# AdeeshKolluru/AdsorbDiff

Measured on AMD Instinct MI355X. Metric: sampled adsorbate sites/sec (50 denoise steps, ~200-atom slabs), higher is better.
Workload: dtype f32 (f16x3-split MFMA, fp32 accumulate; ADF_GEMM=f32 selects exact f32)

## Files before the change

### adsorbdiff_amd/csrc/api.hip

```cpp
#include <stdarg.h>
#include <stdlib.h>
#include <string.h>

#include <new>

#include "common.h"

static thread_local char g_err[512] = "";

void adf_set_error(const char* fmt, ...) {
    va_list ap;
    va_start(ap, fmt);
    vsnprintf(g_err, sizeof(g_err), fmt, ap);
    va_end(ap);
}

extern "C" const char* adf_last_error(void) { return g_err; }
extern "C" const char* adf_version(void) { return "adsorbdiff_hip 0.5.0 (gfx950)"; }

void adf_prof_begin(adf_painn* h, int cat, hipStream_t s) {
    if (!h->prof_on) return;
    if (h->prof_used + 2 > h->prof_ev->size()) {
        for (int i = 0; i < 512; ++i) {
            hipEvent_t e;
            if (hipEventCreate(&e) != hipSuccess) return;
            h->prof_ev->push_back(e);
        }
    }
    h->prof_cat->push_back(cat);
    (void)hipEventRecord((*h->prof_ev)[h->prof_used], s);
    h->prof_used += 1;
}
void adf_prof_end(adf_painn* h, hipStream_t s) {
    if (!h->prof_on || (h->prof_used & 1) == 0) return;
    (void)hipEventRecord((*h->prof_ev)[h->prof_used], s);
    h->prof_used += 1;
}

extern "C" int32_t adf_profile_enable(adf_painn_t h, int32_t on) {
    if (!h) { adf_set_error("null handle"); return ADF_EINVAL; }
    h->prof_on = on != 0;
    h->prof_used = 0;
    h->prof_cat->clear();
    ADF_HIP_CHECK(hipMemset(h->kcount, 0, 8 * sizeof(unsigned long long)));
    return ADF_OK;
}

extern "C" int32_t adf_profile_read(adf_painn_t h, float* ms, int64_t* count, int64_t* message_ksteps, void* stream) {
    if (!h || !ms || !count) { adf_set_error("null argument"); return ADF_EINVAL; }
    ADF_HIP_CHECK(hipStreamSynchronize((hipStream_t)stream));
    if (message_ksteps) {
        unsigned long long k[8];
        ADF_HIP_CHECK(hipMemcpy(k, h->kcount, sizeof(k), hipMemcpyDeviceToHost));
        ADF_HIP_CHECK(hipMemset(h->kcount, 0, sizeof(k)));
        *message_ksteps = (int64_t)k[0];
    }
    for (int c = 0; c < ADF_PROF_NCAT; ++c) { ms[c] = 0.f; count[c] = 0; }
    const size_t pairs = h->prof_used / 2;
    for (size_t i = 0; i < pairs; ++i) {
        float t = 0.f;
        ADF_HIP_CHECK(hipEventElapsedTime(&t, (*h->prof_ev)[2 * i], (*h->prof_ev)[2 * i + 1]));
        const int c = (*h->prof_cat)[i];
        ms[c] += t;
        count[c] += 1;
    }
    h->prof_used = 0;
    h->prof_cat->clear();
    return ADF_OK;
}

template <typename T>
static int32_t dev_alloc(T** p, size_t count) {
    if (*p) { (void)hipFree(*p); *p = nullptr; }
    if (count == 0) return ADF_OK;
    hipError_t e = hipMalloc(reinterpret_cast<void**>(p), count * sizeof(T));
    if (e != hipSuccess) {
        *p = nullptr;
        (void)hipGetLastError();
        adf_set_error("hipMalloc of %zu bytes failed: %s", count * sizeof(T), hipGetErrorString(e));
        return ADF_EOOM;
    }
    return ADF_OK;
}

extern "C" int32_t adf_painn_create(const adf_painn_hparams* hp, adf_painn_t* out) {
    if (!hp || !out) { adf_set_error("null argument"); return ADF_EINVAL; }
    if (hp->hidden_channels % ADF_SLICE_CH != 0 || hp->hidden_channels < 128 || hp->hidden_channels > 1024) {
        adf_set_error("hidden_channels=%d must be a multiple of %d in [128,1024]", hp->hidden_channels, ADF_SLICE_CH);
        return ADF_EINVAL;
    }
    if (hp->num_rbf % 2 != 0 || hp->num_rbf > 128 || hp->num_rbf < 2) {
        adf_set_error("num_rbf=%d must be even and <= 128", hp->num_rbf);
        return ADF_EINVAL;
    }
    if (hp->max_neighbors < 1 || hp->max_neighbors > ADF_MAX_K) {
        adf_set_error("max_neighbors=%d must be in [1,%d]", hp->max_neighbors, ADF_MAX_K);
        return ADF_EINVAL;
    }
    if (hp->num_layers < 1 || hp->num_layers > 16 || hp->num_heads < 0 || hp->num_heads > 2) {
        adf_set_error("num_layers must be in [1,16], num_heads in [0,2]");
        return ADF_EINVAL;
    }
    adf_painn* h = new (std::nothrow) adf_painn();
    if (!h) { adf_set_error("host allocation failed"); return ADF_EOOM; }
    memset(h, 0, sizeof(*h));
    h->hp = *hp;
    h->prof_ev = new std::vector<hipEvent_t>();
    h->prof_cat = new std::vector<int>();
    hipDeviceProp_t prop;
    if (hipGetDevice(&h->device) != hipSuccess || hipGetDeviceProperties(&prop, h->device) != hipSuccess) {
        adf_set_error("no usable HIP device: %s", hipGetErrorString(hipGetLastError()));
        adf_painn_destroy(h);
        return ADF_EHIP;
    }
    h->num_cus = prop.multiProcessorCount;
    h->dist_floor = 1.0e-3f;
    {
        const char* e = getenv("ADF_INCREMENTAL");
        h->inc_on = !(e && e[0] == '0');
        const char* e2 = getenv("ADF_INC_SYNC");
        h->inc_sync = e2 && e2[0] == '1';
    }
    const int H = hp->hidden_channels, R = hp->num_rbf, L = hp->num_layers;
    int32_t st = dev_alloc(&h->rbf_pack, (size_t)L * (H / ADF_SLICE_CH) * R * 192);
    if (st == ADF_OK) st = dev_alloc(&h->rbf_bias_pack, (size_t)L * (H / ADF_SLICE_CH) * 192);
    {
        uint16_t* p16 = nullptr;
        if (st == ADF_OK) st = dev_alloc(&p16, (size_t)L * (H / ADF_SLICE_CH) * R * 192 * 2);
        h->rbf_pack16 = p16;
    }
    if (st == ADF_OK) st = dev_alloc(&h->rbf_bias_pack16, (size_t)L * (H / ADF_SLICE_CH) * 192);
    if (st == ADF_OK) st = dev_alloc(&h->rbf_scales, 16);
    if (st == ADF_OK) st = dev_alloc(&h->flags, ADF_NFLAGS);
    if (st == ADF_OK && hipMemset(h->flags, 0, sizeof(int32_t) * ADF_NFLAGS) != hipSuccess) st = ADF_EHIP;
    {
        const size_t HH = (size_t)H * H;
        const size_t per_layer = HH + 3 * HH + 2 * HH + 2 * HH + 3 * HH;
        const size_t per_head = HH + HH / 2 + 2 * HH + HH + HH / 4 + HH / 2;
        const size_t elems = (size_t)L * per_layer + (size_t)hp->num_heads * per_head;
        h->w16_bytes = elems * 2 * sizeof(uint16_t) + 4096;
        if (st == ADF_OK) st = dev_alloc(&h->w16_arena, h->w16_bytes);
        if (st == ADF_OK) st = dev_alloc(&h->w16_scales, 256);
        if (st == ADF_OK) st = dev_alloc(&h->w16_bias_perm, (size_t)L * 2 * 3 * H);
        if (st == ADF_OK) st = dev_alloc(&h->w16_scratch, 1);
        if (st == ADF_OK) st = dev_alloc(&h->wfrag_arena, h->w16_bytes);
        {
            const char* ef = getenv("ADF_FUSED_MLP");
            h->fused_mlp = ef ? atoi(ef) : 0;
            if (h->fused_mlp < 0 || h->fused_mlp > 2) h->fused_mlp = 0;
        }
        const char* e = getenv("ADF_GEMM");
        h->gemm_f32 = e && strcmp(e, "f32") == 0;
        const char* el = getenv("ADF_LIFT");
        h->lift_on = !(el && strcmp(el, "0") == 0);
        const char* e2 = getenv("ADF_MSG");
        h->msg_f32 = e2 ? strcmp(e2, "f32") == 0 : h->gemm_f32;
        const char* er = getenv("ADF_ROW_MAXIMA");
        h->rmx = (er && atoi(er) == 0) ? 0 : 1;
    }
    if (st == ADF_OK) st = dev_alloc(&h->kcount, 8);
    if (st == ADF_OK && hipMemset(h->kcount, 0, 8 * sizeof(unsigned long long)) != hipSuccess) st = ADF_EHIP;
    if (st != ADF_OK) { adf_painn_destroy(h); return st; }
    *out = h;
    return ADF_OK;
}

static void inc_free(adf_painn* h) {
    for (int l = 0; l <= ADF_MAX_LAYERS; ++l) {
        if (h->incX[l]) (void)hipFree(h->incX[l]);
        if (h->incV[l]) (void)hipFree(h->incV[l]);
        if (l < ADF_MAX_LAYERS && h->incR[l]) (void)hipFree(h->incR[l]);
        h->incX[l] = h->incV[l] = nullptr;
        if (l < ADF_MAX_LAYERS) h->incR[l] = nullptr;
    }
    void* ptrs[] = {h->inc_c0, h->inc_chg, h->inc_pend, h->inc_need, h->inc_tf, h->inc_list, h->inc_cnt, h->inc_tmp};
    for (void* p : ptrs)
        if (p) (void)hipFree(p);
    h->inc_c0 = h->inc_chg = h->inc_pend = h->inc_need = h->inc_tf = nullptr;
    h->inc_list = h->inc_cnt = nullptr; h->inc_tmp = nullptr; h->inc_tmp_bytes = 0;
    h->inc_capN = 0; h->inc_valid = false;
}

static void free_workspaces(adf_painn* h) {
    void* ptrs[] = {h->nbr_cnt, h->nbr_src, h->nbr_shift, h->deg, h->nptr, h->cursor, h->img_cnt, h->sys_slow, h->scan_tmp,
                    h->e_src, h->e_geom, h->x, h->vecA, h->vecB, h->y, h->xh, h->vv, h->cat, h->dot, h->sys, h->rec, h->lift.buf, h->mag_a, h->mag_b, h->mag_v3,
                    h->rmx_part, h->cache_d2, h->cache_cid, h->cache_cnt, h->prev_nptr, h->prev_src, h->prev_geom};
    for (void* p : ptrs)
        if (p) (void)hipFree(p);
    h->prev_nptr = h->prev_src = nullptr; h->prev_geom = nullptr; h->inc_valid = false;
    h->nbr_cnt = h->nbr_src = h->nbr_shift = h->deg = h->nptr = h->cursor = h->img_cnt = h->sys_slow = h->e_src = nullptr;
    h->scan_tmp = nullptr; h->scan_tmp_bytes = 0;
    h->e_geom = nullptr;
    h->x = h->vecA = h->vecB = h->y = h->xh = h->vv = h->cat = h->dot = h->sys = h->rec = nullptr;
    h->lift.buf = h->mag_a = h->mag_b = h->mag_v3 = nullptr; h->lift.cap = 0; h->mag_v3_valid = false;
    h->rmx_part = h->xpart = h->catpart = h->vpart = nullptr; h->part_stride = 0;
    h->part_x = h->part_vec = nullptr; h->dbg_msg_rows = h->dbg_cat_rows = h->dbg_comb_rows = 0; h->dbg_mag = nullptr;
    h->cache_d2 = nullptr; h->cache_cid = nullptr; h->cache_cnt = nullptr; h->cache_valid = false;
    h->capN = h->capB = h->capE = 0;
}

extern "C" int32_t adf_painn_destroy(adf_painn_t h) {
    if (!h) return ADF_OK;
    free_workspaces(h);
    if (h->rbf_pack) (void)hipFree(h->rbf_pack);
    if (h->rbf_bias_pack) (void)hipFree(h->rbf_bias_pack);
    if (h->rec0) (void)hipFree(h->rec0);
    inc_free(h);
    if (h->inc_cnt_host) (void)hipHostFree(h->inc_cnt_host);
    for (int i = 0; i < 2; ++i)
        if (h->inc_ev[i]) (void)hipEventDestroy((hipEvent_t)h->inc_ev[i]);
    if (h->sub_x) (void)hipFree(h->sub_x);
    if (h->sub_vec) (void)hipFree(h->sub_vec);
    if (h->sub_f) (void)hipFree(h->sub_f);
    if (h->rbf_pack16) (void)hipFree(h->rbf_pack16);
    if (h->rbf_bias_pack16) (void)hipFree(h->rbf_bias_pack16);
    if (h->rbf_scales) (void)hipFree(h->rbf_scales);
    if (h->flags) (void)hipFree(h->flags);
    if (h->kcount) (void)hipFree(h->kcount);
    if (h->w16_arena) (void)hipFree(h->w16_arena);
    if (h->wfrag_arena) (void)hipFree(h->wfrag_arena);
    if (h->w16_scales) (void)hipFree(h->w16_scales);
    if (h->w16_bias_perm) (void)hipFree(h->w16_bias_perm);
    if (h->w16_scratch) (void)hipFree(h->w16_scratch);
    if (h->oe0_buf) (void)hipFree(h->oe0_buf);
    adf_grad_free(h);
    if (h->prof_ev) { for (hipEvent_t e : *h->prof_ev) (void)hipEventDestroy(e); delete h->prof_ev; }
    delete h->prof_cat;
    delete h;
    return ADF_OK;
}

extern "C" int32_t adf_painn_set_weights(adf_painn_t h, int32_t n_weights, const void* const* w,
                                         const float* scale_factors, void* stream) {
    if (!h || !w || !scale_factors) { adf_set_error("null argument"); return ADF_EINVAL; }
    const int L = h->hp.num_layers;
    const int expect = 2 + ADF_WEIGHTS_PER_LAYER * L + ADF_WEIGHTS_PER_HEAD * h->hp.num_heads;
    if (n_weights != expect) {
        adf_set_error("expected %d weight tensors, got %d", expect, n_weights);
        return ADF_EINVAL;
    }
    for (int i = 0; i < n_weights; ++i)
        if (!w[i]) { adf_set_error("weight %d is null", i); return ADF_EINVAL; }
    auto f = [&](int i) { return reinterpret_cast<const float*>(w[i]); };
    h->emb = f(0);
    h->rbf_offset = f(1);
    int k = 2;
    for (int l = 0; l < L; ++l) {
        adf_layer_weights& lw = h->layer[l];
        lw.ln_w = f(k++); lw.ln_b = f(k++); lw.xp0_w = f(k++); lw.xp0_b = f(k++); lw.xp2_w = f(k++); lw.xp2_b = f(k++);
        lw.rbf_w = f(k++); lw.rbf_b = f(k++); lw.vp_w = f(k++); lw.xv0_w = f(k++); lw.xv0_b = f(k++);
        lw.xv2_w = f(k++); lw.xv2_b = f(k++);
        h->scale[l] = scale_factors[l];
    }
    for (int hd = 0; hd < h->hp.num_heads; ++hd)
        for (int b = 0; b < 2; ++b) {
            adf_block_weights& bw = h->head[hd][b];
            bw.vec1_w = f(k++); bw.vec2_w = f(k++); bw.un0_w = f(k++); bw.un0_b = f(k++); bw.un2_w = f(k++);
            bw.un2_b = f(k++);
        }
    ADF_TRY(adf_pack_rbf(h, (hipStream_t)stream));
    {
        hipStream_t s = (hipStream_t)stream;
        const long long H = h->hp.hidden_channels, HH = H * H;
        unsigned char* cur = h->w16_arena;
        unsigned char* fcur = h->wfrag_arena;
        int nscale = 0;
        float* bperm = h->w16_bias_perm;
        auto split = [&](const float* w, long long rows, long long K, adf_w16* out, const float* fused_bias = nullptr,
                         bool pair_perm = false) -> int32_t {
            const long long n = rows * K;
            out->hi = cur; cur += n * 2;
            out->lo = cur; cur += n * 2;
            out->inv_scale = h->w16_scales + nscale++;
            out->bias_perm = nullptr;
            out->frag = nullptr;
            if (fused_bias) {
                out->bias_perm = bperm; bperm += 3 * H;
                ADF_TRY(adf_split_weight(w, n, out, h->w16_scratch, s, (int)H, (int)H, fused_bias));
            } else if (pair_perm) {
                ADF_TRY(adf_split_weight(w, n, out, h->w16_scratch, s, (int)H, (int)H, nullptr, 2));
            } else {
                ADF_TRY(adf_split_weight(w, n, out, h->w16_scratch, s));
            }
            if (rows % 32 == 0 && K % 16 == 0) {
                out->frag = fcur; fcur += n * 4;
                ADF_TRY(adf_pack_frag(out, (int)rows, (int)K, out->frag, s));
            }
            return ADF_OK;
        };
        for (int l = 0; l < L; ++l) {
            adf_layer_weights& lw = h->layer[l];
            ADF_TRY(split(lw.xp0_w, H, H, &lw.xp0_16));
            ADF_TRY(split(lw.xp2_w, 3 * H, H, &lw.xp2_16, lw.xp2_b));
            ADF_TRY(split(lw.vp_w, 2 * H, H, &lw.vp_16, nullptr, true));
            ADF_TRY(split(lw.xv0_w, H, 2 * H, &lw.xv0_16));
            ADF_TRY(split(lw.xv2_w, 3 * H, H, &lw.xv2_16, lw.xv2_b));
        }
        for (int hd = 0; hd < h->hp.num_heads; ++hd) {
            adf_block_weights& b0 = h->head[hd][0];
            adf_block_weights& b1 = h->head[hd][1];
            ADF_TRY(split(b0.vec1_w, H, H, &b0.vec1_16));
            ADF_TRY(split(b0.vec2_w, H / 2, H, &b0.vec2_16));
            ADF_TRY(split(b0.un0_w, H, 2 * H, &b0.un0_16));
            ADF_TRY(split(b0.un2_w, H, H, &b0.un2_16));
            ADF_TRY(split(b1.vec1_w, H / 2, H / 2, &b1.vec1_16));
            ADF_TRY(split(b1.un0_w, H / 2, H, &b1.un0_16));
        }
        if ((size_t)(cur - h->w16_arena) > h->w16_bytes || (size_t)(fcur - h->wfrag_arena) > h->w16_bytes || nscale > 256) {
            adf_set_error("internal: fp16 weight arena overflow");
            return ADF_EINVAL;
        }
    }
    h->weights_set = true;
    h->rec0_valid = false;
    h->inc_valid = false;
    adf_grad_invalidate(h);
    return ADF_OK;
}

static int32_t ensure_capacity(adf_painn* h, int64_t N, int64_t B) {
    if (N <= h->capN && B <= h->capB) return ADF_OK;
    const int64_t capN = N > h->capN ? N : h->capN;
    const int64_t capB = B > h->capB ? B : h->capB;
    ADF_HIP_CHECK(hipDeviceSynchronize());
    free_workspaces(h);
    const int64_t H = h->hp.hidden_channels, K = h->hp.max_neighbors;
    const int64_t capE = 2 * capN * K;
    int32_t st = ADF_OK;
#define ALLOC(field, count) if (st == ADF_OK) st = dev_alloc(&h->field, (size_t)(count))
    ALLOC(nbr_cnt, capN);
    ALLOC(nbr_src, capN * K);
    ALLOC(nbr_shift, capN * K);
    ALLOC(cache_d2, capN * K);
    ALLOC(cache_cid, capN * K);
    ALLOC(cache_cnt, capN);
    ALLOC(deg, capN + 1);
    ALLOC(nptr, capN + 1);
    ALLOC(cursor, capN);
    ALLOC(img_cnt, capB);
    ALLOC(sys_slow, capB);
    ALLOC(e_src, capE);
    ALLOC(e_geom, capE);
    if (h->inc_on) {
        ALLOC(prev_nptr, capN + 1);
        ALLOC(prev_src, capE);
        ALLOC(prev_geom, capE);
    }
    if (st == ADF_OK) {
        h->scan_tmp_bytes = adf_scan_temp_bytes(capN + 1);
        unsigned char* tmp = nullptr;
        st = dev_alloc(&tmp, h->scan_tmp_bytes + 16);
        h->scan_tmp = tmp;
    }
    ALLOC(x, capN * H);
    ALLOC(vecA, capN * 3 * H);
    ALLOC(vecB, capN * 3 * H);
    ALLOC(rec, (capN + 1) * 5 * H);
    ALLOC(y, capN * H);
    ALLOC(xh, capN * 3 * H);
    ALLOC(vv, capN * 6 * H);
    ALLOC(cat, capN * 2 * H);
    ALLOC(dot, capN * H);
    ALLOC(sys, capB * 16);
    ALLOC(lift.buf, capN * 3);
    ALLOC(mag_a, capN);
    ALLOC(mag_b, capN);
    ALLOC(mag_v3, capN * 3);
    const int64_t ps = (capN + 31) / 32 * 32, ns = H / ADF_SLICE_CH;
    if (h->rmx) ALLOC(rmx_part, (4 * ns + H / 32 + 4) * ps);
#undef ALLOC
    h->lift.cap = st == ADF_OK ? capN * 3 : 0;
    if (st != ADF_OK) { free_workspaces(h); return st; }
    if (h->rmx) {
        h->part_stride = ps;
        h->xpart = h->rmx_part; h->catpart = h->xpart + ns * ps; h->vpart = h->catpart + (H / 32) * ps;
        h->dbg_mag = h->vpart + 3 * ns * ps;
    }
    h->capN = capN; h->capB = capB; h->capE = capE;
    return ADF_OK;
}

static int32_t check_batch(const adf_painn* h, const adf_batch* b) {
    if (!h || !b) { adf_set_error("null argument"); return ADF_EINVAL; }
    if (b->num_atoms <= 0 || b->num_systems <= 0) { adf_set_error("empty batch"); return ADF_EINVAL; }
    if (!b->pos || !b->cell || !b->batch || !b->atom_offset) { adf_set_error("null batch array"); return ADF_EINVAL; }
    for (int k = 0; k < 3; ++k)
        if (b->reps[k] < 0 || b->reps[k] > 16) { adf_set_error("reps[%d]=%d out of range", k, b->reps[k]); return ADF_EINVAL; }
    return ADF_OK;
}

static int32_t read_flags(adf_painn* h, hipStream_t s) {
    int32_t f[ADF_NFLAGS];
    ADF_HIP_CHECK(hipMemcpyAsync(f, h->flags, sizeof(f), hipMemcpyDeviceToHost, s));
    ADF_HIP_CHECK(hipMemsetAsync(h->flags, 0, sizeof(f), s));
    ADF_HIP_CHECK(hipStreamSynchronize(s));
    if (f[4]) { adf_set_error("atomic number outside [1, %d] (rows of the embedding table)", h->hp.num_elements); return ADF_EINVAL; }
    if (f[0]) { adf_set_error("a centre atom has more than %d in-cutoff candidates", ADF_MAX_CAND); return ADF_EOVERFLOW; }
    if (f[2]) { adf_set_error("edge buffer overflow"); return ADF_EOVERFLOW; }
    if (f[3]) { adf_set_error("an atom has more than %d incoming edges", ADF_MAX_INDEG); return ADF_EOVERFLOW; }
    if (f[1]) { adf_set_error("An image has no neighbors"); return ADF_ENONEIGHBOR; }
    if (f[6]) { adf_set_error("energy gradient: an edge row has no reverse row in its partner's segment (asymmetric graph)"); return ADF_EINVAL; }
    if (f[5]) {
        adf_set_error("non-finite model output%s", h->gemm_f32 ? " (exact-f32 arithmetic: the inputs or weights are not finite)"
                      : " in f16x3 arithmetic: an activation left the fp16 range or the inputs are not finite; "
                        "adf_painn_set_arithmetic(h, 1) selects exact f32");
        return ADF_ENUMERIC;
    }
    return ADF_OK;
}

extern "C" int32_t adf_graph_set_moving(adf_painn_t h, const int32_t* moving, const int32_t* mov_idx,
                                        const int32_t* mov_off) {
    if (!h) { adf_set_error("null handle"); return ADF_EINVAL; }
    if (moving && (!mov_idx || !mov_off)) { adf_set_error("moving mask needs mov_idx and mov_off"); return ADF_EINVAL; }
    h->moving = moving; h->mov_idx = mov_idx; h->mov_off = mov_off;
    ADF_HIP_CHECK(hipMemset(h->flags, 0, sizeof(int32_t) * ADF_NFLAGS));
    h->cache_valid = false;
    h->rec0_valid = false;
    h->inc_valid = false;
    return ADF_OK;
}

extern "C" int32_t adf_graph_build(adf_painn_t h, const adf_batch* b, void* stream, int64_t* num_edges) {
    ADF_TRY(check_batch(h, b));
    ADF_TRY(ensure_capacity(h, b->num_atoms, b->num_systems));
    hipStream_t s = (hipStream_t)stream;
    ADF_TRY(adf_graph_build_impl(h, b, s));
    if (num_edges) {
        int32_t e = 0;
        ADF_HIP_CHECK(hipMemcpyAsync(&e, h->nptr + b->num_atoms, sizeof(int32_t), hipMemcpyDeviceToHost, s));
        ADF_TRY(read_flags(h, s));
        *num_edges = e;
    }
    return ADF_OK;
}

__global__ void adf_export_edges_kernel(const int32_t* nptr, const int32_t* e_src, const float4* eg, int N,
                                        int32_t* src, int32_t* dst, float* dist, float* vec, long long cap) {
    const int n = blockIdx.x * 4 + (threadIdx.x >> 6);
    if (n >= N) return;
    for (int e = nptr[n] + (threadIdx.x & 63); e < nptr[n + 1]; e += 64) {
        if (e >= cap) continue;
        if (src) src[e] = e_src[e];
        if (dst) dst[e] = n;
        const float4 q = eg[e];
        if (dist) dist[e] = q.w;
        if (vec) { vec[3 * (size_t)e] = q.x; vec[3 * (size_t)e + 1] = q.y; vec[3 * (size_t)e + 2] = q.z; }
    }
}

__global__ void adf_export_shift_kernel(const int32_t* nbr_shift, int32_t* out, long long n, int r0, int r1, int r2) {
    const long long i = (long long)blockIdx.x * blockDim.x + threadIdx.x;
    if (i >= n) return;
    const int c = nbr_shift[i];
    const int n2 = 2 * r2 + 1, n1 = 2 * r1 + 1;
    const int ia = c / (n1 * n2), rem = c - ia * (n1 * n2);
    out[3 * i] = ia - r0;
    out[3 * i + 1] = rem / n2 - r1;
    out[3 * i + 2] = rem % n2 - r2;
}

extern "C" int32_t adf_graph_export(adf_painn_t h, int32_t* nbr_count, int32_t* nbr_src, int32_t* nbr_shift,
                                    int64_t edge_capacity, int32_t* edge_src, int32_t* edge_dst, float* edge_dist,
                                    float* edge_vec, int64_t* num_edges, void* stream) {
    if (!h || h->lastN <= 0) { adf_set_error("no graph built"); return ADF_EINVAL; }
    hipStream_t s = (hipStream_t)stream;
    const int64_t N = h->lastN, K = h->hp.max_neighbors;
    if (nbr_count) ADF_HIP_CHECK(hipMemcpyAsync(nbr_count, h->nbr_cnt, sizeof(int32_t) * N, hipMemcpyDeviceToDevice, s));
    if (nbr_src) ADF_HIP_CHECK(hipMemcpyAsync(nbr_src, h->nbr_src, sizeof(int32_t) * N * K, hipMemcpyDeviceToDevice, s));
    if (nbr_shift)
        hipLaunchKernelGGL(adf_export_shift_kernel, dim3((unsigned)((N * K + 255) / 256)), dim3(256), 0, s, h->nbr_shift,
                           nbr_shift, (long long)(N * K), h->last_reps[0], h->last_reps[1], h->last_reps[2]);
    if (edge_src || edge_dst || edge_dist || edge_vec)
        hipLaunchKernelGGL(adf_export_edges_kernel, dim3((unsigned)((N + 3) / 4)), dim3(256), 0, s, h->nptr, h->e_src,
                           h->e_geom, (int)N, edge_src, edge_dst, edge_dist, edge_vec, (long long)edge_capacity);
    ADF_HIP_CHECK(hipGetLastError());
    int32_t e = 0;
    ADF_HIP_CHECK(hipMemcpyAsync(&e, h->nptr + N, sizeof(int32_t), hipMemcpyDeviceToHost, s));
    ADF_HIP_CHECK(hipStreamSynchronize(s));
    if (num_edges) *num_edges = e;
    return ADF_OK;
}

static int32_t zero_pad_rows(adf_painn* h, int N, hipStream_t s) {
    const size_t row = (size_t)5 * h->hp.hidden_channels;
    ADF_HIP_CHECK(hipMemsetAsync(h->rec + (size_t)N * row, 0, sizeof(float) * row, s));
    return ADF_OK;
}

static bool use_fused_mlp(const adf_painn* h, int rows) {
    if (h->hp.hidden_channels != 512 || h->gemm_f32 || h->fused_mlp == 0) return false;
    if (h->fused_mlp == 1) return true;
    return rows >= 2 * 64 * h->num_cus;
}

static int32_t make_records(adf_painn* h, int l, int n, const float* x, const float* vec, bool vec_is_zero, float* rec,
                            const int32_t* row_map, hipStream_t s) {
    const int H = h->hp.hidden_channels;
    const adf_layer_weights& w = h->layer[l];
    if (n <= 0) return ADF_OK;
    adf_prof_begin(h, ADF_PROF_NODE, s);
    const bool lift = h->lift_on && !h->gemm_f32;
    static int emit = -1;
    if (emit < 0) { const char* e = getenv("ADF_LIFT_EMIT"); emit = (e && atoi(e) == 0) ? 0 : 1; }
    const bool em = lift && emit;
    ADF_TRY(adf_nodewise_layernorm(x, w.ln_w, w.ln_b, h->y, n, H, s, em ? h->mag_a : nullptr, h->rows_dev));
    if (use_fused_mlp(h, n) && (em || !lift)) {
        adf_epi ep = {};
        ep.vec_in = vec; ep.rec = rec ? rec : h->rec; ep.H = H; ep.vec_is_zero = vec_is_zero ? 1 : 0;
        ep.row_map = row_map; ep.m_dev = h->rows_dev; ep.lift_y = lift ? 1 : 0;
        ep.rec_rows = row_map ? (long long)h->inc_capN : (long long)n;
        ADF_TRY(adf_launch_mlp16(h->y, nullptr, H, em ? h->mag_a : nullptr, w.xp0_16.frag, &w.xp0_16, w.xp0_b, w.xp2_16.frag, &w.xp2_16, n,
                                 H, 1, &ep, s));
        adf_prof_end(h, s);
        return ADF_OK;
    }
    ADF_TRY(adf_linear(h, h->y, H, w.xp0_w, &w.xp0_16, w.xp0_b, h->cat, H, n, H, H, 1, s, em ? h->mag_a : nullptr,
                       em ? h->mag_b : nullptr));
    if (h->gemm_f32) {
        if (row_map) { adf_set_error("internal: mapped records need the f16x3 path"); return ADF_EINVAL; }
        ADF_TRY(adf_launch_gemm(h->cat, H, w.xp2_w, H, w.xp2_b, h->xh, 3 * H, n, 3 * H, H, 0, s));
        ADF_TRY(adf_pack_records(h, n, h->xh, vec, vec_is_zero, s, rec));
    } else {
        adf_epi ep = {};
        ep.vec_in = vec; ep.rec = rec ? rec : h->rec; ep.H = H; ep.vec_is_zero = vec_is_zero ? 1 : 0;
        ep.row_map = row_map;
        ep.rmag = em ? h->mag_b : nullptr;
        ep.m_dev = h->rows_dev;
        ADF_TRY(adf_launch_gemm16_fused(h->cat, H, &w.xp2_16, n, H, H, 1, &ep, s, lift ? &h->lift : nullptr));
    }
    adf_prof_end(h, s);
    return ADF_OK;
}

static int32_t message_layer(adf_painn* h, int l, int N, const float* x, const float* vec, float* x_out,
                             float* vec_out, bool vec_is_zero, hipStream_t s, const int32_t* tlist = nullptr,
                             int n_targets = 0, float* rec = nullptr, bool records_ready = false) {
    if (!records_ready) ADF_TRY(make_records(h, l, N, x, vec, vec_is_zero, rec, nullptr, s));
    adf_prof_begin(h, ADF_PROF_MESSAGE, s);
    const int items = tlist ? n_targets : N;
    const bool emit = h->rmx && h->lift_on && !h->gemm_f32 && !h->msg_f32 && items > 0 && items <= h->part_stride;
    h->part_x = h->part_vec = nullptr;
    const int32_t st = adf_message_impl(h, l, N, x, h->xh, vec, x_out, vec_out, vec_is_zero, s, tlist, n_targets, rec,
                                        tlist ? h->rows_dev : nullptr, emit ? h->xpart : nullptr, h->vpart, h->part_stride);
    if (st == ADF_OK && emit) {
        h->part_x = x_out; h->part_vec = vec_out; h->part_n = items; h->part_dev = tlist ? h->rows_dev : nullptr;
        h->dbg_msg_rows = items;
    }
    adf_prof_end(h, s);
    return st;
}

static int32_t update_layer(adf_painn* h, int l, int N, float* x, float* vec, hipStream_t s, bool from_message = true) {
    const int H = h->hp.hidden_channels;
    const adf_layer_weights& w = h->layer[l];
    adf_prof_begin(h, ADF_PROF_NODE, s);
    const bool parts = from_message && h->rmx && h->lift_on && !h->gemm_f32 && N > 0 && h->part_x == x && h->part_vec == vec &&
                       h->part_n == N && h->part_dev == h->rows_dev;
    h->part_x = h->part_vec = nullptr;
    if (h->gemm_f32) {
        ADF_TRY(adf_launch_gemm(vec, H, w.vp_w, H, nullptr, h->vv, 2 * H, 3 * N, 2 * H, H, 0, s));
        ADF_TRY(adf_nodewise_update_prep(h->vv, x, h->cat, h->dot, N, H, s));
        ADF_TRY(adf_linear(h, h->cat, 2 * H, w.xv0_w, &w.xv0_16, w.xv0_b, h->y, H, N, H, 2 * H, 1, s));
    } else {
        adf_epi ep = {};
        ep.v1 = h->vv; ep.dotw = h->dot; ep.cat = h->cat; ep.H = H; ep.m_dev = h->rows_dev;
        const adf_lift* lf = h->lift_on ? &h->lift : nullptr;
        if (parts) {
            ADF_TRY(adf_launch_rowmax_combine(h->vpart, 3 * h->part_stride, H / ADF_SLICE_CH, 3ll * N, h->lift.buf, s, h->rows_dev, 3));
            ep.rmag = h->lift.buf;
            if (h->dbg_capture) ADF_HIP_CHECK(hipMemcpyAsync(h->dbg_mag, h->lift.buf, sizeof(float) * 3 * (size_t)N, hipMemcpyDeviceToDevice, s));
        }
        if (parts || (h->dbg_capture && h->rmx && lf && N <= h->part_stride)) {
            ep.catpart = h->catpart; ep.part_stride = h->part_stride; h->dbg_cat_rows = N;
        }
        ADF_TRY(adf_launch_gemm16_fused(vec, H, &w.vp_16, N, H, H, 3, &ep, s, lf));
        if (parts) {
            ADF_TRY(adf_launch_rowmax_combine(h->xpart, h->part_stride, H / ADF_SLICE_CH + H / 32, N, h->lift.buf, s, h->rows_dev, 1));
            if (h->dbg_capture) {
                ADF_HIP_CHECK(hipMemcpyAsync(h->dbg_mag + 3 * h->part_stride, h->lift.buf, sizeof(float) * (size_t)N, hipMemcpyDeviceToDevice, s));
                h->dbg_comb_rows = N;
            }
        }
        if (use_fused_mlp(h, N)) {
            const float* rm = nullptr;
            if (lf) {
                if (N > lf->cap) { adf_set_error("mlp16: lift scratch holds %lld rows, need %d", lf->cap, N); return ADF_EINVAL; }
                if (!parts) ADF_TRY(adf_launch_rowmag(x, H, H, h->cat, H, N, lf->buf, s, h->rows_dev, 1));
                rm = lf->buf;
            }
            adf_epi e2 = {};
            e2.x = x; e2.vec = vec; e2.dot = h->dot; e2.vv = h->vv; e2.scale = h->scale[l]; e2.H = H;
            e2.m_dev = h->rows_dev; e2.lift_y = h->lift_on ? 1 : 0;
            const int32_t stf = adf_launch_mlp16(x, h->cat, H, rm, w.xv0_16.frag, &w.xv0_16, w.xv0_b, w.xv2_16.frag, &w.xv2_16, N, H, 2, &e2, s);
            adf_prof_end(h, s);
            return stf;
        }
        ADF_TRY(adf_launch_gemm16(x, H, &w.xv0_16, w.xv0_b, h->y, H, N, H, 2 * H, 1, s, h->cat, H, lf, parts ? h->lift.buf : nullptr,
                                  h->lift_on ? h->mag_b : nullptr, h->rows_dev));
    }
    int32_t st;
    if (h->gemm_f32) {
        ADF_TRY(adf_launch_gemm(h->y, H, w.xv2_w, H, w.xv2_b, h->xh, 3 * H, N, 3 * H, H, 0, s));
        st = adf_nodewise_update_apply(h->xh, h->dot, h->vv, x, vec, h->scale[l], N, H, s);
    } else {
        adf_epi ep = {};
        ep.x = x; ep.vec = vec; ep.dot = h->dot; ep.vv = h->vv; ep.scale = h->scale[l]; ep.H = H;
        ep.rmag = h->lift_on ? h->mag_b : nullptr;
        ep.m_dev = h->rows_dev;
        st = adf_launch_gemm16_fused(h->y, H, &w.xv2_16, N, H, H, 2, &ep, s);
    }
    adf_prof_end(h, s);
    return st;
}

extern "C" int32_t adf_painn_message_layer(adf_painn_t h, int32_t layer, int32_t N, const float* x, const float* vec,
                                           float* x_out, float* vec_out, void* stream) {
    if (!h || !h->weights_set || layer < 0 || layer >= h->hp.num_layers || N != h->lastN) {
        adf_set_error("message_layer: bad handle/layer, or N differs from the built graph");
        return ADF_EINVAL;
    }
    hipStream_t s = (hipStream_t)stream;
    ADF_TRY(zero_pad_rows(h, N, s));
    ADF_TRY(message_layer(h, layer, N, x, vec, x_out, vec_out, false, s));
    return ADF_OK;
}

extern "C" int32_t adf_painn_update_layer(adf_painn_t h, int32_t layer, int32_t N, float* x, float* vec, void* stream) {
    if (!h || !h->weights_set || layer < 0 || layer >= h->hp.num_layers) {
        adf_set_error("update_layer: bad handle/layer");
        return ADF_EINVAL;
    }
    ADF_TRY(ensure_capacity(h, N, 1));
    return update_layer(h, layer, N, x, vec, (hipStream_t)stream, false);
}

extern "C" int32_t adf_painn_debug_row_maxima(adf_painn_t h, int32_t which, float* out, int64_t capacity, int32_t* rows,
                                              void* stream) {
    if (!h || which < 0 || which > 6) { adf_set_error("debug_row_maxima: null handle or which outside 0..6"); return ADF_EINVAL; }
    if (which == 4) { h->dbg_capture = capacity != 0; h->dbg_comb_rows = 0; return ADF_OK; }
    const int H = h->hp.hidden_channels, ns = H / ADF_SLICE_CH;
    const int n = which <= 1 ? h->dbg_msg_rows : which <= 3 ? h->dbg_cat_rows : h->dbg_comb_rows;
    if (!h->rmx_part || n <= 0) { adf_set_error("debug_row_maxima: no launch has emitted row maxima (ADF_ROW_MAXIMA=0?)"); return ADF_EINVAL; }
    if (rows) *rows = n;
    if (!out) return ADF_OK;
    const int64_t need = (which == 1 || which == 5) ? 3ll * n : which == 3 ? (int64_t)n * H : n;
    if (capacity < need) { adf_set_error("debug_row_maxima: out holds %lld floats, need %lld", (long long)capacity, (long long)need); return ADF_EINVAL; }
    hipStream_t s = (hipStream_t)stream;
    if (which == 0) return adf_launch_rowmax_combine(h->xpart, h->part_stride, ns, n, out, s);
    if (which == 1) return adf_launch_rowmax_combine(h->vpart, 3 * h->part_stride, ns, 3ll * n, out, s);
    if (which == 2) return adf_launch_rowmax_combine(h->catpart, h->part_stride, H / 32, n, out, s);
    if (which >= 5) {
        ADF_HIP_CHECK(hipMemcpyAsync(out, h->dbg_mag + (which == 5 ? 0 : 3 * h->part_stride), sizeof(float) * (size_t)need, hipMemcpyDeviceToDevice, s));
        return ADF_OK;
    }
    ADF_HIP_CHECK(hipMemcpyAsync(out, h->cat, sizeof(float) * (size_t)n * H, hipMemcpyDeviceToDevice, s));
    return ADF_OK;
}

__global__ void adf_scatter_rows3_kernel(const float* __restrict__ src, const int32_t* __restrict__ idx, int n,
                                         float* __restrict__ dst) {
    const int i = blockIdx.x * blockDim.x + threadIdx.x;
    if (i < 3 * n) dst[(size_t)idx[i / 3] * 3 + i % 3] = src[i];
}

static int32_t forward_impl(adf_painn_t h, const adf_batch* b, const int32_t* out_idx, int32_t n_out, float* f1,
                            float* f2, void* stream, bool head1_only = false);

extern "C" int32_t adf_painn_forward(adf_painn_t h, const adf_batch* b, float* f1, float* f2, void* stream) {
    return forward_impl(h, b, nullptr, 0, f1, f2, stream);
}

extern "C" int32_t adf_painn_forward_subset(adf_painn_t h, const adf_batch* b, const int32_t* out_idx, int32_t n_out,
                                            float* f1, float* f2, void* stream) {
    if (!out_idx || n_out < 0) { adf_set_error("forward_subset: null index list"); return ADF_EINVAL; }
    return forward_impl(h, b, out_idx, n_out, f1, f2, stream);
}

static int inc_prepare(adf_painn* h, int N) {
    const int L = h->hp.num_layers, H = h->hp.hidden_channels;
    if (!h->inc_on || !h->moving || h->gemm_f32 || h->msg_f32 || L > ADF_MAX_LAYERS || !h->prev_nptr)
        return 0;
    if (N > h->inc_capN) {
        (void)hipDeviceSynchronize();
        inc_free(h);
        const size_t cap = (size_t)N;
        int32_t st = ADF_OK;
        for (int l = 0; l <= L && st == ADF_OK; ++l) {
            st = dev_alloc(&h->incX[l], cap * H);
            if (st == ADF_OK && l >= 1) st = dev_alloc(&h->incV[l], cap * 3 * H);
            if (st == ADF_OK && l < L) st = dev_alloc(&h->incR[l], (cap + 1) * 5 * H);
        }
        if (st == ADF_OK) st = dev_alloc(&h->inc_c0, cap);
        if (st == ADF_OK) st = dev_alloc(&h->inc_chg, 2 * cap);
        if (st == ADF_OK) st = dev_alloc(&h->inc_pend, cap * L);
        if (st == ADF_OK) st = dev_alloc(&h->inc_need, cap * L);
        if (st == ADF_OK) st = dev_alloc(&h->inc_tf, cap * L);
        if (st == ADF_OK) st = dev_alloc(&h->inc_list, cap * L);
        if (st == ADF_OK) st = dev_alloc(&h->inc_cnt, (size_t)2 * ADF_MAX_LAYERS + 1);
        if (st == ADF_OK) {
            h->inc_tmp_bytes = adf_inc_temp_bytes((int64_t)cap);
            unsigned char* tmp = nullptr;
            st = dev_alloc(&tmp, h->inc_tmp_bytes + 16);
            h->inc_tmp = tmp;
        }
        if (st == ADF_OK && !h->inc_cnt_host &&
            hipHostMalloc(reinterpret_cast<void**>(&h->inc_cnt_host), sizeof(int32_t) * 2 * (2 * ADF_MAX_LAYERS + 1)) != hipSuccess)
            st = ADF_EOOM;
        for (int i = 0; i < 2 && st == ADF_OK; ++i)
            if (!h->inc_ev[i] && hipEventCreateWithFlags(reinterpret_cast<hipEvent_t*>(&h->inc_ev[i]), hipEventDisableTiming) != hipSuccess)
                st = ADF_EHIP;
        if (st != ADF_OK) {
            (void)hipGetLastError();
            inc_free(h);
            h->inc_on = false;
            fprintf(stderr, "adsorbdiff_hip: no memory for incremental layers (%d atoms), continuing without\n", N);
            return 0;
        }
        h->inc_capN = (int64_t)cap;
    }
    if (h->inc_N != N || h->inc_layers != L || h->build_serial != h->inc_serial) h->inc_valid = false;
    h->inc_N = N; h->inc_layers = L;
    int32_t* tn = h->nptr; h->nptr = h->prev_nptr; h->prev_nptr = tn;
    int32_t* ts = h->e_src; h->e_src = h->prev_src; h->prev_src = ts;
    float4* tg = h->e_geom; h->e_geom = h->prev_geom; h->prev_geom = tg;
    const int state = h->inc_valid ? 1 : 2;
    h->inc_valid = false;
    return state;
}

__global__ void adf_scatter_rows3_kernel(const float* __restrict__ src, const int32_t* __restrict__ idx, int n,
                                         float* __restrict__ dst);

static int32_t inc_harvest(adf_painn* h, int slot, bool wait, bool peek = false) {
    if (!h->inc_ev_live[slot]) return ADF_OK;
    hipEvent_t ev = (hipEvent_t)h->inc_ev[slot];
    if (wait) {
        ADF_HIP_CHECK(hipEventSynchronize(ev));
    } else {
        const hipError_t q = hipEventQuery(ev);
        if (q == hipErrorNotReady) { (void)hipGetLastError(); return ADF_OK; }
        ADF_HIP_CHECK(q);
    }
    const int L = h->inc_layers, N = h->inc_pend_N[slot];
    const int32_t* c = h->inc_cnt_host + (size_t)slot * (2 * ADF_MAX_LAYERS + 1);
    for (int i = 0; i < 2 * L + 1; ++i) h->inc_seen[i] = c[i];
    h->inc_seen_valid = true;
    h->inc_pend_Nseen = N;
    if (peek) return ADF_OK;
    h->inc_ev_live[slot] = false;
    for (int l = 0; l < L; ++l) {
        const bool whole = h->inc_pend_whole[slot][l] != 0;
        h->inc_rows += (unsigned long long)(whole ? N : c[l]);
        h->inc_rows_full += (unsigned long long)N;
        h->inc_edges += (unsigned long long)(whole ? c[2 * L] : c[L + l]);
        if (whole || c[l] > 0) ++h->inc_launches;
    }
    return ADF_OK;
}

static int32_t forward_incremental(adf_painn* h, int N, const int32_t* Z, const int32_t* out_idx, int32_t n_out,
                                   float* f1, float* f2, bool first, int heads, hipStream_t s) {
    const int L = h->hp.num_layers, H = h->hp.hidden_channels;
    const size_t cap = (size_t)h->inc_capN, row = (size_t)5 * H;
    if (out_idx && n_out == 0) return ADF_OK;
    adf_prof_begin(h, ADF_PROF_GRAPH, s);
    if (first) {
        ADF_TRY(adf_nodewise_embed(h, Z, N, h->incX[0], s));
        for (int l = 0; l < L; ++l) ADF_HIP_CHECK(hipMemsetAsync(h->incR[l] + (size_t)N * row, 0, sizeof(float) * row, s));
        ADF_HIP_CHECK(hipMemsetAsync(h->inc_pend, 0, cap * L, s));
    } else {
        ADF_TRY(adf_inc_compare(h, N, s));
    }
    ADF_HIP_CHECK(hipMemsetAsync(h->inc_cnt, 0, sizeof(int32_t) * (2 * ADF_MAX_LAYERS + 1), s));
    if (out_idx) ADF_TRY(adf_inc_need_from_list(h, N, L, out_idx, n_out, s));
    for (int l = 0; l < L; ++l) ADF_TRY(adf_inc_plan_layer(h, l, N, first, out_idx != nullptr, s));
    ADF_HIP_CHECK(hipMemcpyAsync(h->inc_cnt + 2 * L, h->nptr + N, sizeof(int32_t), hipMemcpyDeviceToDevice, s));
    const int slot = h->inc_slot;
    h->inc_slot ^= 1;
    if (h->inc_ev_live[slot]) ADF_TRY(inc_harvest(h, slot, true));
    int32_t* host = h->inc_cnt_host + (size_t)slot * (2 * ADF_MAX_LAYERS + 1);
    ADF_HIP_CHECK(hipMemcpyAsync(host, h->inc_cnt, sizeof(int32_t) * (2 * L + 1), hipMemcpyDeviceToHost, s));
    ADF_HIP_CHECK(hipEventRecord((hipEvent_t)h->inc_ev[slot], s));
    h->inc_ev_live[slot] = true;
    h->inc_pend_N[slot] = N;
    ADF_TRY(inc_harvest(h, slot ^ 1, false));
    if (h->inc_sync) ADF_TRY(inc_harvest(h, slot, true, true));
    adf_prof_end(h, s);
    if (first) ADF_TRY(make_records(h, 0, N, h->incX[0], nullptr, true, h->incR[0], nullptr, s));
    for (int l = 0; l < L; ++l) {
        const int n_seen = h->inc_seen_valid ? h->inc_seen[l] : N;
        const bool whole = first || !h->inc_seen_valid || h->inc_pend_Nseen != N || (long long)n_seen * 10 >= (long long)N * 9;
        h->inc_pend_whole[slot][l] = whole ? 1 : 0;
        if (h->inc_sync && !whole && n_seen == 0) continue;
        const float* vin = l == 0 ? h->vecA : h->incV[l];
        if (whole) {
            ADF_TRY(message_layer(h, l, N, h->incX[l], vin, h->incX[l + 1], h->incV[l + 1], l == 0, s, nullptr, 0,
                                  h->incR[l], true));
            ADF_TRY(update_layer(h, l, N, h->incX[l + 1], h->incV[l + 1], s));
            if (l + 1 < L)
                ADF_TRY(make_records(h, l + 1, N, h->incX[l + 1], h->incV[l + 1], false, h->incR[l + 1], nullptr, s));
            continue;
        }
        const int32_t* list = h->inc_list + cap * l;
        const int ncap = h->inc_sync ? n_seen : N;
        h->rows_dev = h->inc_cnt + l;
        int32_t st = message_layer(h, l, N, h->incX[l], vin, h->x, h->vecB, l == 0, s, list, ncap, h->incR[l], true);
        if (st == ADF_OK) st = update_layer(h, l, ncap, h->x, h->vecB, s);
        if (st == ADF_OK) {
            adf_prof_begin(h, ADF_PROF_NODE, s);
            st = adf_inc_scatter_rows(h->x, list, ncap, H, h->incX[l + 1], s, h->rows_dev);
            if (st == ADF_OK) st = adf_inc_scatter_rows(h->vecB, list, ncap, 3 * H, h->incV[l + 1], s, h->rows_dev);
            adf_prof_end(h, s);
        }
        if (st == ADF_OK && l + 1 < L) st = make_records(h, l + 1, ncap, h->x, h->vecB, false, h->incR[l + 1], list, s);
        h->rows_dev = nullptr;
        ADF_TRY(st);
    }
    adf_prof_begin(h, ADF_PROF_HEADS, s);
    if (!out_idx) {
        if (heads >= 1) ADF_TRY(adf_head_forward(h, 0, N, h->incX[L], h->incV[L], f1, s));
        if (heads == 2) ADF_TRY(adf_head_forward(h, 1, N, h->incX[L], h->incV[L], f2, s));
        h->x_last = h->incX[L];
    } else {
        if (n_out > h->capS) {
            const int64_t c = (int64_t)n_out + n_out / 4 + 64;
            if (h->sub_x) (void)hipFree(h->sub_x);
            if (h->sub_vec) (void)hipFree(h->sub_vec);
            if (h->sub_f) (void)hipFree(h->sub_f);
            h->sub_x = h->sub_vec = h->sub_f = nullptr; h->capS = 0;
            ADF_TRY(dev_alloc(&h->sub_x, (size_t)c * H));
            ADF_TRY(dev_alloc(&h->sub_vec, (size_t)c * 3 * H));
            ADF_TRY(dev_alloc(&h->sub_f, (size_t)c * 3));
            h->capS = c;
        }
        ADF_TRY(adf_inc_gather_rows(h->incX[L], out_idx, n_out, H, h->sub_x, s));
        ADF_TRY(adf_inc_gather_rows(h->incV[L], out_idx, n_out, 3 * H, h->sub_vec, s));
        for (int hd = 0; hd < heads; ++hd) {
            ADF_TRY(adf_head_forward(h, hd, n_out, h->sub_x, h->sub_vec, h->sub_f, s));
            hipLaunchKernelGGL(adf_scatter_rows3_kernel, dim3((3 * n_out + 255) / 256), dim3(256), 0, s, h->sub_f, out_idx,
                               n_out, hd == 0 ? f1 : f2);
        }
        ADF_HIP_CHECK(hipGetLastError());
    }
    adf_prof_end(h, s);
    h->inc_valid = true;
    return ADF_OK;
}

static int32_t forward_impl(adf_painn_t h, const adf_batch* b, const int32_t* out_idx, int32_t n_out, float* f1,
                            float* f2, void* stream, bool head1_only) {
    ADF_TRY(check_batch(h, b));
    if (!h->weights_set) { adf_set_error("weights not set"); return ADF_EINVAL; }
    const int heads = head1_only ? 1 : h->hp.num_heads;
    if (heads > h->hp.num_heads) { adf_set_error("the model has no force head"); return ADF_EINVAL; }
    if (!b->atomic_numbers || (heads >= 1 && !f1) || (heads == 2 && !f2)) { adf_set_error("null argument"); return ADF_EINVAL; }
    h->x_last = nullptr;
    hipStream_t s = (hipStream_t)stream;
    const int N = b->num_atoms;
    ADF_TRY(ensure_capacity(h, N, b->num_systems));
    const int inc = inc_prepare(h, N);
    adf_prof_begin(h, ADF_PROF_GRAPH, s);
    ADF_TRY(adf_graph_build_impl(h, b, s));
    adf_prof_end(h, s);
    if (inc) {
        h->inc_serial = h->build_serial;
        return forward_incremental(h, N, b->atomic_numbers, out_idx, n_out, f1, f2, inc == 2, heads, s);
    }
    ADF_TRY(zero_pad_rows(h, N, s));
    ADF_TRY(adf_nodewise_embed(h, b->atomic_numbers, N, h->x, s));
    float* vin = h->vecA;
    float* vout = h->vecB;
    const int L = h->hp.num_layers, H = h->hp.hidden_channels;
    float* rec0 = nullptr;
    bool rec0_ready = false;
    if (h->moving) {
        const size_t row = (size_t)5 * H;
        if ((int64_t)N + 1 > h->rec0_cap) {
            if (h->rec0) { (void)hipFree(h->rec0); h->rec0 = nullptr; }
            h->rec0_cap = 0; h->rec0_valid = false;
            ADF_TRY(dev_alloc(&h->rec0, ((size_t)N + 1) * row));
            h->rec0_cap = (int64_t)N + 1;
        }
        rec0 = h->rec0;
        rec0_ready = h->rec0_valid && h->rec0_N == N;
        if (!rec0_ready) ADF_HIP_CHECK(hipMemsetAsync(rec0 + (size_t)N * row, 0, sizeof(float) * row, s));
        h->rec0_valid = true; h->rec0_N = N;
    }
    if (!out_idx) {
        for (int l = 0; l < L; ++l) {
            if (l == 0) ADF_TRY(message_layer(h, 0, N, h->x, vin, h->x, vout, true, s, nullptr, 0, rec0, rec0_ready));
            else
            ADF_TRY(message_layer(h, l, N, h->x, vin, h->x, vout, l == 0, s));
            ADF_TRY(update_layer(h, l, N, h->x, vout, s));
            float* t = vin; vin = vout; vout = t;
        }
        adf_prof_begin(h, ADF_PROF_HEADS, s);
        if (heads >= 1) ADF_TRY(adf_head_forward(h, 0, N, h->x, vin, f1, s));
        if (heads == 2) ADF_TRY(adf_head_forward(h, 1, N, h->x, vin, f2, s));
        adf_prof_end(h, s);
        h->x_last = h->x;
        return ADF_OK;
    }
    if (n_out == 0) return ADF_OK;
    if (n_out > h->capS) {
        const int64_t cap = (int64_t)n_out + n_out / 4 + 64;
        if (h->sub_x) (void)hipFree(h->sub_x);
        if (h->sub_vec) (void)hipFree(h->sub_vec);
        if (h->sub_f) (void)hipFree(h->sub_f);
        h->sub_x = h->sub_vec = h->sub_f = nullptr; h->capS = 0;
        ADF_TRY(dev_alloc(&h->sub_x, (size_t)cap * H));
        ADF_TRY(dev_alloc(&h->sub_vec, (size_t)cap * 3 * H));
        ADF_TRY(dev_alloc(&h->sub_f, (size_t)cap * 3));
        h->capS = cap;
    }
    for (int l = 0; l + 1 < L; ++l) {
        if (l == 0) ADF_TRY(message_layer(h, 0, N, h->x, vin, h->x, vout, true, s, nullptr, 0, rec0, rec0_ready));
        else
        ADF_TRY(message_layer(h, l, N, h->x, vin, h->x, vout, l == 0, s));
        ADF_TRY(update_layer(h, l, N, h->x, vout, s));
        float* t = vin; vin = vout; vout = t;
    }
    ADF_TRY(message_layer(h, L - 1, N, h->x, vin, h->sub_x, h->sub_vec, L == 1, s, out_idx, n_out,
                          L == 1 ? rec0 : nullptr, L == 1 && rec0_ready));
    ADF_TRY(update_layer(h, L - 1, n_out, h->sub_x, h->sub_vec, s));
    adf_prof_begin(h, ADF_PROF_HEADS, s);
    for (int hd = 0; hd < heads; ++hd) {
        ADF_TRY(adf_head_forward(h, hd, n_out, h->sub_x, h->sub_vec, h->sub_f, s));
        hipLaunchKernelGGL(adf_scatter_rows3_kernel, dim3((3 * n_out + 255) / 256), dim3(256), 0, s, h->sub_f, out_idx,
                           n_out, hd == 0 ? f1 : f2);
    }
    ADF_HIP_CHECK(hipGetLastError());
    adf_prof_end(h, s);
    return ADF_OK;
}

extern "C" int32_t adf_painn_set_energy_head(adf_painn_t h, int32_t n_weights, const void* const* w, void* stream) {
    if (!h || !w) { adf_set_error("null argument"); return ADF_EINVAL; }
    if (n_weights != 4) { adf_set_error("set_energy_head: expected 4 tensors (out_energy.0.weight/bias, out_energy.2.weight/bias), got %d", n_weights); return ADF_EINVAL; }
    for (int i = 0; i < 4; ++i)
        if (!w[i]) { adf_set_error("energy-head tensor %d is null", i); return ADF_EINVAL; }
    const int H = h->hp.hidden_channels, H2 = H / 2;
    const size_t n = (size_t)H2 * H;
    if (!h->oe0_buf) ADF_TRY(dev_alloc(&h->oe0_buf, n * 4 + 64));
    h->oe0_w = reinterpret_cast<const float*>(w[0]);
    h->oe0_b = reinterpret_cast<const float*>(w[1]);
    h->oe2_w = reinterpret_cast<const float*>(w[2]);
    h->oe2_b = reinterpret_cast<const float*>(w[3]);
    adf_w16& e = h->oe0_16;
    e = adf_w16{};
    e.hi = h->oe0_buf; e.lo = h->oe0_buf + n * 2; e.inv_scale = reinterpret_cast<float*>(h->oe0_buf + n * 4);
    ADF_TRY(adf_split_weight(h->oe0_w, (long long)n, &e, reinterpret_cast<unsigned int*>(h->oe0_buf + n * 4 + 16),
                             (hipStream_t)stream));
    h->energy_set = true;
    adf_grad_invalidate(h);
    return ADF_OK;
}

extern "C" int32_t adf_painn_set_distance_floor(adf_painn_t h, float floor) {
    if (!h || !(floor > 0.f)) { adf_set_error("set_distance_floor: null handle or non-positive floor"); return ADF_EINVAL; }
    if (floor != h->dist_floor) {
        h->dist_floor = floor;
        h->cache_valid = false;
        h->rec0_valid = false;
        h->inc_valid = false;
    }
    return ADF_OK;
}

__global__ __launch_bounds__(256) void adf_energy_sum_kernel(const float* __restrict__ y, int H2, const float* __restrict__ w,
                                                             const float* __restrict__ bias, const int32_t* __restrict__ atom_offset,
                                                             float* __restrict__ energy) {
    __shared__ float part[4];
    const int b = blockIdx.x, lane = threadIdx.x & 63, wave = threadIdx.x >> 6;
    const int a0 = atom_offset[b], a1 = atom_offset[b + 1];
    const float b0 = bias[0];
    float acc = 0.f;
    for (int a = a0 + wave; a < a1; a += 4) {
        const float* row = y + (size_t)a * H2;
        float d = 0.f;
        for (int c = lane; c < H2; c += 64) d = fmaf(row[c], w[c], d);
        for (int o = 32; o > 0; o >>= 1) d = __fadd_rn(d, __shfl_xor(d, o, 64));
        acc = __fadd_rn(acc, __fadd_rn(d, b0));
    }
    if (lane == 0) part[wave] = acc;
    __syncthreads();
    if (threadIdx.x == 0) energy[b] = __fadd_rn(__fadd_rn(part[0], part[1]), __fadd_rn(part[2], part[3]));
}

int32_t adf_energy_sum(const float* y, int H2, const float* w, const float* bias, const int32_t* atom_offset, float* energy,
                       int num_systems, hipStream_t s) {
    hipLaunchKernelGGL(adf_energy_sum_kernel, dim3(num_systems), dim3(256), 0, s, y, H2, w, bias, atom_offset, energy);
    ADF_HIP_CHECK(hipGetLastError());
    return ADF_OK;
}

extern "C" int32_t adf_painn_forward_energy(adf_painn_t h, const adf_batch* b, float* energy, float* forces, void* stream) {
    ADF_TRY(check_batch(h, b));
    if (!h->energy_set) { adf_set_error("forward_energy: energy head not set (adf_painn_set_energy_head)"); return ADF_EINVAL; }
    if (!energy || (h->hp.num_heads >= 1 && !forces)) { adf_set_error("forward_energy: null output"); return ADF_EINVAL; }
    if (h->hp.num_heads > 1) { adf_set_error("forward_energy: the S2EF model has one force head"); return ADF_EINVAL; }
    hipStream_t s = (hipStream_t)stream;
    ADF_TRY(forward_impl(h, b, nullptr, 0, forces, nullptr, stream));
    if (!h->x_last) { adf_set_error("internal: no node features after the forward"); return ADF_EINVAL; }
    const int N = b->num_atoms, H = h->hp.hidden_channels, H2 = H / 2;
    adf_prof_begin(h, ADF_PROF_HEADS, s);
    ADF_TRY(adf_linear(h, h->x_last, H, h->oe0_w, &h->oe0_16, h->oe0_b, h->y, H2, N, H2, H, 1, s));
    ADF_TRY(adf_energy_sum(h->y, H2, h->oe2_w, h->oe2_b, b->atom_offset, energy, b->num_systems, s));
    adf_prof_end(h, s);
    return ADF_OK;
}

extern "C" int32_t adf_linear_forward(const float* A, const float* W, const float* bias, float* C, int32_t M,
                                      int32_t N, int32_t K, int32_t act_ssilu, int32_t mode, void* stream) {
    hipStream_t s = (hipStream_t)stream;
    if (!A || !W || !C || M <= 0 || N <= 0 || K <= 0) { adf_set_error("bad argument"); return ADF_EINVAL; }
    if (mode == 0) return adf_launch_gemm(A, K, W, K, bias, C, N, M, N, K, act_ssilu, s);
    unsigned char* buf = nullptr;
    const size_t n = (size_t)N * K;
    ADF_TRY(dev_alloc(&buf, n * 4 + 64));
    adf_w16 w16 = {};
    w16.hi = buf; w16.lo = buf + n * 2; w16.inv_scale = reinterpret_cast<float*>(buf + n * 4);
    unsigned int* scratch = reinterpret_cast<unsigned int*>(buf + n * 4 + 16);
    int32_t st = adf_split_weight(W, (long long)n, &w16, scratch, s);
    float* mags = nullptr;
    const char* el = getenv("ADF_LIFT");
    const bool lift = !(el && strcmp(el, "0") == 0);
    if (st == ADF_OK && lift) st = dev_alloc(&mags, (size_t)M);
    adf_lift lf = {mags, M};
    if (st == ADF_OK) st = adf_launch_gemm16(A, K, &w16, bias, C, N, M, N, K, act_ssilu, s, nullptr, 0, lift ? &lf : nullptr);
    (void)hipStreamSynchronize(s);
    (void)hipFree(buf);
    if (mags) (void)hipFree(mags);
    return st;
}

extern "C" int32_t adf_painn_set_arithmetic(adf_painn_t h, int32_t exact_f32) {
    if (!h) { adf_set_error("null handle"); return ADF_EINVAL; }
    h->gemm_f32 = exact_f32 != 0;
    h->msg_f32 = exact_f32 != 0;
    h->rec0_valid = false;
    h->inc_valid = false;
    return ADF_OK;
}

extern "C" int32_t adf_painn_set_fused_mlp(adf_painn_t h, int32_t mode) {
    if (!h || mode < 0 || mode > 2) { adf_set_error("set_fused_mlp: mode must be 0 (never), 1 (always) or 2 (by size)"); return ADF_EINVAL; }
    h->fused_mlp = mode;
    return ADF_OK;
}

extern "C" int32_t adf_painn_set_incremental(adf_painn_t h, int32_t on) {
// ... 127 lines not shown
```

### adsorbdiff_amd/csrc/common.h

```cpp
#pragma once
#include <hip/hip_runtime.h>
#include <stdint.h>
#include <stdio.h>
#include <string>
#include <vector>

#include "../../include/adsorbdiff_hip.h"

#define ADF_GROUP_NODES 32
#define ADF_SLICE_CH 64
#define ADF_MAX_CAND 1024
#define ADF_MAX_K 128
#define ADF_NFLAGS 8
#define ADF_MAX_INDEG 1024
#define ADF_MAX_LAYERS 16

void adf_set_error(const char* fmt, ...);

#define ADF_HIP_CHECK(expr)                                                             \
    do {                                                                                \
        hipError_t _e = (expr);                                                         \
        if (_e != hipSuccess) {                                                         \
            adf_set_error("%s failed: %s (%s:%d)", #expr, hipGetErrorString(_e),        \
                          __FILE__, __LINE__);                                          \
            return (_e == hipErrorOutOfMemory) ? ADF_EOOM : ADF_EHIP;                   \
        }                                                                               \
    } while (0)

#define ADF_TRY(expr)                     \
    do {                                  \
        int32_t _s = (expr);              \
        if (_s != ADF_OK) return _s;      \
    } while (0)

struct adf_w16 {
    void* hi;
    void* lo;
    float* inv_scale;
    float* bias_perm;
    void* frag;
};
struct adf_epi {
    const float* vec_in;
    float* rec;
    float* x;
    float* vec;
    const float* dot;
    const float* vv;
    float* v1;
    float* dotw;
    float* cat;
    float scale;
    int H;
    int vec_is_zero;
    const float* A2;
    int K1;
    const int32_t* row_map;
    const float* rmag;
    unsigned int* out_mag;
    const int32_t* m_dev;
    int accumulate;
    int lift_y;
    const float* gate;
    int gate_ld;
    long long rec_rows;
    float* catpart;
    long long part_stride;
};
struct adf_lift {
    float* buf;
    long long cap;
};
struct adf_layer_weights {
    const float *ln_w, *ln_b, *xp0_w, *xp0_b, *xp2_w, *xp2_b, *rbf_w, *rbf_b;
    const float *vp_w, *xv0_w, *xv0_b, *xv2_w, *xv2_b;
    adf_w16 xp0_16, xp2_16, vp_16, xv0_16, xv2_16;
};
struct adf_block_weights {
    const float *vec1_w, *vec2_w, *un0_w, *un0_b, *un2_w, *un2_b;
    adf_w16 vec1_16, vec2_16, un0_16, un2_16;
};

struct adf_painn {
    adf_painn_hparams hp;
    int device;
    bool weights_set;
    const float* emb;
    const float* rbf_offset;
    adf_layer_weights layer[16];
    adf_block_weights head[2][2];
    float scale[16];
    float* rbf_pack;
    float* rbf_bias_pack;
    void* rbf_pack16;
    float* rbf_bias_pack16;
    float* rbf_scales;
    unsigned char* w16_arena;
    size_t w16_bytes;
    float* w16_scales;
    float* w16_bias_perm;
    unsigned int* w16_scratch;
    unsigned char* wfrag_arena;
    int fused_mlp;
    bool gemm_f32;
    bool msg_f32;
    bool lift_on;
    adf_lift lift;
    float *mag_a, *mag_b;
    float* mag_v3;
    bool mag_v3_valid;
    int rmx;
    float* rmx_part;
    float *xpart, *catpart, *vpart;
    int64_t part_stride;
    const float *part_x, *part_vec;
    int part_n;
    const int32_t* part_dev;
    int dbg_msg_rows, dbg_cat_rows;
    bool dbg_capture;
    float* dbg_mag;
    int dbg_comb_rows;

    int64_t capN, capB, capE;
    int32_t* nbr_cnt;
    int32_t* nbr_src;
    int32_t* nbr_shift;
    int32_t* deg;
    int32_t* nptr;
    int32_t* cursor;
    int32_t* img_cnt;
    int32_t* sys_slow;
    void* scan_tmp;
    size_t scan_tmp_bytes;
    const int32_t* moving;
    const int32_t* mov_idx;
    const int32_t* mov_off;
    float* cache_d2;
    int32_t* cache_cid;
    int32_t* cache_cnt;
    bool cache_valid;
    int32_t* e_src;
    float4* e_geom;
    int32_t* flags;
    float *x, *vecA, *vecB, *y, *xh, *vv, *cat, *dot;
    float* rec;
    bool rbf_uniform;
    float* rec0;
    int64_t rec0_cap, rec0_N;
    bool rec0_valid;
    bool inc_on;
    bool inc_valid;
    int64_t inc_capN, inc_N;
    int inc_layers;
    float* incX[ADF_MAX_LAYERS + 1];
    float* incV[ADF_MAX_LAYERS + 1];
    float* incR[ADF_MAX_LAYERS];
    int32_t *prev_nptr, *prev_src;
    float4* prev_geom;
    unsigned char *inc_c0, *inc_chg;
    unsigned char *inc_pend, *inc_need, *inc_tf;
    int32_t* inc_list;
    int32_t* inc_cnt;
    int32_t* inc_cnt_host;
    void* inc_ev[2];
    bool inc_ev_live[2];
    int inc_slot;
    bool inc_sync;
    int32_t inc_seen[2 * ADF_MAX_LAYERS + 1];
    bool inc_seen_valid;
    unsigned char inc_pend_whole[2][ADF_MAX_LAYERS];
    int32_t inc_pend_N[2];
    int32_t inc_pend_Nseen;
    const int32_t* rows_dev;
    void* inc_tmp; size_t inc_tmp_bytes;
    unsigned long long inc_rows, inc_rows_full, inc_edges, inc_launches;
    unsigned long long build_serial, inc_serial;
    float *sub_x, *sub_vec, *sub_f;
    int64_t capS;
    float* sys;
    const float *oe0_w, *oe0_b, *oe2_w, *oe2_b;
    adf_w16 oe0_16;
    unsigned char* oe0_buf;
    bool energy_set;
    const float* x_last;
    float dist_floor;
    void* grad;
    int64_t lastN, lastB;
    int32_t last_reps[3];
    int num_cus;
    bool prof_on;
    std::vector<hipEvent_t>* prof_ev;
    std::vector<int>* prof_cat;
    size_t prof_used;
    unsigned long long* kcount;
};

enum { ADF_PROF_GRAPH = 0, ADF_PROF_MESSAGE = 1, ADF_PROF_NODE = 2, ADF_PROF_HEADS = 3, ADF_PROF_STEPPER = 4 };
void adf_prof_begin(adf_painn* h, int cat, hipStream_t s);
void adf_prof_end(adf_painn* h, hipStream_t s);

int32_t adf_launch_gemm(const float* A, int lda, const float* W, int ldw, const float* bias, float* C, int ldc,
                        int M, int N, int K, int act_ssilu, hipStream_t s);
int32_t adf_launch_gemm16(const float* A, int lda, const adf_w16* W, const float* bias, float* C, int ldc, int M,
                          int N, int K, int act_ssilu, hipStream_t s, const float* A2 = nullptr, int K1 = 0,
                          const adf_lift* lf = nullptr, const float* premag = nullptr, float* out_mag = nullptr,
                          const int32_t* m_dev = nullptr, int accumulate = 0,
                          const float* gate = nullptr, int gate_ld = 0);
int32_t adf_launch_rowmag(const float* A, int lda, int K1, const float* A2, int K2, long long M, float* mag, hipStream_t s,
                          const int32_t* m_dev = nullptr, int m_mul = 1);
int32_t adf_launch_rowmax_combine(const float* part, long long stride, int nparts, long long M, float* mag, hipStream_t s,
                                  const int32_t* m_dev = nullptr, int m_mul = 1);
int32_t adf_split_weight(const float* w, long long n, adf_w16* out, unsigned int* scratch_bits, hipStream_t s,
                         int perm_H = 0, int K = 0, const float* bias = nullptr, int parts = 3);
int32_t adf_launch_gemm16_vecnorm(const float* A, int lda, const adf_w16* W, float* nrm, int M, int N, int K,
                                  hipStream_t s, const adf_lift* lf = nullptr, const float* premag = nullptr);
int32_t adf_launch_gemm16_fused(const float* A, int lda, const adf_w16* W, int M, int H, int K, int epi,
                                const adf_epi* ep, hipStream_t s, const adf_lift* lf = nullptr);
static inline int32_t adf_linear(const adf_painn* h, const float* A, int lda, const float* W, const adf_w16* W16,
                                 const float* bias, float* C, int ldc, int M, int N, int K, int act, hipStream_t s,
                                 const float* premag = nullptr, float* out_mag = nullptr) {
    if (h->gemm_f32) return adf_launch_gemm(A, lda, W, K, bias, C, ldc, M, N, K, act, s);
    return adf_launch_gemm16(A, lda, W16, bias, C, ldc, M, N, K, act, s, nullptr, 0, h->lift_on ? &h->lift : nullptr,
                             h->lift_on ? premag : nullptr, h->lift_on ? out_mag : nullptr, h->rows_dev);
}
int32_t adf_pack_frag(const adf_w16* w, int N, int K, void* out, hipStream_t s);
int32_t adf_launch_mlp16(const float* A1, const float* A2, int lda, const float* rmag, const void* W0f, const adf_w16* W0,
                         const float* bias0, const void* W2f, const adf_w16* W2, int M, int H, int epi, const adf_epi* ep,
                         hipStream_t s);
int32_t adf_graph_build_impl(adf_painn* h, const adf_batch* b, hipStream_t s);
int32_t adf_energy_sum(const float* y, int H2, const float* w, const float* bias, const int32_t* atom_offset, float* energy,
                       int num_systems, hipStream_t s);
__device__ __forceinline__ float adf_row16_max(float v) {
#define ADF_ROR(n_) __int_as_float(__builtin_amdgcn_update_dpp(0, __float_as_int(v), 0x120 + (n_), 0xf, 0xf, false))
    v = fmaxf(v, ADF_ROR(8));
    v = fmaxf(v, ADF_ROR(4));
    v = fmaxf(v, ADF_ROR(2));
    v = fmaxf(v, ADF_ROR(1));
#undef ADF_ROR
    return v;
}
__device__ __forceinline__ float adf_half32_max_hi(float v) {
    v = adf_row16_max(v);
    return fmaxf(v, __int_as_float(__builtin_amdgcn_update_dpp(0, __float_as_int(v), 0x142, 0xa, 0xf, false)));
}
__device__ __forceinline__ float adf_lane8_max(float v) {
#define ADF_DPP(c_) __int_as_float(__builtin_amdgcn_update_dpp(0, __float_as_int(v), (c_), 0xf, 0xf, false))
    v = fmaxf(v, ADF_DPP(0xb1));
    v = fmaxf(v, ADF_DPP(0x4e));
    v = fmaxf(v, ADF_DPP(0x141));
#undef ADF_DPP
    return v;
}
__device__ __forceinline__ float adf_ssilu(float x) { return x / (1.0f + expf(-x)) * 1.6666666666666667f; }
__device__ __forceinline__ float adf_dssilu_times(float x, float w) {
    const float sg = 1.0f / (1.0f + expf(-x));
    return sg * (1.0f + x * (1.0f - sg)) * 1.6666666666666667f * w;
}
void adf_grad_invalidate(adf_painn* h);
void adf_grad_free(adf_painn* h);
bool adf_message_geo_supported(const adf_painn* h);
int32_t adf_message_geo(adf_painn* h, int layer, const float* xh, const float* vec, bool vec_is_zero, float4* part,
                        long long ecap, bool accumulate, hipStream_t s);
size_t adf_inc_temp_bytes(int64_t n);
int32_t adf_inc_compare(adf_painn* h, int N, hipStream_t s);
int32_t adf_inc_need_from_list(adf_painn* h, int N, int L, const int32_t* out_idx, int n_out, hipStream_t s);
int32_t adf_inc_plan_layer(adf_painn* h, int l, int N, bool first, bool have_need, hipStream_t s);
int32_t adf_inc_scatter_rows(const float* src, const int32_t* idx, int n, int width, float* dst, hipStream_t s,
                             const int32_t* n_dev = nullptr);
int32_t adf_inc_gather_rows(const float* src, const int32_t* idx, int n, int width, float* dst, hipStream_t s);
size_t adf_scan_temp_bytes(int64_t n);
int32_t adf_message_impl(adf_painn* h, int layer, int N, const float* x, const float* xh, const float* vec,
                         float* x_out, float* vec_out, bool vec_is_zero, hipStream_t s,
                         const int32_t* tlist = nullptr, int n_targets = 0, const float* rec = nullptr,
                         const int32_t* n_targets_dev = nullptr,
                         float* xpart = nullptr, float* vpart = nullptr, long long part_stride = 0);
int32_t adf_pack_rbf(adf_painn* h, hipStream_t s);
int32_t adf_pack_rbf_layer(adf_painn* h, int l, hipStream_t s);
int32_t adf_pack_records(adf_painn* h, int N, const float* xh, const float* vec, bool vec_is_zero, hipStream_t s,
                         float* rec = nullptr);
int32_t adf_nodewise_embed(adf_painn* h, const int32_t* Z, int N, float* x, hipStream_t s);
int32_t adf_nodewise_layernorm(const float* x, const float* w, const float* b, float* y, int N, int H, hipStream_t s,
                               float* out_mag = nullptr, const int32_t* n_dev = nullptr);
int32_t adf_nodewise_update_prep(const float* vv, const float* x, float* cat, float* dot, int N, int H, hipStream_t s);
int32_t adf_nodewise_update_apply(const float* h3, const float* dot, const float* vv, float* x, float* vec,
                                  float scale, int N, int H, hipStream_t s);
int32_t adf_head_forward(adf_painn* h, int head, int N, const float* x, const float* vec, float* out, hipStream_t s);
int32_t adf_stepper_init(const adf_batch* b, float* pos, const int32_t* tags, const float* noise,
                         hipStream_t s);
int32_t adf_stepper_step(float* sys, const adf_batch* b, float* pos, const int32_t* tags, const int32_t* fixed,
                         const float* f1, const float* f2, const adf_step_coef* coef, const adf_step_coef* coefs_dev,
                         int num_steps, const float* z_tr, const float* z_rot, int32_t early_stop_count,
                         int32_t* state, float* dcom, float* drot, hipStream_t s);
int32_t adf_stepper_tr_step(float* sys, const adf_batch* b, float* pos, const int32_t* tags, const float* f1,
                            const adf_tr_coef* coef, const adf_tr_coef* coefs_dev, int num_steps, const float* z,
                            int32_t early_stop_count, int32_t* state, float* dcom, hipStream_t s);

struct adf_model {
    void* h;
    int32_t (*check)(void* h, const adf_batch* b);
    int32_t (*grow)(void* h, const adf_batch* b, float** sys);
    int32_t (*forward)(void* h, const adf_batch* b, const int32_t* out_idx, int32_t n_out, float* f1, float* f2,
                       hipStream_t s);
    void (*prof)(void* h, bool begin, hipStream_t s);
};
int32_t adf_frames_push_impl(adf_frames* f, const float* src, hipStream_t s);
int32_t adf_model_init_placement(const adf_model& m, const adf_batch* b, float* pos, const int32_t* tags,
                                 const float* noise, hipStream_t s);
int32_t adf_model_sde_step(const adf_model& m, const adf_batch* b, float* pos, const int32_t* tags, const int32_t* fixed,
                           const float* f1, const float* f2, const adf_step_coef* coef, const adf_step_coef* coefs_dev,
                           int32_t num_steps, const float* z_tr, const float* z_rot, int32_t early_stop_count,
                           int32_t* state, float* dcom, float* drot, hipStream_t s);
int32_t adf_model_tr_step(const adf_model& m, const adf_batch* b, float* pos, const int32_t* tags, const float* f1,
                          const adf_tr_coef* coef, const adf_tr_coef* coefs_dev, int32_t num_steps, const float* z,
                          int32_t early_stop_count, int32_t* state, float* dcom, hipStream_t s);
int32_t adf_model_sample(const adf_model& m, const adf_batch* b, float* pos, const int32_t* tags, const int32_t* fixed,
                         const adf_step_coef* coefs_dev, int32_t num_steps, const float* z_tr_all, const float* z_rot_all,
                         int32_t early_stop_count, int32_t poll_every, int32_t* state, const int32_t* out_idx,
                         int32_t n_out, float* f1, float* f2, adf_frames* sink, int32_t frame_every, hipStream_t s);
int32_t adf_model_tr_sample(const adf_model& m, const adf_batch* b, float* pos, const int32_t* tags,
                            const adf_tr_coef* coefs_dev, int32_t num_steps, const float* z_all, int32_t early_stop_count,
                            int32_t poll_every, int32_t* state, const int32_t* out_idx, int32_t n_out, float* f1,
                            adf_frames* sink, int32_t frame_every, hipStream_t s);
```

### adsorbdiff_amd/csrc/gemm16.hip

```cpp
#include <stdlib.h>

#include "common.h"

typedef float f32x16 __attribute__((ext_vector_type(16)));
typedef _Float16 half8 __attribute__((ext_vector_type(8)));
typedef _Float16 half4 __attribute__((ext_vector_type(4)));

#ifndef EPI_ABL
#define EPI_ABL 0
#endif
#ifndef EPI2_POLICY
#define EPI2_POLICY 0
#endif
#ifndef G16_ABL
#define G16_ABL 0
#endif
#ifndef G16_WDEEP
#define G16_WDEEP 1
#endif
#define HK 32
#define TLD3 96
#define TLD2 64
#define HLD 40

__device__ __forceinline__ float adf_pow2_lift(float mx) {
    if (!(mx > 0.f) || !(mx < 3.0e38f)) return 1.0f;
    int e;
    (void)frexpf(mx, &e);
    e = 15 - e;
    e = e > 120 ? 120 : (e < -120 ? -120 : e);
    return ldexpf(1.0f, e);
}

__device__ __forceinline__ float ssilu16(float x) {
    float s = x / (1.0f + expf(-x));
    return s * 1.6666666666666667f;
}

template <int ACT, int MI, int NJ, int EPI, bool WR = false, int NWN = 2>
__global__ __launch_bounds__(128 * NWN, (MI == 4 || NWN == 4 ? 1 : 2)) void adf_gemm_f16x3_kernel(
    const float* __restrict__ A, int lda, const _Float16* __restrict__ Whi, const _Float16* __restrict__ Wlo,
    const float* __restrict__ inv_scale, const float* __restrict__ bias, float* __restrict__ C, int ldc, int Mh, int N,
    int K, int tiles_n, adf_epi ep) {
    const int M = ep.m_dev ? min(Mh, (int)*ep.m_dev) : Mh;
    static_assert(NWN == 2 || WR, "eight waves only with the register-streamed weights");
    constexpr int NT = 128 * NWN;
    constexpr int TM = 64 * MI;
    constexpr int TN = 32 * NJ * NWN;
    constexpr int NA = TM * 8 / NT;
    static_assert(TM * 8 % NT == 0, "A staging: whole float4s per thread");
    constexpr int LDS_WR = 4 * TM * HLD > NT / 64 * 6400 ? 4 * TM * HLD : NT / 64 * 6400;
    __shared__ __attribute__((aligned(16))) _Float16 lds[WR ? LDS_WR : (2 * TM + 2 * TN) * HLD];
    __shared__ float rinv[TM];
    _Float16* Ahi = lds;
    _Float16* Alo = Ahi + TM * HLD;
    _Float16* Bhi = Alo + TM * HLD;
    _Float16* Blo = Bhi + TN * HLD;
    const int tid = threadIdx.x;
    const int lane = tid & 63;
    const int wave = tid >> 6;
    const int wm = (wave / NWN) * (32 * MI);
    const int wn = (wave % NWN) * (32 * NJ);

    const int id = blockIdx.x;
    const int xcd = id & 7;
    const int qd = id >> 3;
    const int tile_m = (qd / tiles_n) * 8 + xcd;
    const int tile_n = qd % tiles_n;
    const int m0 = tile_m * (EPI >= 3 ? TM / 3 : TM);
    const int n0 = tile_n * TN;
    if (m0 >= M) return;

    unsigned int a_goff[NA];
    int a_off[NA];
    float a_rs[NA];
    auto global_row = [&](int row) -> unsigned int {
        if constexpr (EPI >= 3) {
            const int atom = m0 + (row / 96) * 32 + (row & 31), ax = (row % 96) >> 5;
            return (unsigned int)min(atom, M - 1) * 3u + ax;
        } else {
            return (unsigned int)min(m0 + row, M - 1);
        }
    };
#pragma unroll
    for (int i = 0; i < NA; ++i) {
        const int f = tid + NT * i;
        const int row = f >> 3, kq = f & 7;
        const unsigned int grow = global_row(row);
        a_goff[i] = (grow * (unsigned int)lda + kq * 4) * 4u;
        a_off[i] = row * HLD + kq * 4;
        a_rs[i] = ep.rmag ? adf_pow2_lift(ep.rmag[grow]) : 1.0f;
    }
    if (tid < TM) rinv[tid] = ep.rmag ? 1.0f / adf_pow2_lift(ep.rmag[global_row(tid)]) : 1.0f;
    const char* const A1b = reinterpret_cast<const char*>(A);
    const char* const A2b = reinterpret_cast<const char*>(ep.A2) - (size_t)ep.K1 * 4;
    int w_src[NJ];
    int w_off[NJ];
#pragma unroll
    for (int i = 0; i < NJ; ++i) {
        const int f = tid + 256 * i;
        const int row = f >> 2, part = f & 3;
        w_src[i] = min(n0 + row, N - 1) * K + part * 8;
        w_off[i] = row * HLD + part * 8;
    }

    float4 ra[NA];
    half8 rwh[NJ], rwl[NJ];
#pragma unroll
    for (int i = 0; i < NA; ++i) ra[i] = *reinterpret_cast<const float4*>(A1b + a_goff[i]);
    if constexpr (!WR) {
#pragma unroll
        for (int i = 0; i < NJ; ++i) {
            rwh[i] = *reinterpret_cast<const half8*>(Whi + w_src[i]);
            rwl[i] = *reinterpret_cast<const half8*>(Wlo + w_src[i]);
        }
    }
    half8 wfa[NJ][2], wfb[NJ][2];
    const half8* const wfr = reinterpret_cast<const half8*>(Whi) + (size_t)((n0 + wn) / 32) * (K / 16) * 128 + lane;
    auto load_wf = [&](int s_, half8 (&wf)[NJ][2]) {
#pragma unroll
        for (int j = 0; j < NJ; ++j) {
            const size_t base = ((size_t)j * (K / 16) + s_) * 128;
            wf[j][0] = wfr[base];
            wf[j][1] = wfr[base + 64];
        }
    };
    if constexpr (WR) load_wf(0, wfa);

    f32x16 acc[MI][NJ];
#pragma unroll
    for (int i = 0; i < MI; ++i)
#pragma unroll
        for (int j = 0; j < NJ; ++j)
#pragma unroll
            for (int r = 0; r < 16; ++r) acc[i][j][r] = 0.f;

    const int nk = K / HK;
    const int fa = (wm + (lane & 31)) * HLD + (lane >> 5) * 8;
    const int fb = (wn + (lane & 31)) * HLD + (lane >> 5) * 8;
    auto stage_a = [&](int boff = 0) {
#pragma unroll
        for (int i = 0; i < NA; ++i) {
            if (G16_ABL & 2) {
                *reinterpret_cast<float2*>(Ahi + boff + a_off[i]) = make_float2(ra[i].x, ra[i].y);
                *reinterpret_cast<float2*>(Alo + boff + a_off[i]) = make_float2(ra[i].z, ra[i].w);
                continue;
            }
            const float sx = ra[i].x * a_rs[i], sy = ra[i].y * a_rs[i], sz = ra[i].z * a_rs[i], sw = ra[i].w * a_rs[i];
            half4 h, l;
            h[0] = (_Float16)sx; h[1] = (_Float16)sy; h[2] = (_Float16)sz; h[3] = (_Float16)sw;
            l[0] = (_Float16)(sx - (float)h[0]); l[1] = (_Float16)(sy - (float)h[1]);
            l[2] = (_Float16)(sz - (float)h[2]); l[3] = (_Float16)(sw - (float)h[3]);
            *reinterpret_cast<half4*>(Ahi + boff + a_off[i]) = h;
            *reinterpret_cast<half4*>(Alo + boff + a_off[i]) = l;
        }
    };
    auto request_a = [&](int kt1) {
        const int k1 = kt1 * HK;
        const char* ab = ((ep.K1 > 0 && k1 >= ep.K1) ? A2b : A1b) + (size_t)k1 * 4;
#pragma unroll
        for (int i = 0; i < NA; ++i) ra[i] = *reinterpret_cast<const float4*>(ab + ((G16_ABL & 4) ? (a_goff[i] & 127u) : a_goff[i]));
    };
    if constexpr (WR) {
        auto kstep = [&](int boff, int ks, const half8 (&cur)[NJ][2]) {
            if (G16_ABL & 8) { asm volatile("" :: "v"(cur[0][0]), "v"(cur[0][1]), "v"(cur[NJ - 1][0]), "v"(cur[NJ - 1][1])); return; }
#pragma unroll
            for (int i = 0; i < MI; ++i) {
                const half8 ah = *reinterpret_cast<const half8*>(Ahi + boff + fa + i * 32 * HLD + ks * 16);
                const half8 al = *reinterpret_cast<const half8*>(Alo + boff + fa + i * 32 * HLD + ks * 16);
#pragma unroll
                for (int j = 0; j < NJ; ++j) {
                    acc[i][j] = __builtin_amdgcn_mfma_f32_32x32x16_f16(al, cur[j][0], acc[i][j], 0, 0, 0);
                    acc[i][j] = __builtin_amdgcn_mfma_f32_32x32x16_f16(ah, cur[j][1], acc[i][j], 0, 0, 0);
                    acc[i][j] = __builtin_amdgcn_mfma_f32_32x32x16_f16(ah, cur[j][0], acc[i][j], 0, 0, 0);
                }
            }
        };
        {
            constexpr int BUF = 2 * TM * HLD;
            float4 rb[NA];
            auto request_b = [&](int kt1) {
                const int k1 = kt1 * HK;
                const char* ab = ((ep.K1 > 0 && k1 >= ep.K1) ? A2b : A1b) + (size_t)k1 * 4;
#pragma unroll
                for (int i = 0; i < NA; ++i) rb[i] = *reinterpret_cast<const float4*>(ab + ((G16_ABL & 4) ? (a_goff[i] & 127u) : a_goff[i]));
            };
            auto stage_from = [&](const float4 (&src)[NA], int boff) {
#pragma unroll
                for (int i = 0; i < NA; ++i) {
                    if (G16_ABL & 2) {
                        *reinterpret_cast<float2*>(Ahi + boff + a_off[i]) = make_float2(src[i].x, src[i].y);
                        *reinterpret_cast<float2*>(Alo + boff + a_off[i]) = make_float2(src[i].z, src[i].w);
// ... 113 lines not shown
#pragma unroll
            for (int jj = 0; jj < NJ / 2; ++jj) {
                const int cb = n0 + wn + 64 * jj;
                const float bv0 = (bias && cb + q < N) ? bias[cb + q] : 0.f;
                const float bv1 = (bias && cb + 32 + q < N) ? bias[cb + 32 + q] : 0.f;
#pragma unroll
                for (int i = 0; i < MI; ++i) {
#pragma unroll
                    for (int r = 0; r < 16; ++r) {
                        const int lr = (r & 3) + 8 * (r >> 2) + 4 * (lane >> 5);
                        const float sc = isc * rinv[wm + 32 * i + lr];
                        float v0 = acc[i][2 * jj][r] * sc + bv0, v1 = acc[i][2 * jj + 1][r] * sc + bv1;
                        if (ACT) { v0 = ssilu16(v0); v1 = ssilu16(v1); }
                        T[lr * TLD2 + q] = v0;
                        T[lr * TLD2 + 32 + q] = v1;
                    }
                    __builtin_amdgcn_fence(__ATOMIC_RELEASE, "wavefront");
                    __builtin_amdgcn_wave_barrier();
#pragma unroll
                    for (int it = 0; it < 8; ++it) {
                        const int item = lane + 64 * it;
                        const int lr = item >> 4, c4 = item & 15;
                        const int row = m0 + wm + 32 * i + lr, col = cb + 4 * c4;
                        float4 v = *reinterpret_cast<const float4*>(T + lr * TLD2 + 4 * c4);
                        if (row < M && col < N) {
                            if (ep.gate) {
                                const float4 g4 = *reinterpret_cast<const float4*>(ep.gate + (size_t)(row / 3) * ep.gate_ld + col);
                                v.x = g4.x * v.x; v.y = g4.y * v.y; v.z = g4.z * v.z; v.w = g4.w * v.w;
                            }
                            if (ep.accumulate) {
                                const float4 o = *reinterpret_cast<const float4*>(C + (size_t)row * ldc + col);
                                v.x += o.x; v.y += o.y; v.z += o.z; v.w += o.w;
                            }
                            *reinterpret_cast<float4*>(C + (size_t)row * ldc + col) = v;
                        }
                        if (ep.out_mag) {
                            float mg = col < N ? fmaxf(fmaxf(fabsf(v.x), fabsf(v.y)), fmaxf(fabsf(v.z), fabsf(v.w))) : 0.f;
                            mg = adf_row16_max(mg);
                            if (c4 == 0 && row < M) atomicMax(ep.out_mag + row, __float_as_uint(mg));
                        }
                    }
                    __builtin_amdgcn_wave_barrier();
                }
            }
            return;
        }
#pragma unroll
        for (int j = 0; j < NJ; ++j) {
            const int col = n0 + wn + 32 * j + (lane & 31);
            if (col >= N) continue;
            const float bv = bias ? bias[col] : 0.f;
#pragma unroll
            for (int i = 0; i < MI; ++i) {
#pragma unroll
                for (int r = 0; r < 16; ++r) {
                    const int row = m0 + wm + 32 * i + (r & 3) + 8 * (r >> 2) + 4 * (lane >> 5);
                    if (row < M) {
                        float v = acc[i][j][r] * (isc * rinv[row - m0]) + bv;
                        if (ACT) v = ssilu16(v);
                        if (ep.accumulate) v += C[(size_t)row * ldc + col];
                        C[(size_t)row * ldc + col] = v;
                        if (ep.out_mag) atomicMax(ep.out_mag + row, __float_as_uint(fabsf(v)));
                    }
                }
            }
        }
    } else if constexpr (EPI == 3) {
        static_assert(EPI != 3 || (NJ == 2 && MI == 3), "vec_proj epilogue: 3 components x (v1, v2)");
        const int q = lane & 31;
        const int g = (n0 + wn) / 64;
        const int H = ep.H;
        const float inv_sqrt_h = 1.0f / sqrtf((float)H);
        __syncthreads();
        float* T = reinterpret_cast<float*>(lds) + wave * 3200;
        const int a0 = m0 + (wave / NWN) * 32;
        float dv[16], nv[16];
#pragma unroll
        for (int r = 0; r < 16; ++r) {
            const int lr = (r & 3) + 8 * (r >> 2) + 4 * (lane >> 5);
            float d = 0.f, qq = 0.f;
#pragma unroll
            for (int i = 0; i < 3; ++i) {
                const float sc = isc * rinv[wm + 32 * i + lr];
                const float v1 = acc[i][0][r] * sc, v2 = acc[i][1][r] * sc;
                d += v1 * v2;
                qq += v2 * v2;
                T[lr * TLD3 + i * 32 + q] = v1;
            }
            dv[r] = d * inv_sqrt_h;
            nv[r] = sqrtf(qq + 1e-8f);
        }
        __builtin_amdgcn_fence(__ATOMIC_RELEASE, "wavefront");
        __builtin_amdgcn_wave_barrier();
#pragma unroll
        for (int it = 0; it < 4; ++it) {
            const int item = lane + 64 * it;
            const int lr = item >> 3, c4 = item & 7;
            const int n = a0 + lr;
            if (n < M) {
                float* vo = ep.v1 + (size_t)n * 3 * H + 32 * g + 4 * c4;
#pragma unroll
                for (int ax = 0; ax < 3; ++ax) {
                    const float4 tv_ = *reinterpret_cast<const float4*>(T + lr * TLD3 + ax * 32 + 4 * c4);
                    if (G16_ABL & 1) asm volatile("" :: "v"(tv_.x), "v"(tv_.w)); else
                    *reinterpret_cast<float4*>(vo + ax * H) = tv_;
                }
            }
        }
        __builtin_amdgcn_wave_barrier();
#pragma unroll
        for (int r = 0; r < 16; ++r) {
            const int lr = (r & 3) + 8 * (r >> 2) + 4 * (lane >> 5);
            T[lr * TLD3 + q] = dv[r];
            T[lr * TLD3 + 32 + q] = nv[r];
        }
        __builtin_amdgcn_fence(__ATOMIC_RELEASE, "wavefront");
        __builtin_amdgcn_wave_barrier();
#pragma unroll
        for (int it = 0; it < 4; ++it) {
            const int lr = it * 8 + (lane >> 3), c4 = lane & 7;
            const int n = a0 + lr, c = 32 * g + 4 * c4;
            const float4 dv_ = *reinterpret_cast<const float4*>(T + lr * TLD3 + 4 * c4);
            const float4 nv_ = *reinterpret_cast<const float4*>(T + lr * TLD3 + 32 + 4 * c4);
            if (n < M) {
                if (G16_ABL & 1) { asm volatile("" :: "v"(dv_.x), "v"(nv_.w)); } else {
                *reinterpret_cast<float4*>(ep.dotw + (size_t)n * H + c) = dv_;
                *reinterpret_cast<float4*>(ep.cat + (size_t)n * H + c) = nv_;
                }
            }
            if (ep.catpart) {
                const float mg = adf_lane8_max(fmaxf(fmaxf(fmaxf(0.f, fabsf(nv_.x)), fabsf(nv_.y)), fmaxf(fabsf(nv_.z), fabsf(nv_.w))));
                if (c4 == 0 && n < M) ep.catpart[(size_t)g * ep.part_stride + n] = mg;
            }
        }
    } else if constexpr (EPI == 4) {
        static_assert(EPI != 4 || (NJ == 2 && MI == 3), "norm epilogue: 3 components x 64 columns per wave");
        const int q = lane & 31;
        const int cb = n0 + wn;
        __syncthreads();
        float* T = reinterpret_cast<float*>(lds) + wave * 3200;
        const int a0 = m0 + (wave / NWN) * 32;
#pragma unroll
        for (int r = 0; r < 16; ++r) {
            const int lr = (r & 3) + 8 * (r >> 2) + 4 * (lane >> 5);
#pragma unroll
            for (int j = 0; j < 2; ++j) {
                const float a = acc[0][j][r] * (isc * rinv[wm + lr]), b = acc[1][j][r] * (isc * rinv[wm + 32 + lr]),
                            d = acc[2][j][r] * (isc * rinv[wm + 64 + lr]);
                T[lr * TLD2 + j * 32 + q] = sqrtf(a * a + b * b + d * d);
            }
        }
        __builtin_amdgcn_fence(__ATOMIC_RELEASE, "wavefront");
        __builtin_amdgcn_wave_barrier();
#pragma unroll
        for (int it = 0; it < 8; ++it) {
            const int lr = it * 4 + (lane >> 4), c4 = lane & 15;
            const int n = a0 + lr, c = cb + 4 * c4;
            if (n < M && c < N)
                *reinterpret_cast<float4*>(ep.cat + (size_t)n * N + c) = *reinterpret_cast<const float4*>(T + lr * TLD2 + 4 * c4);
        }
    } else {
        static_assert(EPI >= 3 || (NJ == 3 && MI == 2), "fused epilogues are written for the 64 x 96 wave tile");
        if (((EPI_ABL & 1) && EPI == 1) || ((EPI_ABL & 2) && EPI == 2)) {
            float sacc = 0.f;
            for (int i = 0; i < MI; ++i) for (int j = 0; j < NJ; ++j) for (int r = 0; r < 16; ++r) sacc += acc[i][j][r];
            if (ep.H < 0) ep.x[0] = sacc;
            return;
        }
        const int q = lane & 31;
        const int g = (n0 + wn) / 96;
        const int H = ep.H;
        const float b0 = bias[n0 + wn + q], b1 = bias[n0 + wn + 32 + q], b2 = bias[n0 + wn + 64 + q];
        __syncthreads();
        float* T = reinterpret_cast<float*>(lds) + wave * 3200;
#pragma unroll
        for (int i = 0; i < MI; ++i) {
#pragma unroll
            for (int r = 0; r < 16; ++r) {
                const int lr = (r & 3) + 8 * (r >> 2) + 4 * (lane >> 5);
                const float sc = isc * rinv[wm + 32 * i + lr];
                T[lr * TLD3 + q] = acc[i][0][r] * sc + b0;
                T[lr * TLD3 + 32 + q] = acc[i][1][r] * sc + b1;
                T[lr * TLD3 + 64 + q] = acc[i][2][r] * sc + b2;
            }
            __builtin_amdgcn_fence(__ATOMIC_RELEASE, "wavefront");
            __builtin_amdgcn_wave_barrier();
            const int c4 = lane & 7;
            const int c = 32 * g + 4 * c4;
            if constexpr (EPI == 1) {
                float4 v0[4], v1[4], v2[4];
                if (EPI_ABL & 4) { for (int it = 0; it < 4; ++it) { v0[it] = make_float4(1.f, 2.f, 3.f, 4.f); v1[it] = v0[it]; v2[it] = v0[it]; } }
                else if (!ep.vec_is_zero) {
#pragma unroll
                    for (int it = 0; it < 4; ++it) {
                        const int n = min(m0 + wm + 32 * i + it * 8 + (lane >> 3), M - 1);
                        const float* vr = ep.vec_in + (size_t)n * 3 * H + c;
                        v0[it] = *reinterpret_cast<const float4*>(vr);
                        v1[it] = *reinterpret_cast<const float4*>(vr + H);
                        v2[it] = *reinterpret_cast<const float4*>(vr + 2 * H);
                    }
                }
#pragma unroll
                for (int it = 0; it < 4; ++it) {
                    const int lr = it * 8 + (lane >> 3);
                    const int n = m0 + wm + 32 * i + lr;
                    const float4 p0 = *reinterpret_cast<const float4*>(T + lr * TLD3 + 4 * c4);
                    const float4 p1 = *reinterpret_cast<const float4*>(T + lr * TLD3 + 32 + 4 * c4);
                    const float4 p2 = *reinterpret_cast<const float4*>(T + lr * TLD3 + 64 + 4 * c4);
                    if ((EPI_ABL & 8) && n >= 0) { if (ep.H < 0) ep.rec[0] = p0.x + p1.x + p2.x + v0[it].x + v1[it].y + v2[it].z; }
                    else if (n < M) {
                        float* rec = ep.rec + ((size_t)(ep.row_map ? ep.row_map[n] : n) * (H / 32) + g) * 160;
                        float4* ra_ = reinterpret_cast<float4*>(rec + 16 * c4);
                        if (!ep.vec_is_zero) {
                            ra_[0] = make_float4(v0[it].x * p1.x, v1[it].x * p1.x, v2[it].x * p1.x, p0.x);
                            ra_[1] = make_float4(v0[it].y * p1.y, v1[it].y * p1.y, v2[it].y * p1.y, p0.y);
                            ra_[2] = make_float4(v0[it].z * p1.z, v1[it].z * p1.z, v2[it].z * p1.z, p0.z);
                            ra_[3] = make_float4(v0[it].w * p1.w, v1[it].w * p1.w, v2[it].w * p1.w, p0.w);
                        } else {
                            ra_[0] = make_float4(0.f, 0.f, 0.f, p0.x);
                            ra_[1] = make_float4(0.f, 0.f, 0.f, p0.y);
                            ra_[2] = make_float4(0.f, 0.f, 0.f, p0.z);
                            ra_[3] = make_float4(0.f, 0.f, 0.f, p0.w);
                        }
                        *reinterpret_cast<float4*>(rec + 128 + 4 * c4) = p2;
                    }
                }
            } else {
                float4 d[4], xv[4], w1[4][3], tv[4][3];
#pragma unroll
                for (int it = 0; it < 4; ++it) {
                    const int n = min(m0 + wm + 32 * i + it * 8 + (lane >> 3), M - 1);
                    const size_t xo = (size_t)n * H + c;
#if EPI2_POLICY & 2
                    typedef float f32x4_t __attribute__((ext_vector_type(4)));
                    auto ntld = [](const float* p_) { const f32x4_t v = __builtin_nontemporal_load(reinterpret_cast<const f32x4_t*>(p_));
                                                      return make_float4(v.x, v.y, v.z, v.w); };
#define EPI2_LD(p_) ntld(p_)
#else
#define EPI2_LD(p_) (*reinterpret_cast<const float4*>(p_))
#endif
                    d[it] = EPI2_LD(ep.dot + xo);
                    xv[it] = EPI2_LD(ep.x + xo);
                    const float* vr = ep.vec + (size_t)n * 3 * H + c;
                    const float* v1p = ep.vv + (size_t)n * 3 * H + c;
#pragma unroll
                    for (int ax = 0; ax < 3; ++ax) {
                        w1[it][ax] = EPI2_LD(v1p + ax * H);
                        tv[it][ax] = EPI2_LD(vr + ax * H);
                    }
                }
#pragma unroll
                for (int it = 0; it < 4; ++it) {
                    const int lr = it * 8 + (lane >> 3);
                    const int n = m0 + wm + 32 * i + lr;
                    const float4 p0 = *reinterpret_cast<const float4*>(T + lr * TLD3 + 4 * c4);
                    const float4 p1 = *reinterpret_cast<const float4*>(T + lr * TLD3 + 32 + 4 * c4);
                    const float4 p2 = *reinterpret_cast<const float4*>(T + lr * TLD3 + 64 + 4 * c4);
                    const float k2 = 0.70710678118654752f, sc = ep.scale;
                    float4 xo4 = xv[it];
                    xo4.x = (xo4.x + (p0.x + p1.x * d[it].x) * k2) * sc;
                    xo4.y = (xo4.y + (p0.y + p1.y * d[it].y) * k2) * sc;
                    xo4.z = (xo4.z + (p0.z + p1.z * d[it].z) * k2) * sc;
                    xo4.w = (xo4.w + (p0.w + p1.w * d[it].w) * k2) * sc;
#undef EPI2_LD
#if EPI2_POLICY & 1
                    typedef unsigned int u32x4 __attribute__((ext_vector_type(4)));
                    const auto rx = __builtin_amdgcn_make_buffer_rsrc(ep.x, 0, (int)((unsigned int)M * (unsigned int)H * 4u), 0x00020000);
                    const auto rv = __builtin_amdgcn_make_buffer_rsrc(ep.vec, 0, (int)((unsigned int)M * 3u * (unsigned int)H * 4u), 0x00020000);
#define EPI2_ST(r_, p_, base_, v_) __builtin_amdgcn_raw_buffer_store_b128(__builtin_bit_cast(u32x4, v_), r_, (int)(((p_) - (base_)) * 4), 0, 16)
#else
#define EPI2_ST(r_, p_, base_, v_) (*reinterpret_cast<float4*>(p_) = (v_))
#endif
                    if (n < M) {
                        EPI2_ST(rx, ep.x + (size_t)n * H + c, ep.x, xo4);
                        float* vr = ep.vec + (size_t)n * 3 * H + c;
#pragma unroll
                        for (int ax = 0; ax < 3; ++ax) {
                            float4 t = tv[it][ax];
                            const float4 v1 = w1[it][ax];
                            t.x += p2.x * v1.x; t.y += p2.y * v1.y; t.z += p2.z * v1.z; t.w += p2.w * v1.w;
                            EPI2_ST(rv, vr + ax * H, ep.vec, t);
                        }
                    }
#undef EPI2_ST
                }
            }
            __builtin_amdgcn_wave_barrier();
        }
    }
}

__global__ __launch_bounds__(256) void adf_rowmag_kernel(const float* __restrict__ A, int lda, int K1,
                                                         const float* __restrict__ A2, int K2, long long M,
                                                         float* __restrict__ mag, const int32_t* __restrict__ m_dev,
                                                         int m_mul) {
    const long long r = (long long)blockIdx.x * 4 + (threadIdx.x >> 6);
    const int lane = threadIdx.x & 63;
    if (r >= M || (m_dev && r >= (long long)*m_dev * m_mul)) return;
    float mx = 0.f;
    const float* a = A + (size_t)r * lda;
    for (int k = lane * 4; k < K1; k += 256) {
        const float4 v = *reinterpret_cast<const float4*>(a + k);
        mx = fmaxf(fmaxf(fmaxf(mx, fabsf(v.x)), fabsf(v.y)), fmaxf(fabsf(v.z), fabsf(v.w)));
    }
    if (A2) {
        const float* b = A2 + (size_t)r * lda;
        for (int k = lane * 4; k < K2; k += 256) {
            const float4 v = *reinterpret_cast<const float4*>(b + k);
            mx = fmaxf(fmaxf(fmaxf(mx, fabsf(v.x)), fabsf(v.y)), fmaxf(fabsf(v.z), fabsf(v.w)));
        }
    }
#pragma unroll
    for (int o = 32; o > 0; o >>= 1) mx = fmaxf(mx, __shfl_xor(mx, o));
    if (lane == 0) mag[r] = mx;
}

__global__ __launch_bounds__(256) void adf_rowmax_combine_kernel(const float* __restrict__ part, long long stride, int nparts,
                                                                 long long M, float* __restrict__ mag,
                                                                 const int32_t* __restrict__ m_dev, int m_mul) {
    const long long r = (long long)blockIdx.x * 256 + threadIdx.x;
    if (r >= M || (m_dev && r >= (long long)*m_dev * m_mul)) return;
    float mx = 0.f;
    for (int p = 0; p < nparts; ++p) mx = fmaxf(mx, part[(size_t)p * stride + r]);
    mag[r] = mx;
}

int32_t adf_launch_rowmax_combine(const float* part, long long stride, int nparts, long long M, float* mag, hipStream_t s,
                                  const int32_t* m_dev, int m_mul) {
    if (M <= 0) return ADF_OK;
    hipLaunchKernelGGL(adf_rowmax_combine_kernel, dim3((unsigned)((M + 255) / 256)), dim3(256), 0, s, part, stride, nparts, M,
                       mag, m_dev, m_mul);
    ADF_HIP_CHECK(hipGetLastError());
    return ADF_OK;
}

int32_t adf_launch_rowmag(const float* A, int lda, int K1, const float* A2, int K2, long long M, float* mag, hipStream_t s,
                          const int32_t* m_dev, int m_mul) {
    if (M <= 0) return ADF_OK;
    hipLaunchKernelGGL(adf_rowmag_kernel, dim3((unsigned)((M + 3) / 4)), dim3(256), 0, s, A, lda, K1, A2, K2, M, mag, m_dev,
                       m_mul);
    ADF_HIP_CHECK(hipGetLastError());
    return ADF_OK;
}

static int32_t lift_mags(const float* A, int lda, int K1, const float* A2, int K2, long long rows, const adf_lift* lf,
                         const float* premag, const float** out, hipStream_t s, const int32_t* m_dev = nullptr, int m_mul = 1) {
    *out = premag;
    if (!premag && lf && lf->buf) {
        if (rows > lf->cap) { adf_set_error("gemm16: lift scratch holds %lld rows, need %lld", lf->cap, rows); return ADF_EINVAL; }
        ADF_TRY(adf_launch_rowmag(A, lda, K1, A2, K2, rows, lf->buf, s, m_dev, m_mul));
        *out = lf->buf;
    }
    return ADF_OK;
}

__global__ void adf_absmax_kernel(const float* __restrict__ w, long long n, unsigned int* out_bits) {
    float m = 0.f;
    for (long long i = (long long)blockIdx.x * blockDim.x + threadIdx.x; i < n; i += (long long)gridDim.x * blockDim.x)
        m = fmaxf(m, fabsf(w[i]));
#pragma unroll
    for (int o = 32; o > 0; o >>= 1) m = fmaxf(m, __shfl_xor(m, o));
    if ((threadIdx.x & 63) == 0) atomicMax(out_bits, __float_as_uint(m));
}

__global__ void adf_split_kernel(const float* __restrict__ w, long long n, const unsigned int* absmax_bits,
                                 _Float16* __restrict__ hi, _Float16* __restrict__ lo, float* inv_scale, int perm_H,
                                 int K, const float* __restrict__ bias, float* __restrict__ bias_perm, int parts) {
    const float amax = __uint_as_float(*absmax_bits);
    int e = 0;
    if (amax > 0.f) (void)frexpf(amax, &e);
    const float scale = ldexpf(1.0f, 10 - e);
    if (blockIdx.x == 0 && threadIdx.x == 0) *inv_scale = 1.0f / scale;
    for (long long i = (long long)blockIdx.x * blockDim.x + threadIdx.x; i < n; i += (long long)gridDim.x * blockDim.x) {
        long long src = i;
        if (perm_H > 0) {
            const long long prow = i / K;
            const int k = (int)(i - prow * K);
            const int gw = 32 * parts;
            const int g = (int)(prow / gw), part = (int)((prow % gw) / 32), qq = (int)(prow % 32);
            const long long orow = (long long)part * perm_H + 32 * g + qq;
            src = orow * K + k;
            if (k == 0 && bias_perm) bias_perm[prow] = bias ? bias[orow] : 0.f;
        }
        const float v = w[src] * scale;
        const _Float16 h = (_Float16)v;
        hi[i] = h;
        lo[i] = (_Float16)(v - (float)h);
    }
}

int32_t adf_split_weight(const float* w, long long n, adf_w16* out, unsigned int* scratch_bits, hipStream_t s,
                         int perm_H, int K, const float* bias, int parts) {
    ADF_HIP_CHECK(hipMemsetAsync(scratch_bits, 0, sizeof(unsigned int), s));
    hipLaunchKernelGGL(adf_absmax_kernel, dim3(64), dim3(256), 0, s, w, n, scratch_bits);
    hipLaunchKernelGGL(adf_split_kernel, dim3(64), dim3(256), 0, s, w, n, scratch_bits, (_Float16*)out->hi,
                       (_Float16*)out->lo, out->inv_scale, perm_H, K, bias, out->bias_perm, parts);
    ADF_HIP_CHECK(hipGetLastError());
    return ADF_OK;
}

static int32_t check_a_span(long long rows, int lda) {
    if (rows * (long long)lda * 4 >= (1ll << 32)) {
        adf_set_error("gemm16: A operand of %lld rows x %d exceeds the 32-bit offset range, split the batch", rows, lda);
        return ADF_EOOM;
    }
    return ADF_OK;
}

int32_t adf_launch_gemm16(const float* A, int lda, const adf_w16* W, const float* bias, float* C, int ldc, int M,
                          int N, int K, int act_ssilu, hipStream_t s, const float* A2, int K1, const adf_lift* lf,
                          const float* premag, float* out_mag, const int32_t* m_dev, int accumulate, const float* gate,
                          int gate_ld) {
    if (M <= 0) return ADF_OK;
    if (K % HK != 0 || (lda & 3) || (A2 && (K1 <= 0 || K1 % HK != 0 || K1 >= K))) {
        adf_set_error("gemm16: K=%d (K1=%d) must be multiples of %d and lda a multiple of 4", K, K1, HK);
        return ADF_EINVAL;
    }
    ADF_TRY(check_a_span(M, lda));
    static int mi = 0;
    if (!mi) { const char* e = getenv("ADF_GEMM16_MI"); mi = e ? atoi(e) : 2; if (mi != 4) mi = 2; }
    const int TM = 64 * mi, TN = 256;
    const int tiles_n = (N + TN - 1) / TN;
    const int tiles_m = (M + TM - 1) / TM;
    const int tiles_m8 = (tiles_m + 7) / 8 * 8;
    dim3 grid((unsigned)(tiles_m8 * tiles_n));
    adf_epi ep = {};
    ep.A2 = A2; ep.K1 = A2 ? K1 : 0; ep.m_dev = m_dev; ep.accumulate = accumulate;
    ep.gate = gate; ep.gate_ld = gate_ld;
    if (gate && ((N | ldc) & 3)) { adf_set_error("gemm16: the gate epilogue needs N and ldc multiples of 4"); return ADF_EINVAL; }
    ADF_TRY(lift_mags(A, lda, A2 ? K1 : K, A2, A2 ? K - K1 : 0, M, lf, premag, &ep.rmag, s, m_dev, 1));
    if (out_mag) {
        ADF_HIP_CHECK(hipMemsetAsync(out_mag, 0, sizeof(float) * (size_t)M, s));
        ep.out_mag = reinterpret_cast<unsigned int*>(out_mag);
    }
    static int w8 = -1;
    if (w8 < 0) { const char* e = getenv("ADF_GEMM_W8_PLAIN"); w8 = (e && atoi(e) == 0) ? 0 : 1; }
    static int ncu = 0;
    if (!ncu) { int dev = 0; if (hipGetDevice(&dev) != hipSuccess || hipDeviceGetAttribute(&ncu, hipDeviceAttributeMultiprocessorCount, dev) != hipSuccess || ncu <= 0) ncu = 256; }
    const long long wg8 = (long long)((M + 191) / 192) * (N / 256 > 0 ? N / 256 : 1);
    const bool ragged = wg8 < 4ll * ncu && wg8 % ncu != 0 && wg8 % ncu < (3 * ncu) / 10 && wg8 > ncu;
    if (w8 == 1 && W->frag && N % 256 == 0 && (K / HK) % 2 == 0 && mi == 2 && !ragged) {
        const int tn8 = N / 256, tmw8 = ((M + 191) / 192 + 7) / 8 * 8;
        dim3 g8((unsigned)(tmw8 * tn8));
        if (act_ssilu)
            hipLaunchKernelGGL((adf_gemm_f16x3_kernel<1, 3, 2, 0, true, 4>), g8, dim3(512), 0, s, A, lda, (const _Float16*)W->frag,
                               (const _Float16*)nullptr, W->inv_scale, bias, C, ldc, M, N, K, tn8, ep);
        else
            hipLaunchKernelGGL((adf_gemm_f16x3_kernel<0, 3, 2, 0, true, 4>), g8, dim3(512), 0, s, A, lda, (const _Float16*)W->frag,
                               (const _Float16*)nullptr, W->inv_scale, bias, C, ldc, M, N, K, tn8, ep);
        ADF_HIP_CHECK(hipGetLastError());
        return ADF_OK;
    }
#define LAUNCH16(ACT_, MI_)                                                                                  \
    hipLaunchKernelGGL((adf_gemm_f16x3_kernel<ACT_, MI_, 4, 0>), grid, dim3(256), 0, s, A, lda,              \
                       (const _Float16*)W->hi, (const _Float16*)W->lo, W->inv_scale, bias, C, ldc, M, N, K, \
                       tiles_n, ep)
    if (mi == 4) { if (act_ssilu) LAUNCH16(1, 4); else LAUNCH16(0, 4); }
    else { if (act_ssilu) LAUNCH16(1, 2); else LAUNCH16(0, 2); }
#undef LAUNCH16
    ADF_HIP_CHECK(hipGetLastError());
    return ADF_OK;
}

int32_t adf_launch_gemm16_vecnorm(const float* A, int lda, const adf_w16* W, float* nrm, int M, int N, int K,
                                  hipStream_t s, const adf_lift* lf, const float* premag) {
    if (M <= 0) return ADF_OK;
    if (K % HK != 0 || (lda & 3) || (N & 3)) { adf_set_error("gemm16_vecnorm: bad shape"); return ADF_EINVAL; }
    ADF_TRY(check_a_span(3ll * M, lda));
    adf_epi ep = {};
    ep.cat = nrm;
    ADF_TRY(lift_mags(A, lda, K, nullptr, 0, 3ll * M, lf, premag, &ep.rmag, s));
    const int tn = (N + 127) / 128, tm8 = ((M + 63) / 64 + 7) / 8 * 8;
    static int w8 = -1;
    if (w8 < 0) { const char* e = getenv("ADF_GEMM_W8"); w8 = (e && atoi(e) == 0) ? 0 : 1; }
    if (w8 && W->frag && N % 256 == 0 && (K / HK) % 2 == 0) {
        hipLaunchKernelGGL((adf_gemm_f16x3_kernel<0, 3, 2, 4, true, 4>), dim3((unsigned)(tm8 * (N / 256))), dim3(512), 0, s, A, lda,
                           (const _Float16*)W->frag, (const _Float16*)nullptr, W->inv_scale, (const float*)nullptr,
                           (float*)nullptr, 0, M, N, K, N / 256, ep);
        ADF_HIP_CHECK(hipGetLastError());
        return ADF_OK;
    }
    hipLaunchKernelGGL((adf_gemm_f16x3_kernel<0, 3, 2, 4>), dim3((unsigned)(tm8 * tn)), dim3(256), 0, s, A, lda,
                       (const _Float16*)W->hi, (const _Float16*)W->lo, W->inv_scale, (const float*)nullptr,
                       (float*)nullptr, 0, M, N, K, tn, ep);
    ADF_HIP_CHECK(hipGetLastError());
    return ADF_OK;
}

int32_t adf_launch_gemm16_fused(const float* A, int lda, const adf_w16* W, int M, int H, int K, int epi,
                                const adf_epi* ep_in, hipStream_t s, const adf_lift* lf) {
    adf_epi epv = *ep_in;
    const adf_epi* ep = &epv;
    if (M <= 0) return ADF_OK;
    if (K % HK != 0 || (lda & 3) || H % 64 != 0 || (epi != 3 && !W->bias_perm)) {
        adf_set_error("gemm16_fused: bad shape");
        return ADF_EINVAL;
    }
    ADF_TRY(check_a_span(epi == 3 ? 3ll * M : (long long)M, lda));
    ADF_TRY(lift_mags(A, lda, K, nullptr, 0, epi == 3 ? 3ll * M : (long long)M, lf, ep_in->rmag, &epv.rmag, s, ep_in->m_dev,
                      epi == 3 ? 3 : 1));
    const int N = 3 * H, TM = 128, TN = 192;
    const int tiles_n = N / TN;
    const int tiles_m = (M + TM - 1) / TM;
    const int tiles_m8 = (tiles_m + 7) / 8 * 8;
    dim3 grid((unsigned)(tiles_m8 * tiles_n));
    if (epi == 3) {
        const int tn = 2 * H / 128, tm8 = ((M + 63) / 64 + 7) / 8 * 8;
        static int wreg = -1;
        if (wreg < 0) { const char* e = getenv("ADF_GEMM_WREG"); wreg = (e && atoi(e) == 0) ? 0 : 1; }
        static int w8 = -1;
        if (w8 < 0) { const char* e = getenv("ADF_GEMM_W8"); w8 = (e && atoi(e) == 0) ? 0 : 1; }
        if (wreg && W->frag && w8 == 1 && (2 * H) % 256 == 0 && (K / HK) % 2 == 0)
            hipLaunchKernelGGL((adf_gemm_f16x3_kernel<0, 3, 2, 3, true, 4>), dim3((unsigned)(tm8 * (2 * H / 256))), dim3(512), 0, s,
                               A, lda, (const _Float16*)W->frag, (const _Float16*)nullptr, W->inv_scale, (const float*)nullptr,
                               (float*)nullptr, 0, M, 2 * H, K, 2 * H / 256, *ep);
        else
        hipLaunchKernelGGL((adf_gemm_f16x3_kernel<0, 3, 2, 3>), dim3((unsigned)(tm8 * tn)), dim3(256), 0, s, A, lda,
                           (const _Float16*)W->hi, (const _Float16*)W->lo, W->inv_scale, (const float*)nullptr,
                           (float*)nullptr, 0, M, 2 * H, K, tn, *ep);
        ADF_HIP_CHECK(hipGetLastError());
        return ADF_OK;
    }
    static int wf = -1;
    if (wf < 0) { const char* e = getenv("ADF_GEMM_WR_FUSED"); wf = e ? atoi(e) : 2; }
    if (wf && W->frag && (K / HK) % 2 == 0 && (wf == 2 || N % 384 == 0)) {
        const int tnw = wf == 4 ? N / 384 : tiles_n;
        dim3 gw((unsigned)(tiles_m8 * tnw));
#define LAUNCHWF(EPI_, NWN_)                                                                                                  \
        hipLaunchKernelGGL((adf_gemm_f16x3_kernel<0, 2, 3, EPI_, true, NWN_>), gw, dim3(128 * NWN_), 0, s, A, lda,            \
                           (const _Float16*)W->frag, (const _Float16*)nullptr, W->inv_scale, W->bias_perm, (float*)nullptr, 0, \
                           M, N, K, tnw, *ep)
        if (epi == 1) { if (wf == 4) LAUNCHWF(1, 4); else LAUNCHWF(1, 2); }
        else { if (wf == 4) LAUNCHWF(2, 4); else LAUNCHWF(2, 2); }
#undef LAUNCHWF
        ADF_HIP_CHECK(hipGetLastError());
        return ADF_OK;
    }
    if (epi == 1)
        hipLaunchKernelGGL((adf_gemm_f16x3_kernel<0, 2, 3, 1>), grid, dim3(256), 0, s, A, lda, (const _Float16*)W->hi,
                           (const _Float16*)W->lo, W->inv_scale, W->bias_perm, (float*)nullptr, 0, M, N, K, tiles_n, *ep);
    else
        hipLaunchKernelGGL((adf_gemm_f16x3_kernel<0, 2, 3, 2>), grid, dim3(256), 0, s, A, lda, (const _Float16*)W->hi,
                           (const _Float16*)W->lo, W->inv_scale, W->bias_perm, (float*)nullptr, 0, M, N, K, tiles_n, *ep);
    ADF_HIP_CHECK(hipGetLastError());
    return ADF_OK;
}
```

### adsorbdiff_amd/csrc/message.hip

```cpp
#include <stdlib.h>
#include <string.h>

#include "message.h"

#ifndef MSG_ABL
#define MSG_ABL 0
#endif
#ifndef MSG_SKIP
#define MSG_SKIP 1
#endif
#ifndef MSG_EXP_NOXC
#define MSG_EXP_NOXC 0
#endif

__device__ __forceinline__ float wave_min(float v) {
#pragma unroll
    for (int o = 32; o > 0; o >>= 1) v = fminf(v, __shfl_xor(v, o));
    return v;
}
__device__ __forceinline__ float wave_max(float v) {
#pragma unroll
    for (int o = 32; o > 0; o >>= 1) v = fmaxf(v, __shfl_xor(v, o));
    return v;
}

#ifndef FWD_WAVES
#define FWD_WAVES 8
#endif
#ifndef FWD_AHEAD
#define FWD_AHEAD 4
#endif
#define FWD_THREADS (64 * FWD_WAVES)
#define MSG_WAVES_PER_SIMD (FWD_WAVES / 4)
template <bool F16, bool VZ, bool UNI>
__global__ __launch_bounds__(FWD_THREADS, MSG_WAVES_PER_SIMD) void adf_message_kernel(MsgParams p) {
    extern __shared__ __attribute__((aligned(16))) float lds[];
    const int wfloats = F16 ? (2 * MSG_COLS * MSG_LDK) / 2 : p.R * MSG_COLS;
    float* Wl = lds;
    _Float16* Wh = reinterpret_cast<_Float16*>(lds);
    _Float16* Wlo = Wh + MSG_COLS * MSG_LDK;
    float* Bl = lds + wfloats;
    float* Mu = Bl + MSG_COLS;
    float* Meta = Mu + 144;
    int* Ctr = reinterpret_cast<int*>(Meta + FWD_WAVES * 32 * 8);

    const int tid = threadIdx.x;
    const int lane = tid & 63;
    const int wave = tid >> 6;
    const int q = lane & 31;
    const int hi = lane >> 5;
    const int slice = blockIdx.x % p.nslices;
    const int worker = blockIdx.x / p.nslices;
    const int nworkers = gridDim.x / p.nslices;
    const int items = p.items_dev ? min(p.items, (int)*p.items_dev) : p.items;
    const int ngroups = (items + ADF_GROUP_NODES - 1) / ADF_GROUP_NODES;
    if (worker >= ngroups) return;
    const int H = p.H;
    const int c0 = slice * ADF_SLICE_CH;

    {
        if (F16) {
            const int R8 = p.R / 8;
            const half8* src = reinterpret_cast<const half8*>(p.wpack16 + (size_t)slice * 2 * MSG_COLS * p.R);
            const half8 zero8 = {0, 0, 0, 0, 0, 0, 0, 0};
            const _Float16* b16 = reinterpret_cast<const _Float16*>(p.bpack) + (size_t)slice * MSG_COLS * 2;
            for (int i = tid; i < 2 * MSG_COLS * 17; i += FWD_THREADS) {
                const int row = i / 17, piece = i - row * 17;
                half8 v = piece < R8 ? src[row * R8 + piece] : zero8;
                if (piece == 16 && row < MSG_COLS) { v[0] = b16[2 * row]; v[1] = b16[2 * row + 1]; }
                *reinterpret_cast<half8*>(Wh + (size_t)row * MSG_LDK + piece * 8) = v;
            }
        } else {
            const float4* src = reinterpret_cast<const float4*>(p.wpack + (size_t)slice * p.R * MSG_COLS);
            float4* dst = reinterpret_cast<float4*>(Wl);
            const int n4 = p.R * MSG_COLS / 4;
            for (int i = tid; i < n4; i += FWD_THREADS) dst[i] = src[i];
        }
        if (!F16 && tid < MSG_COLS) Bl[tid] = p.bpack[slice * MSG_COLS + tid];
        if (tid < 144) Mu[tid] = (tid < p.R ? p.mu[tid] : 2.0f) * (F16 ? p.sarg : 1.0f);
        if (tid == 0) *Ctr = 0;
    }
    __syncthreads();
    float* meta_w = Meta + wave * 32 * 8;
    const float inv_sqrt3 = 0.57735026918962576f;
    const float inv_sqrt2 = 0.70710678118654752f;
    const float out_scale = F16 ? *p.inv_scale * (1.0f / 256.0f) : 1.0f;
    const float inv_sqrt_h = out_scale / sqrtf((float)H);
    const float umax_scale = (float)(p.R - 1);
    const float coeff2 = p.coeff * 1.44269504088896341f;
    const unsigned int row_bytes = (unsigned int)p.nslices * 1280u;
    const char* recS = reinterpret_cast<const char*>(p.rec) + (size_t)slice * 1280;
    const unsigned int qA = (unsigned int)q * 16u;
    const unsigned int qP = 512u + (unsigned int)q * 4u;

    unsigned int ksteps = 0;

    typedef const __attribute__((address_space(4))) int32_t* cint_ptr;
    const cint_ptr nptr_c = (cint_ptr)p.nptr;
    const cint_ptr tlist_c = (cint_ptr)p.tlist;
    auto fetch_target = [&](int& n_out, int& o_out) -> bool {
        while (true) {
            int t = 0;
            if (lane == 0) t = atomicAdd(Ctr, 1);
            t = __builtin_amdgcn_readfirstlane(t);
            const int g = worker + (t >> 5) * nworkers;
            if (g >= ngroups) return false;
            const int e = g * ADF_GROUP_NODES + (t & 31);
            if (e < items) { o_out = e; n_out = p.tlist ? tlist_c[e] : e; return true; }
        }
    };
    auto load_block = [&](int eb, int e1, float4& geo, int& src, bool& valid) {
        const int e = eb + q;
        valid = e < e1;
        geo = make_float4(0.f, 0.f, 0.f, 0.f);
        src = 0;
        if (valid) { geo = p.e_geom[e]; src = p.e_src[e]; }
    };

    int n = 0, orow = 0, eb = 0, e1 = 0;
    bool have = fetch_target(n, orow);
    if (have) { eb = nptr_c[n]; e1 = nptr_c[n + 1]; }
    int nN = 0, oN = 0, e0N = 0, e1N = 0;
    bool haveN = have && fetch_target(nN, oN);
    if (haveN) { e0N = nptr_c[nN]; e1N = nptr_c[nN + 1]; }
    float4 geo = make_float4(0.f, 0.f, 0.f, 0.f); int src = 0; bool valid = false;
    if (have) load_block(eb, e1, geo, src, valid);
    asm volatile("" : "+v"(geo.x), "+v"(geo.y), "+v"(geo.z), "+v"(geo.w), "+v"(src));
    bool first = true;
    float sx0 = 0.f, sx1 = 0.f, sa0 = 0.f, sa1 = 0.f, sb0 = 0.f, sb1 = 0.f, sc0 = 0.f, sc1 = 0.f;
    float ra0 = 0.f, ra1 = 0.f, rb0 = 0.f, rb1 = 0.f, rc0 = 0.f, rc1 = 0.f;
    float res0 = 0.f, res1 = 0.f, res2 = 0.f, res3 = 0.f;

    while (have) {
        {
            const bool last = eb + 32 >= e1;
            float4 geoN = make_float4(0.f, 0.f, 0.f, 0.f); int srcN = 0; bool validN = false;
            if (!last) load_block(eb + 32, e1, geoN, srcN, validN);
            else if (haveN) load_block(e0N, e1N, geoN, srcN, validN);
            if (first) {
                const size_t xo = (size_t)n * H + c0 + q;
                const size_t vo = (size_t)n * 3 * H + c0 + q;
                if (hi == 0) {
                    res0 = p.x[xo]; res1 = p.x[xo + 32];
                    if (!VZ) { res2 = p.vec[vo]; res3 = p.vec[vo + 32]; }
                } else if (!VZ) {
                    res0 = p.vec[vo + H]; res1 = p.vec[vo + H + 32];
                    res2 = p.vec[vo + 2 * H]; res3 = p.vec[vo + 2 * H + 32];
                }
            }

            const float xs = geo.w * p.inv_cutoff;
            float xp = xs;
            if (p.env_pi == 5) { const float x2 = xs * xs; xp = x2 * x2 * xs; }
            else for (int i = 1; i < p.env_pi; ++i) xp *= xs;
            float env = 1.0f + p.env_a * xp + p.env_b * (xp * xs) + p.env_c * (xp * xs * xs);
            env = (xs < 1.0f && valid) ? env : 0.0f;
            __builtin_amdgcn_wave_barrier();
            if (hi == 0) {
                float* m = meta_w + q * 8;
                m[0] = __uint_as_float((unsigned int)(valid ? src : p.N) * row_bytes);
                m[1] = geo.x; m[2] = geo.y; m[3] = geo.z;
            }
            __builtin_amdgcn_fence(__ATOMIC_RELEASE, "wavefront");
            __builtin_amdgcn_wave_barrier();
            const float u = xs * umax_scale;
            const int nvalid = __builtin_amdgcn_readfirstlane(min(32, e1 - eb));
            const float umin = __int_as_float(__builtin_amdgcn_readlane(__float_as_int(u), 0));
            const float umax = __int_as_float(__builtin_amdgcn_readlane(__float_as_int(u), max(nvalid, 1) - 1));
            int klo, khi;
            if (nvalid <= 0) {
                klo = 0; khi = 16;
            } else if (F16) {
                klo = max(0, (int)floorf(umin) - 5) & ~7;
                khi = min(p.R, (int)ceilf(umax) + 6);
                khi = klo + ((khi - klo + 15) & ~15);
                if (khi > 128) { klo -= khi - 128; khi = 128; }
            } else {
                klo = max(0, (int)floorf(umin) - 7) & ~1;
                khi = min(p.R, ((int)ceilf(umax) + 8 + 1) & ~1);
            }
            klo = __builtin_amdgcn_readfirstlane(klo);
            khi = __builtin_amdgcn_readfirstlane(khi);
            ksteps += (khi - klo) * (VZ && F16 ? 4 : 6);

#define ROW_OF(r) ((r & 3) + 8 * (r >> 2) + 4 * hi)
#define DECL(r)                                                                                 \
    const float* m##r = meta_w + ROW_OF(r) * 8;                                                 \
    float4 ga0##r, ga1##r;                                      \
    float gz0##r, gz1##r;
#define GATHER(r)                                                                               \
    {                                                                                           \
    const unsigned int o##r = __float_as_uint(m##r[0]);                                         \
    if (MSG_EXP_NOXC) { gz0##r = 1.0f; gz1##r = 2.0f; } else {                                 \
    gz0##r = *reinterpret_cast<const float*>(recS + (size_t)(o##r + qP));                       \
    gz1##r = *reinterpret_cast<const float*>(recS + (size_t)(o##r + qP) + 640); }               \
    if (MSG_EXP_NOXC == 2) { ga0##r = make_float4(1.f, 2.f, 3.f, 4.f); ga1##r = ga0##r; }      \
    else if (!VZ) {                                                                             \
        ga0##r = *reinterpret_cast<const float4*>(recS + (size_t)(o##r + qA));                  \
        ga1##r = *reinterpret_cast<const float4*>(recS + (size_t)(o##r + qA) + 640);            \
    } else {                                                                                    \
        ga0##r = make_float4(0.f, 0.f, 0.f, *reinterpret_cast<const float*>(recS + (size_t)(o##r + qA) + 12)); \
        ga1##r = make_float4(0.f, 0.f, 0.f, *reinterpret_cast<const float*>(recS + (size_t)(o##r + qA) + 652)); \
    }                                                                                           \
    }
#define CONSUME(r)                                                                              \
    {                                                                                           \
        const float ux = m##r[1], uy = m##r[2], uz = m##r[3];                                   \
        const float t3 = gz0##r * acc[4][r];                                                    \
        sx0 += ga0##r.w * acc[0][r];                                                            \
        if (!VZ) { sa0 += ga0##r.x * acc[2][r]; sb0 += ga0##r.y * acc[2][r]; sc0 += ga0##r.z * acc[2][r]; } \
        ra0 += t3 * ux; rb0 += t3 * uy; rc0 += t3 * uz;                                         \
        const float u3 = gz1##r * acc[5][r];                                                    \
        sx1 += ga1##r.w * acc[1][r];                                                            \
        if (!VZ) { sa1 += ga1##r.x * acc[3][r]; sb1 += ga1##r.y * acc[3][r]; sc1 += ga1##r.z * acc[3][r]; } \
        ra1 += u3 * ux; rb1 += u3 * uy; rc1 += u3 * uz;                                         \
    }
            DECL(0) DECL(1) DECL(2) DECL(3) DECL(4) DECL(5) DECL(6) DECL(7)
            DECL(8) DECL(9) DECL(10) DECL(11) DECL(12) DECL(13) DECL(14) DECL(15)
            GATHER(0) GATHER(1)
#if FWD_AHEAD == 4
            GATHER(2) GATHER(3)
#endif

            const float env256 = env * 256.0f;
            f32x16 acc[6];
            if (F16) {
                half8 aone = {0, 0, 0, 0, 0, 0, 0, 0};
                if (hi == 0) { aone[0] = (_Float16)256.0f; aone[1] = (_Float16)256.0f; }
                const f32x16 zero16 = {0.f, 0.f, 0.f, 0.f, 0.f, 0.f, 0.f, 0.f, 0.f, 0.f, 0.f, 0.f, 0.f, 0.f, 0.f, 0.f};
// ... 121 lines not shown
                    CONSUME(12) CONSUME(13) CONSUME(14) CONSUME(15)
                }
            }
#else
            GATHER(4) GATHER(5) GATHER(6) GATHER(7)
            CONSUME(0) CONSUME(1) CONSUME(2) CONSUME(3)
            GATHER(8) GATHER(9) GATHER(10) GATHER(11)
            CONSUME(4) CONSUME(5) CONSUME(6) CONSUME(7)
            GATHER(12) GATHER(13) GATHER(14) GATHER(15)
            CONSUME(8) CONSUME(9) CONSUME(10) CONSUME(11)
            CONSUME(12) CONSUME(13) CONSUME(14) CONSUME(15)
#endif
#undef GATHER
#undef DECL
#undef CONSUME
#undef ROW_OF
            if (last) {
                sx0 *= out_scale; sx1 *= out_scale;
                sa0 = (sa0 * inv_sqrt3 + ra0) * inv_sqrt_h; sa1 = (sa1 * inv_sqrt3 + ra1) * inv_sqrt_h;
                sb0 = (sb0 * inv_sqrt3 + rb0) * inv_sqrt_h; sb1 = (sb1 * inv_sqrt3 + rb1) * inv_sqrt_h;
                sc0 = (sc0 * inv_sqrt3 + rc0) * inv_sqrt_h; sc1 = (sc1 * inv_sqrt3 + rc1) * inv_sqrt_h;
                sx0 += __shfl_xor(sx0, 32); sx1 += __shfl_xor(sx1, 32);
                sa0 += __shfl_xor(sa0, 32); sa1 += __shfl_xor(sa1, 32);
                sb0 += __shfl_xor(sb0, 32); sb1 += __shfl_xor(sb1, 32);
                sc0 += __shfl_xor(sc0, 32); sc1 += __shfl_xor(sc1, 32);
                const size_t xo = (size_t)orow * H + c0 + q;
                const size_t vo = (size_t)orow * 3 * H + c0 + q;
                float o0, o1, o2, o3;
                if (hi == 0) {
                    o0 = (res0 + sx0) * inv_sqrt2; o1 = (res1 + sx1) * inv_sqrt2;
                    o2 = res2 + sa0; o3 = res3 + sa1;
                    p.x_out[xo] = o0;
                    p.x_out[xo + 32] = o1;
                    p.vec_out[vo] = o2;
                    p.vec_out[vo + 32] = o3;
                } else {
                    o0 = res0 + sb0; o1 = res1 + sb1;
                    o2 = res2 + sc0; o3 = res3 + sc1;
                    p.vec_out[vo + H] = o0;
                    p.vec_out[vo + H + 32] = o1;
                    p.vec_out[vo + 2 * H] = o2;
                    p.vec_out[vo + 2 * H + 32] = o3;
                }
                if (p.xpart) {
                    const float mA = adf_half32_max_hi(fmaxf(fmaxf(0.f, fabsf(o0)), fabsf(o1)));
                    const float mB = adf_half32_max_hi(fmaxf(fmaxf(0.f, fabsf(o2)), fabsf(o3)));
                    if (q == 16) {
                        float* vp = p.vpart + (size_t)slice * 3 * p.part_stride + (size_t)orow * 3;
                        if (hi == 0) { p.xpart[(size_t)slice * p.part_stride + orow] = mA; vp[0] = mB; }
                        else { vp[1] = mA; vp[2] = mB; }
                    }
                }
                sx0 = sx1 = sa0 = sa1 = sb0 = sb1 = sc0 = sc1 = 0.f;
                ra0 = ra1 = rb0 = rb1 = rc0 = rc1 = 0.f;
                res0 = res1 = res2 = res3 = 0.f;
                have = haveN;
                n = nN; orow = oN; eb = e0N; e1 = e1N;
                first = true;
                if (have) {
                    haveN = fetch_target(nN, oN);
                    if (haveN) { e0N = nptr_c[nN]; e1N = nptr_c[nN + 1]; }
                }
            } else {
                eb += 32;
                first = false;
            }
            geo = geoN; src = srcN; valid = validN;
        }
    }
    if (p.kcount && lane == 0) atomicAdd(p.kcount, (unsigned long long)ksteps);
}

__global__ void adf_pack_rbf_kernel(const float* __restrict__ w, const float* __restrict__ b, float* wpack,
                                    float* bpack, int H, int R) {
    const int nslices = H / ADF_SLICE_CH;
    const int total = nslices * R * MSG_COLS;
    for (int i = blockIdx.x * blockDim.x + threadIdx.x; i < total; i += gridDim.x * blockDim.x) {
        const int col = i % MSG_COLS;
        const int k = (i / MSG_COLS) % R;
        const int slice = i / (MSG_COLS * R);
        const int part = col / 64, j = (col >> 5) & 1, qq = col & 31;
        const int ch = slice * ADF_SLICE_CH + 32 * j + qq;
        wpack[i] = w[(size_t)(part * H + ch) * R + k];
        if (k == 0) bpack[slice * MSG_COLS + col] = b[part * H + ch];
    }
}

__global__ void adf_pack_rbf16_kernel(const float* __restrict__ w, const float* __restrict__ b,
                                      const unsigned int* absmax_bits, _Float16* wpack16, float* bpack16,
                                      float* inv_scale, int H, int R) {
    const float amax = __uint_as_float(*absmax_bits);
    int e = 0;
    if (amax > 0.f) (void)frexpf(amax, &e);
    const float scale = ldexpf(1.0f, 10 - e);
    if (blockIdx.x == 0 && threadIdx.x == 0) *inv_scale = 1.0f / scale;
    const int nslices = H / ADF_SLICE_CH;
    const int total = nslices * MSG_COLS * R;
    for (int i = blockIdx.x * blockDim.x + threadIdx.x; i < total; i += gridDim.x * blockDim.x) {
        const int k = i % R;
        const int col = (i / R) % MSG_COLS;
        const int slice = i / (R * MSG_COLS);
        const int part = col / 64, j = (col >> 5) & 1, qq = col & 31;
        const int ch = slice * ADF_SLICE_CH + 32 * j + qq;
        const float v = w[(size_t)(part * H + ch) * R + k] * scale;
        const _Float16 h = (_Float16)v;
        const size_t base = (size_t)slice * 2 * MSG_COLS * R;
        wpack16[base + (size_t)col * R + k] = h;
        wpack16[base + (size_t)(MSG_COLS + col) * R + k] = (_Float16)(v - (float)h);
        if (k == 0) {
            const float bv = b[part * H + ch] * scale;
            const _Float16 bh = (_Float16)bv;
            _Float16* o = reinterpret_cast<_Float16*>(bpack16 + slice * MSG_COLS + col);
            o[0] = bh; o[1] = (_Float16)(bv - (float)bh);
        }
    }
}

__global__ void adf_absmax_kernel(const float* __restrict__ w, long long n, unsigned int* out_bits);

__global__ void adf_pack_records_kernel(const float* __restrict__ xh, const float* __restrict__ vec,
                                        float* __restrict__ rec, int N, int H, int vec_is_zero) {
    const int ng = H / 32;
    const long long total = (long long)N * ng * 32;
    for (long long t = (long long)blockIdx.x * blockDim.x + threadIdx.x; t < total;
         t += (long long)gridDim.x * blockDim.x) {
        const int qq = (int)(t & 31);
        const int g = (int)((t >> 5) % ng);
        const long long n = t / (32LL * ng);
        const int c = 32 * g + qq;
        const float* xr = xh + (size_t)n * 3 * H;
        const float xa = xr[c], xb = xr[H + c], xc = xr[2 * H + c];
        float* out = rec + ((size_t)n * ng + g) * 160;
        if (!vec_is_zero) {
            const float* vr = vec + (size_t)n * 3 * H;
            reinterpret_cast<float4*>(out)[qq] = make_float4(vr[c] * xb, vr[H + c] * xb, vr[2 * H + c] * xb, xa);
        } else {
            reinterpret_cast<float4*>(out)[qq] = make_float4(0.f, 0.f, 0.f, xa);
        }
        out[128 + qq] = xc;
    }
}

int32_t adf_pack_records(adf_painn* h, int N, const float* xh, const float* vec, bool vec_is_zero, hipStream_t s,
                         float* rec) {
    const int H = h->hp.hidden_channels;
    long long blocks = ((long long)N * H + 255) / 256;
    if (blocks > 256 * 16) blocks = 256 * 16;
    hipLaunchKernelGGL(adf_pack_records_kernel, dim3((unsigned)blocks), dim3(256), 0, s, xh, vec, rec ? rec : h->rec, N, H,
                       vec_is_zero ? 1 : 0);
    ADF_HIP_CHECK(hipGetLastError());
    return ADF_OK;
}

static size_t msg_lds_bytes(int R, bool f16) {
    const size_t w = f16 ? (size_t)2 * MSG_COLS * MSG_LDK * 2 : sizeof(float) * (size_t)R * MSG_COLS;
    return w + sizeof(float) * (MSG_COLS + 144 + FWD_WAVES * 32 * 8) + 16;
}

int32_t adf_pack_rbf_layer(adf_painn* h, int l, hipStream_t s) {
    const int H = h->hp.hidden_channels, R = h->hp.num_rbf;
    const size_t per_layer = (size_t)(H / ADF_SLICE_CH) * R * MSG_COLS;
    const size_t per_layer_b = (size_t)(H / ADF_SLICE_CH) * MSG_COLS;
    hipLaunchKernelGGL(adf_pack_rbf_kernel, dim3(256), dim3(256), 0, s, h->layer[l].rbf_w, h->layer[l].rbf_b,
                       h->rbf_pack + l * per_layer, h->rbf_bias_pack + l * per_layer_b, H, R);
    ADF_HIP_CHECK(hipMemsetAsync(h->w16_scratch, 0, sizeof(unsigned int), s));
    hipLaunchKernelGGL(adf_absmax_kernel, dim3(64), dim3(256), 0, s, h->layer[l].rbf_w, (long long)3 * H * R,
                       h->w16_scratch);
    hipLaunchKernelGGL(adf_absmax_kernel, dim3(8), dim3(256), 0, s, h->layer[l].rbf_b, (long long)3 * H,
                       h->w16_scratch);
    hipLaunchKernelGGL(adf_pack_rbf16_kernel, dim3(256), dim3(256), 0, s, h->layer[l].rbf_w, h->layer[l].rbf_b,
                       h->w16_scratch, reinterpret_cast<_Float16*>(h->rbf_pack16) + l * 2 * per_layer,
                       h->rbf_bias_pack16 + l * per_layer_b, h->rbf_scales + l, H, R);
    ADF_HIP_CHECK(hipGetLastError());
    return ADF_OK;
}

int32_t adf_pack_rbf(adf_painn* h, hipStream_t s) {
    const int H = h->hp.hidden_channels, R = h->hp.num_rbf;
    {
        float mu[128];
        ADF_HIP_CHECK(hipMemcpyAsync(mu, h->rbf_offset, sizeof(float) * R, hipMemcpyDeviceToHost, s));
        ADF_HIP_CHECK(hipStreamSynchronize(s));
        bool uni = true;
        for (int k = 0; k < R; ++k) uni = uni && fabsf(mu[k] - (float)k / (float)(R - 1)) <= 2e-7f;
        const char* e = getenv("ADF_MSG_RBF");
        h->rbf_uniform = uni && !(e && strcmp(e, "direct") == 0);
    }
    for (int l = 0; l < h->hp.num_layers; ++l) ADF_TRY(adf_pack_rbf_layer(h, l, s));
    ADF_HIP_CHECK(hipGetLastError());
    {
#define SET_LDS(F16_, VZ_, UNI_)                                                                              \
    ADF_HIP_CHECK(hipFuncSetAttribute(reinterpret_cast<const void*>(adf_message_kernel<F16_, VZ_, UNI_>),     \
                                      hipFuncAttributeMaxDynamicSharedMemorySize, (int)msg_lds_bytes(128, F16_)))
        SET_LDS(false, false, false); SET_LDS(false, true, false); SET_LDS(true, false, false); SET_LDS(true, true, false);
        SET_LDS(true, false, true); SET_LDS(true, true, true);
#undef SET_LDS
    }
    return ADF_OK;
}

int32_t adf_message_impl(adf_painn* h, int layer, int N, const float* x, const float* xh, const float* vec,
                         float* x_out, float* vec_out, bool vec_is_zero, hipStream_t s, const int32_t* tlist,
                         int n_targets, const float* rec, const int32_t* n_targets_dev, float* xpart, float* vpart,
                         long long part_stride) {
    const int H = h->hp.hidden_channels, R = h->hp.num_rbf;
    if ((unsigned long long)(N + 1) * 5ull * H * sizeof(float) >= (1ull << 32)) {
        adf_set_error("message kernel uses 32-bit byte offsets into the node tables: N=%d is too large, split the batch", N);
        return ADF_EOOM;
    }
    MsgParams p;
    p.rec = rec ? rec : h->rec; p.vec = vec; p.x = x; p.x_out = x_out; p.vec_out = vec_out;
    p.nptr = h->nptr; p.e_src = h->e_src; p.e_geom = h->e_geom;
    p.nslices = H / ADF_SLICE_CH;
    const bool f16 = !h->msg_f32;
    p.wpack = h->rbf_pack + (size_t)layer * p.nslices * R * MSG_COLS;
    p.wpack16 = reinterpret_cast<const _Float16*>(h->rbf_pack16) + (size_t)layer * 2 * p.nslices * R * MSG_COLS;
    p.bpack = (f16 ? h->rbf_bias_pack16 : h->rbf_bias_pack) + (size_t)layer * p.nslices * MSG_COLS;
    p.inv_scale = h->rbf_scales + layer;
    p.mu = h->rbf_offset;
    p.N = N; p.H = H; p.R = R;
    p.tlist = tlist; p.items = tlist ? n_targets : N; p.items_dev = tlist ? n_targets_dev : nullptr;
    if (p.items <= 0) return ADF_OK;
    p.G = (p.items + ADF_GROUP_NODES - 1) / ADF_GROUP_NODES;
    p.inv_cutoff = 1.0f / h->hp.cutoff;
    const double step = 1.0 / (R - 1);
    p.coeff = (float)(-0.5 / (step * step));
    p.sarg = (float)sqrt(0.5 / (step * step) * 1.4426950408889634);
    const double pe = (double)h->hp.envelope_exponent;
    p.env_pi = h->hp.envelope_exponent;
    p.env_a = (float)(-(pe + 1) * (pe + 2) / 2);
    p.env_b = (float)(pe * (pe + 2));
    p.env_c = (float)(-pe * (pe + 1) / 2);
    p.kcount = h->prof_on ? h->kcount : nullptr;
    p.xpart = xpart; p.vpart = xpart ? vpart : nullptr; p.part_stride = part_stride;
    int workers = h->num_cus / p.nslices;
    if (workers < 1) workers = 1;
    if (workers > p.G) workers = p.G;
    dim3 grid((unsigned)(workers * p.nslices));
#define LAUNCH_MSG(F16_, VZ_, UNI_)                                                                        \
    hipLaunchKernelGGL((adf_message_kernel<F16_, VZ_, UNI_>), grid, dim3(FWD_THREADS), msg_lds_bytes(R, F16_), s, p)
    {
        const double d = sqrt(0.5 / (step * step) * 1.4426950408889634) * step;
        p.dmu2 = (float)(2.0 * d); p.dmusq = (float)(d * d); p.cstep = (float)exp2(-2.0 * d * d);
    }
    if (f16 && h->rbf_uniform) { if (vec_is_zero) LAUNCH_MSG(true, true, true); else LAUNCH_MSG(true, false, true); }
    else if (f16) { if (vec_is_zero) LAUNCH_MSG(true, true, false); else LAUNCH_MSG(true, false, false); }
    else { if (vec_is_zero) LAUNCH_MSG(false, true, false); else LAUNCH_MSG(false, false, false); }
#undef LAUNCH_MSG
    ADF_HIP_CHECK(hipGetLastError());
    return ADF_OK;
}
```

### adsorbdiff_amd/csrc/nodewise.hip

```cpp
#include "common.h"

__device__ __forceinline__ float ssilu_d(float x) {
    float s = x / (1.0f + expf(-x));
    return s * 1.6666666666666667f;
}

__global__ void adf_embed_kernel(const float* __restrict__ emb, const int32_t* __restrict__ Z, float* __restrict__ x,
                                 int N, int H, int num_elements, int32_t* flags) {
    const int h4 = H / 4;
    const long long total = (long long)N * h4;
    for (long long i = (long long)blockIdx.x * blockDim.x + threadIdx.x; i < total;
         i += (long long)gridDim.x * blockDim.x) {
        const int n = (int)(i / h4), c = (int)(i - (long long)n * h4);
        int z = Z[n] - 1;
        if (z < 0 || z >= num_elements) { if (c == 0) atomicExch(&flags[4], 1); z = min(max(z, 0), num_elements - 1); }
        const float4 v = reinterpret_cast<const float4*>(emb + (size_t)z * H)[c];
        reinterpret_cast<float4*>(x + (size_t)n * H)[c] = v;
    }
}

__global__ __launch_bounds__(256) void adf_layernorm_kernel(const float* __restrict__ x, const float* __restrict__ w,
                                                             const float* __restrict__ b, float* __restrict__ y,
                                                             int N, int H, float* __restrict__ out_mag,
                                                             const int32_t* __restrict__ n_dev) {
    const int lane = threadIdx.x & 63;
    const int row = blockIdx.x * 4 + (threadIdx.x >> 6);
    if (row >= N || (n_dev && row >= *n_dev)) return;
    const float4* xr = reinterpret_cast<const float4*>(x + (size_t)row * H);
    const int h4 = H / 4;
    float4 vals[4];
    float sum = 0.f;
#pragma unroll
    for (int i = 0; i < 4; ++i) {
        const int c = lane + 64 * i;
        vals[i] = c < h4 ? xr[c] : make_float4(0.f, 0.f, 0.f, 0.f);
        sum += (vals[i].x + vals[i].y) + (vals[i].z + vals[i].w);
    }
#pragma unroll
    for (int o = 32; o > 0; o >>= 1) sum += __shfl_xor(sum, o);
    const float mean = sum / (float)H;
    float sq = 0.f;
#pragma unroll
    for (int i = 0; i < 4; ++i)
        if (lane + 64 * i < h4) {
            const float dx = vals[i].x - mean, dy = vals[i].y - mean, dz = vals[i].z - mean, dw = vals[i].w - mean;
            sq += (dx * dx + dy * dy) + (dz * dz + dw * dw);
        }
#pragma unroll
    for (int o = 32; o > 0; o >>= 1) sq += __shfl_xor(sq, o);
    const float rstd = 1.0f / sqrtf(sq / (float)H + 1e-5f);
    float4* yr = reinterpret_cast<float4*>(y + (size_t)row * H);
    const float4* w4 = reinterpret_cast<const float4*>(w);
    const float4* b4 = reinterpret_cast<const float4*>(b);
    float mg = 0.f;
#pragma unroll
    for (int i = 0; i < 4; ++i) {
        const int c = lane + 64 * i;
        if (c < h4) {
            const float4 ww = w4[c], bb = b4[c];
            const float4 o = make_float4((vals[i].x - mean) * rstd * ww.x + bb.x, (vals[i].y - mean) * rstd * ww.y + bb.y,
                                         (vals[i].z - mean) * rstd * ww.z + bb.z, (vals[i].w - mean) * rstd * ww.w + bb.w);
            yr[c] = o;
            mg = fmaxf(fmaxf(fmaxf(mg, fabsf(o.x)), fabsf(o.y)), fmaxf(fabsf(o.z), fabsf(o.w)));
        }
    }
    if (out_mag) {
#pragma unroll
        for (int o = 32; o > 0; o >>= 1) mg = fmaxf(mg, __shfl_xor(mg, o));
        if (lane == 0) out_mag[row] = mg;
    }
}

__global__ void adf_update_prep_kernel(const float* __restrict__ vv, const float* __restrict__ x,
                                       float* __restrict__ cat, float* __restrict__ dot, int N, int H) {
    const int h4 = H / 4;
    const long long total = (long long)N * h4;
    const float inv_sqrt_h = 1.0f / sqrtf((float)H);
    for (long long i = (long long)blockIdx.x * blockDim.x + threadIdx.x; i < total;
         i += (long long)gridDim.x * blockDim.x) {
        const int n = (int)(i / h4), c = (int)(i - (long long)n * h4);
        const float4* base = reinterpret_cast<const float4*>(vv + (size_t)n * 6 * H);
        float4 d = make_float4(0.f, 0.f, 0.f, 0.f), q = d;
#pragma unroll
        for (int a = 0; a < 3; ++a) {
            const float4 v1 = base[a * 2 * h4 + c];
            const float4 v2 = base[a * 2 * h4 + h4 + c];
            d.x += v1.x * v2.x; d.y += v1.y * v2.y; d.z += v1.z * v2.z; d.w += v1.w * v2.w;
            q.x += v2.x * v2.x; q.y += v2.y * v2.y; q.z += v2.z * v2.z; q.w += v2.w * v2.w;
        }
        reinterpret_cast<float4*>(dot + (size_t)n * H)[c] =
            make_float4(d.x * inv_sqrt_h, d.y * inv_sqrt_h, d.z * inv_sqrt_h, d.w * inv_sqrt_h);
        float4* cr = reinterpret_cast<float4*>(cat + (size_t)n * 2 * H);
        cr[c] = reinterpret_cast<const float4*>(x + (size_t)n * H)[c];
        cr[h4 + c] = make_float4(sqrtf(q.x + 1e-8f), sqrtf(q.y + 1e-8f), sqrtf(q.z + 1e-8f), sqrtf(q.w + 1e-8f));
    }
}

__global__ void adf_update_apply_kernel(const float* __restrict__ h3, const float* __restrict__ dot,
                                        const float* __restrict__ vv, float* __restrict__ x, float* __restrict__ vec,
                                        float scale, int N, int H) {
    const int h4 = H / 4;
    const long long total = (long long)N * h4;
    const float inv_sqrt2 = 0.70710678118654752f;
    for (long long i = (long long)blockIdx.x * blockDim.x + threadIdx.x; i < total;
         i += (long long)gridDim.x * blockDim.x) {
        const int n = (int)(i / h4), c = (int)(i - (long long)n * h4);
        const float4* hr = reinterpret_cast<const float4*>(h3 + (size_t)n * 3 * H);
        const float4 a = hr[c], b = hr[h4 + c], g = hr[2 * h4 + c];
        const float4 d = reinterpret_cast<const float4*>(dot + (size_t)n * H)[c];
        float4* xr = reinterpret_cast<float4*>(x + (size_t)n * H) + c;
        float4 xv = *xr;
        xv.x = (xv.x + (a.x + b.x * d.x) * inv_sqrt2) * scale;
        xv.y = (xv.y + (a.y + b.y * d.y) * inv_sqrt2) * scale;
        xv.z = (xv.z + (a.z + b.z * d.z) * inv_sqrt2) * scale;
        xv.w = (xv.w + (a.w + b.w * d.w) * inv_sqrt2) * scale;
        *xr = xv;
        const float4* vb = reinterpret_cast<const float4*>(vv + (size_t)n * 6 * H);
        float4* vr = reinterpret_cast<float4*>(vec + (size_t)n * 3 * H);
#pragma unroll
        for (int ax = 0; ax < 3; ++ax) {
            const float4 v1 = vb[ax * 2 * h4 + c];
            float4 t = vr[ax * h4 + c];
            t.x += g.x * v1.x; t.y += g.y * v1.y; t.z += g.z * v1.z; t.w += g.w * v1.w;
            vr[ax * h4 + c] = t;
        }
    }
}

__global__ void adf_head_norm_cat_kernel(const float* __restrict__ xin, const float* __restrict__ t1,
                                         float* __restrict__ cat, int N, int C) {
    const int c4 = C / 4;
    const long long total = (long long)N * c4;
    for (long long i = (long long)blockIdx.x * blockDim.x + threadIdx.x; i < total;
         i += (long long)gridDim.x * blockDim.x) {
        const int n = (int)(i / c4), c = (int)(i - (long long)n * c4);
        const float4* tb = reinterpret_cast<const float4*>(t1 + (size_t)n * 3 * C);
        const float4 a = tb[c], b = tb[c4 + c], d = tb[2 * c4 + c];
        float4* cr = reinterpret_cast<float4*>(cat + (size_t)n * 2 * C);
        cr[c] = reinterpret_cast<const float4*>(xin + (size_t)n * C)[c];
        cr[c4 + c] = make_float4(sqrtf(a.x * a.x + b.x * b.x + d.x * d.x), sqrtf(a.y * a.y + b.y * b.y + d.y * d.y),
                                 sqrtf(a.z * a.z + b.z * b.z + d.z * d.z), sqrtf(a.w * a.w + b.w * b.w + d.w * d.w));
    }
}

__global__ void adf_head_gate_kernel(const float* __restrict__ o, const float* __restrict__ t2,
                                     float* __restrict__ xout, float* __restrict__ vout, int N, int Cout) {
    const int c4 = Cout / 4;
    const long long total = (long long)N * c4;
    for (long long i = (long long)blockIdx.x * blockDim.x + threadIdx.x; i < total;
         i += (long long)gridDim.x * blockDim.x) {
        const int n = (int)(i / c4), c = (int)(i - (long long)n * c4);
        const float4* orow = reinterpret_cast<const float4*>(o + (size_t)n * 2 * Cout);
        const float4 xs = orow[c], g = orow[c4 + c];
        reinterpret_cast<float4*>(xout + (size_t)n * Cout)[c] =
            make_float4(ssilu_d(xs.x), ssilu_d(xs.y), ssilu_d(xs.z), ssilu_d(xs.w));
        const float4* tb = reinterpret_cast<const float4*>(t2 + (size_t)n * 3 * Cout);
        float4* vb = reinterpret_cast<float4*>(vout + (size_t)n * 3 * Cout);
#pragma unroll
        for (int ax = 0; ax < 3; ++ax) {
            const float4 t = tb[ax * c4 + c];
            vb[ax * c4 + c] = make_float4(g.x * t.x, g.y * t.y, g.z * t.z, g.w * t.w);
        }
    }
}

__global__ void adf_head_xact_kernel(const float* __restrict__ o, float* __restrict__ xout, int N, int Cout) {
    const int c4 = Cout / 4;
    const long long total = (long long)N * c4;
    for (long long i = (long long)blockIdx.x * blockDim.x + threadIdx.x; i < total;
         i += (long long)gridDim.x * blockDim.x) {
        const int n = (int)(i / c4), c = (int)(i - (long long)n * c4);
        const float4 xs = reinterpret_cast<const float4*>(o + (size_t)n * 2 * Cout)[c];
        reinterpret_cast<float4*>(xout + (size_t)n * Cout)[c] =
            make_float4(ssilu_d(xs.x), ssilu_d(xs.y), ssilu_d(xs.z), ssilu_d(xs.w));
    }
}

__global__ __launch_bounds__(256) void adf_head_final_kernel(const float* __restrict__ u, const float* __restrict__ v,
                                                              const float* __restrict__ w_vec2,
                                                              const float* __restrict__ un2_w,
                                                              const float* __restrict__ un2_b, float* __restrict__ out,
                                                              int N, int C, int32_t* flags) {
    const int lane = threadIdx.x & 63;
    const int n = blockIdx.x * 4 + (threadIdx.x >> 6);
    if (n >= N) return;
    float g = 0.f, t0 = 0.f, t1 = 0.f, t2 = 0.f;
    for (int c = lane; c < C; c += 64) {
        const float w2 = w_vec2[c];
        g += u[(size_t)n * C + c] * un2_w[C + c];
        t0 += v[((size_t)n * 3 + 0) * C + c] * w2;
        t1 += v[((size_t)n * 3 + 1) * C + c] * w2;
        t2 += v[((size_t)n * 3 + 2) * C + c] * w2;
    }
#pragma unroll
    for (int o = 32; o > 0; o >>= 1) {
        g += __shfl_xor(g, o); t0 += __shfl_xor(t0, o); t1 += __shfl_xor(t1, o); t2 += __shfl_xor(t2, o);
    }
    if (lane == 0) {
        g += un2_b[1];
        out[(size_t)n * 3 + 0] = g * t0;
        out[(size_t)n * 3 + 1] = g * t1;
        out[(size_t)n * 3 + 2] = g * t2;
        const float s3 = g * t0 + g * t1 + g * t2;
        if (!(fabsf(s3) <= 3.0e38f)) atomicExch(&flags[5], 1);
    }
}

static inline unsigned ew_grid(long long total) {
    long long b = (total + 255) / 256;
    if (b > 256 * 8) b = 256 * 8;
    if (b < 1) b = 1;
    return (unsigned)b;
}

int32_t adf_nodewise_embed(adf_painn* h, const int32_t* Z, int N, float* x, hipStream_t s) {
    const int H = h->hp.hidden_channels;
    hipLaunchKernelGGL(adf_embed_kernel, dim3(ew_grid((long long)N * H / 4)), dim3(256), 0, s, h->emb, Z, x, N, H,
                       h->hp.num_elements, h->flags);
    ADF_HIP_CHECK(hipGetLastError());
    return ADF_OK;
}

int32_t adf_nodewise_layernorm(const float* x, const float* w, const float* b, float* y, int N, int H, hipStream_t s,
                               float* out_mag, const int32_t* n_dev) {
    hipLaunchKernelGGL(adf_layernorm_kernel, dim3((N + 3) / 4), dim3(256), 0, s, x, w, b, y, N, H, out_mag, n_dev);
    ADF_HIP_CHECK(hipGetLastError());
    return ADF_OK;
}

int32_t adf_nodewise_update_prep(const float* vv, const float* x, float* cat, float* dot, int N, int H, hipStream_t s) {
    hipLaunchKernelGGL(adf_update_prep_kernel, dim3(ew_grid((long long)N * H / 4)), dim3(256), 0, s, vv, x, cat, dot, N, H);
    ADF_HIP_CHECK(hipGetLastError());
    return ADF_OK;
}

int32_t adf_nodewise_update_apply(const float* h3, const float* dot, const float* vv, float* x, float* vec,
                                  float scale, int N, int H, hipStream_t s) {
    hipLaunchKernelGGL(adf_update_apply_kernel, dim3(ew_grid((long long)N * H / 4)), dim3(256), 0, s, h3, dot, vv, x,
                       vec, scale, N, H);
    ADF_HIP_CHECK(hipGetLastError());
    return ADF_OK;
}

int32_t adf_head_forward(adf_painn* h, int head, int N, const float* x, const float* vec, float* out, hipStream_t s) {
    const int H = h->hp.hidden_channels, H2 = H / 2;
    const adf_block_weights& b0 = h->head[head][0];
    const adf_block_weights& b1 = h->head[head][1];
    float* t1 = h->vv;
    float* t2 = h->vv + (size_t)3 * N * H;
    float* v1 = t2 + (size_t)3 * N * H2;
    float* o = h->xh;
    float* x1 = h->xh + (size_t)N * H;
    float* t1b = x1 + (size_t)N * H2;
    float* cat1 = h->dot;
    const bool lift = h->lift_on && !h->gemm_f32;
    const adf_lift* lf = lift ? &h->lift : nullptr;
    const float* vmag = nullptr;
    if (lift) {
        if (head == 0 || !h->mag_v3_valid) ADF_TRY(adf_launch_rowmag(vec, H, H, nullptr, 0, 3ll * N, h->mag_v3, s));
        h->mag_v3_valid = head == 0;
        vmag = h->mag_v3;
    }
    if (h->gemm_f32) {
        ADF_TRY(adf_linear(h, vec, H, b0.vec1_w, &b0.vec1_16, nullptr, t1, H, 3 * N, H, H, 0, s));
        hipLaunchKernelGGL(adf_head_norm_cat_kernel, dim3(ew_grid((long long)N * H / 4)), dim3(256), 0, s, x, t1, h->cat, N, H);
    } else {
        ADF_TRY(adf_launch_gemm16_vecnorm(vec, H, &b0.vec1_16, h->cat, N, H, H, s, lf, vmag));
    }
    static int fuse_gate = -1;
    if (fuse_gate < 0) { const char* e = getenv("ADF_HEAD_GATE_FUSED"); fuse_gate = (e && atoi(e) == 0) ? 0 : 1; }
    const bool fg = fuse_gate && !h->gemm_f32 && (H2 & 3) == 0;
    if (!fg) ADF_TRY(adf_linear(h, vec, H, b0.vec2_w, &b0.vec2_16, nullptr, t2, H2, 3 * N, H2, H, 0, s, vmag));
    if (h->gemm_f32) ADF_TRY(adf_linear(h, h->cat, 2 * H, b0.un0_w, &b0.un0_16, b0.un0_b, h->y, H, N, H, 2 * H, 1, s));
    else ADF_TRY(adf_launch_gemm16(x, H, &b0.un0_16, b0.un0_b, h->y, H, N, H, 2 * H, 1, s, h->cat, H,
                                   h->lift_on ? &h->lift : nullptr, nullptr, h->lift_on ? h->mag_b : nullptr));
    ADF_TRY(adf_linear(h, h->y, H, b0.un2_w, &b0.un2_16, b0.un2_b, o, H, N, H, H, 0, s, (h->lift_on && !h->gemm_f32) ? h->mag_b : nullptr));
    if (fg) {
        ADF_TRY(adf_launch_gemm16(vec, H, &b0.vec2_16, nullptr, v1, H2, 3 * N, H2, H, 0, s, nullptr, 0, lf, vmag,
                                  lift ? h->lift.buf : nullptr, nullptr, 0, o + H2, H));
        hipLaunchKernelGGL(adf_head_xact_kernel, dim3(ew_grid((long long)N * H2 / 4)), dim3(256), 0, s, o, x1, N, H2);
    } else
    hipLaunchKernelGGL(adf_head_gate_kernel, dim3(ew_grid((long long)N * H2 / 4)), dim3(256), 0, s, o, t2, x1, v1, N, H2);
    if (h->gemm_f32) {
        ADF_TRY(adf_linear(h, v1, H2, b1.vec1_w, &b1.vec1_16, nullptr, t1b, H2, 3 * N, H2, H2, 0, s));
        hipLaunchKernelGGL(adf_head_norm_cat_kernel, dim3(ew_grid((long long)N * H2 / 4)), dim3(256), 0, s, x1, t1b, cat1, N, H2);
        ADF_TRY(adf_linear(h, cat1, H, b1.un0_w, &b1.un0_16, b1.un0_b, h->y, H2, N, H2, H, 1, s));
    } else {
        ADF_TRY(adf_launch_gemm16_vecnorm(v1, H2, &b1.vec1_16, cat1, N, H2, H2, s, h->lift_on ? &h->lift : nullptr,
                                          (fg && lift) ? h->lift.buf : nullptr));
        ADF_TRY(adf_launch_gemm16(x1, H2, &b1.un0_16, b1.un0_b, h->y, H2, N, H2, H, 1, s, cat1, H2, h->lift_on ? &h->lift : nullptr));
    }
    hipLaunchKernelGGL(adf_head_final_kernel, dim3((N + 3) / 4), dim3(256), 0, s, h->y, v1, b1.vec2_w, b1.un2_w,
                       b1.un2_b, out, N, H2, h->flags);
    ADF_HIP_CHECK(hipGetLastError());
    return ADF_OK;
}
```

Before: 253.6.

## Emit head row maxima from last update epilogue and add 12-wave message variant

The last interaction layer's fused update epilogue now writes per-row absolute-max partials for x and vec. The force head then reuses these as precomputed magnitudes instead of running separate rowmag passes. The head's vecnorm GEMMs and the x-activation kernel also emit row maxima for the following lifted GEMMs, and the magnitudes are cached across incremental denoise steps. Separately, a 12-wave variant of the message kernel is added behind an env knob, defaulting to 8, which leaves the default path unchanged. In exchange there is more partial-buffer bookkeeping and extra combine launches.

After: 255.0, median of 6. Within noise of the previous version (+0.6%).

```diff
diff --git a/adsorbdiff_amd/csrc/api.hip b/adsorbdiff_amd/csrc/api.hip
--- a/adsorbdiff_amd/csrc/api.hip
+++ b/adsorbdiff_amd/csrc/api.hip
@@ -155,6 +155,8 @@
         h->lift_on = !(el && strcmp(el, "0") == 0);
         const char* e2 = getenv("ADF_MSG");
         h->msg_f32 = e2 ? strcmp(e2, "f32") == 0 : h->gemm_f32;
+        const char* ew = getenv("ADF_MSG_VZ_WAVES");
+        h->msg_vz_waves = (ew && atoi(ew) == 12) ? 12 : (ew && atoi(ew) == 8) ? 8 : ADF_MSG_VZ_WAVES_DEFAULT;
         const char* er = getenv("ADF_ROW_MAXIMA");
         h->rmx = (er && atoi(er) == 0) ? 0 : 1;
     }
@@ -173,9 +175,11 @@
         h->incX[l] = h->incV[l] = nullptr;
         if (l < ADF_MAX_LAYERS) h->incR[l] = nullptr;
     }
-    void* ptrs[] = {h->inc_c0, h->inc_chg, h->inc_pend, h->inc_need, h->inc_tf, h->inc_list, h->inc_cnt, h->inc_tmp};
+    void* ptrs[] = {h->inc_c0, h->inc_chg, h->inc_pend, h->inc_need, h->inc_tf, h->inc_list, h->inc_cnt, h->inc_tmp,
+                    h->inc_magX, h->inc_magV};
     for (void* p : ptrs)
         if (p) (void)hipFree(p);
+    h->inc_magX = h->inc_magV = nullptr; h->inc_mag_valid = false; h->hm_x = h->hm_vec = nullptr;
     h->inc_c0 = h->inc_chg = h->inc_pend = h->inc_need = h->inc_tf = nullptr;
     h->inc_list = h->inc_cnt = nullptr; h->inc_tmp = nullptr; h->inc_tmp_bytes = 0;
     h->inc_capN = 0; h->inc_valid = false;
@@ -184,7 +188,7 @@
 static void free_workspaces(adf_painn* h) {
     void* ptrs[] = {h->nbr_cnt, h->nbr_src, h->nbr_shift, h->deg, h->nptr, h->cursor, h->img_cnt, h->sys_slow, h->scan_tmp,
                     h->e_src, h->e_geom, h->x, h->vecA, h->vecB, h->y, h->xh, h->vv, h->cat, h->dot, h->sys, h->rec, h->lift.buf, h->mag_a, h->mag_b, h->mag_v3,
-                    h->rmx_part, h->cache_d2, h->cache_cid, h->cache_cnt, h->prev_nptr, h->prev_src, h->prev_geom};
+                    h->rmx_part, h->hmx_part, h->cache_d2, h->cache_cid, h->cache_cnt, h->prev_nptr, h->prev_src, h->prev_geom};
     for (void* p : ptrs)
         if (p) (void)hipFree(p);
     h->prev_nptr = h->prev_src = nullptr; h->prev_geom = nullptr; h->inc_valid = false;
@@ -195,6 +199,8 @@
     h->lift.buf = h->mag_a = h->mag_b = h->mag_v3 = nullptr; h->lift.cap = 0; h->mag_v3_valid = false;
     h->rmx_part = h->xpart = h->catpart = h->vpart = nullptr; h->part_stride = 0;
     h->part_x = h->part_vec = nullptr; h->dbg_msg_rows = h->dbg_cat_rows = h->dbg_comb_rows = 0; h->dbg_mag = nullptr;
+    h->hmx_part = h->hxpart = h->hvpart = h->npart0 = h->npart1 = h->x1mag = h->mag_xl = nullptr;
+    h->hm_x = h->hm_vec = nullptr; h->dbg_head_rows = 0; h->inc_mag_valid = false;
     h->cache_d2 = nullptr; h->cache_cid = nullptr; h->cache_cnt = nullptr; h->cache_valid = false;
     h->capN = h->capB = h->capE = 0;
 }
@@ -368,6 +374,8 @@
     ALLOC(mag_v3, capN * 3);
     const int64_t ps = (capN + 31) / 32 * 32, ns = H / ADF_SLICE_CH;
     if (h->rmx) ALLOC(rmx_part, (4 * ns + H / 32 + 4) * ps);
+    const int64_t ng = H / 32;
+    if (h->rmx) ALLOC(hmx_part, (4 * ng + H / 64 + H / 128 + 1 + 2) * ps);
 #undef ALLOC
     h->lift.cap = st == ADF_OK ? capN * 3 : 0;
     if (st != ADF_OK) { free_workspaces(h); return st; }
@@ -375,6 +383,8 @@
         h->part_stride = ps;
         h->xpart = h->rmx_part; h->catpart = h->xpart + ns * ps; h->vpart = h->catpart + (H / 32) * ps;
         h->dbg_mag = h->vpart + 3 * ns * ps;
+        h->hxpart = h->hmx_part; h->hvpart = h->hxpart + ng * ps; h->npart0 = h->hvpart + 3 * ng * ps;
+        h->npart1 = h->npart0 + (H / 64) * ps; h->x1mag = h->npart1 + (H / 128 + 1) * ps; h->mag_xl = h->x1mag + ps;
     }
     h->capN = capN; h->capB = capB; h->capE = capE;
     return ADF_OK;
@@ -551,7 +561,10 @@
     return st;
 }
 
-static int32_t update_layer(adf_painn* h, int l, int N, float* x, float* vec, hipStream_t s, bool from_message = true) {
+struct head_mag_dst { float* magx; float* magv; const int32_t* list; };
+static int32_t update_layer(adf_painn* h, int l, int N, float* x, float* vec, hipStream_t s, bool from_message = true,
+                            const head_mag_dst* hm = nullptr, bool* emitted = nullptr) {
+    if (emitted) *emitted = false;
     const int H = h->hp.hidden_channels;
     const adf_layer_weights& w = h->layer[l];
     adf_prof_begin(h, ADF_PROF_NODE, s);
@@ -608,7 +621,15 @@
         ep.x = x; ep.vec = vec; ep.dot = h->dot; ep.vv = h->vv; ep.scale = h->scale[l]; ep.H = H;
         ep.rmag = h->lift_on ? h->mag_b : nullptr;
         ep.m_dev = h->rows_dev;
+        const bool emit = hm && hm->magx && hm->magv && h->rmx && h->lift_on && h->hxpart && N > 0 && N <= h->part_stride;
+        if (emit) { ep.hxpart = h->hxpart; ep.hvpart = h->hvpart; ep.part_stride = h->part_stride; }
         st = adf_launch_gemm16_fused(h->y, H, &w.xv2_16, N, H, H, 2, &ep, s);
+        if (st == ADF_OK && emit) {
+            st = adf_launch_rowmax_combine(h->hxpart, h->part_stride, H / 32, N, hm->magx, s, h->rows_dev, 1, nullptr, hm->list);
+            if (st == ADF_OK)
+                st = adf_launch_rowmax_combine(h->hvpart, 3 * h->part_stride, H / 32, 3ll * N, hm->magv, s, h->rows_dev, 3, nullptr, hm->list);
+            if (st == ADF_OK && emitted) *emitted = true;
+        }
     }
     adf_prof_end(h, s);
     return st;
@@ -637,8 +658,23 @@
 
 extern "C" int32_t adf_painn_debug_row_maxima(adf_painn_t h, int32_t which, float* out, int64_t capacity, int32_t* rows,
                                               void* stream) {
-    if (!h || which < 0 || which > 6) { adf_set_error("debug_row_maxima: null handle or which outside 0..6"); return ADF_EINVAL; }
+    if (!h || which < 0 || which > 14) { adf_set_error("debug_row_maxima: null handle or which outside 0..14"); return ADF_EINVAL; }
     if (which == 4) { h->dbg_capture = capacity != 0; h->dbg_comb_rows = 0; return ADF_OK; }
+    if (which >= 7) {
+        const int H = h->hp.hidden_channels, H2 = H / 2, n = h->dbg_head_rows;
+        if (!h->hmx_part || n <= 0) { adf_set_error("debug_row_maxima: the last head launch measured its rows itself"); return ADF_EINVAL; }
+        if (rows) *rows = n;
+        if (!out) return ADF_OK;
+        const int64_t need = which == 8 ? 3ll * n : which == 12 ? (int64_t)n * H : which >= 13 ? (int64_t)n * H2 : n;
+        if (capacity < need) { adf_set_error("debug_row_maxima: out holds %lld floats, need %lld", (long long)capacity, (long long)need); return ADF_EINVAL; }
+        hipStream_t s = (hipStream_t)stream;
+        if (which == 9) return adf_launch_rowmax_combine(h->npart0, h->part_stride, (H + 63) / 64, n, out, s);
+        if (which == 10) return adf_launch_rowmax_combine(h->npart1, h->part_stride, (H2 + 63) / 64, n, out, s);
+        const float* src = which == 7 ? h->dbg_hm_magx : which == 8 ? h->dbg_hm_magv : which == 11 ? h->x1mag : which == 12 ? h->cat
+                           : which == 13 ? h->dot : h->xh + (size_t)n * H;
+        ADF_HIP_CHECK(hipMemcpyAsync(out, src, sizeof(float) * (size_t)need, hipMemcpyDeviceToDevice, s));
+        return ADF_OK;
+    }
     const int H = h->hp.hidden_channels, ns = H / ADF_SLICE_CH;
     const int n = which <= 1 ? h->dbg_msg_rows : which <= 3 ? h->dbg_cat_rows : h->dbg_comb_rows;
     if (!h->rmx_part || n <= 0) { adf_set_error("debug_row_maxima: no launch has emitted row maxima (ADF_ROW_MAXIMA=0?)"); return ADF_EINVAL; }
@@ -691,6 +727,8 @@
             if (st == ADF_OK && l >= 1) st = dev_alloc(&h->incV[l], cap * 3 * H);
             if (st == ADF_OK && l < L) st = dev_alloc(&h->incR[l], (cap + 1) * 5 * H);
         }
+        if (st == ADF_OK && h->rmx) st = dev_alloc(&h->inc_magX, cap);
+        if (st == ADF_OK && h->rmx) st = dev_alloc(&h->inc_magV, 3 * cap);
         if (st == ADF_OK) st = dev_alloc(&h->inc_c0, cap);
         if (st == ADF_OK) st = dev_alloc(&h->inc_chg, 2 * cap);
         if (st == ADF_OK) st = dev_alloc(&h->inc_pend, cap * L);
@@ -788,6 +826,10 @@
     if (h->inc_sync) ADF_TRY(inc_harvest(h, slot, true, true));
     adf_prof_end(h, s);
     if (first) ADF_TRY(make_records(h, 0, N, h->incX[0], nullptr, true, h->incR[0], nullptr, s));
+    const bool mags_before = h->inc_mag_valid && !first;
+    bool mags_ok = mags_before;
+    h->inc_mag_valid = false;
+    const head_mag_dst hm_all = {h->inc_magX, h->inc_magV, nullptr};
     for (int l = 0; l < L; ++l) {
         const int n_seen = h->inc_seen_valid ? h->inc_seen[l] : N;
         const bool whole = first || !h->inc_seen_valid || h->inc_pend_Nseen != N || (long long)n_seen * 10 >= (long long)N * 9;
@@ -797,6 +839,8 @@
         if (whole) {
             ADF_TRY(message_layer(h, l, N, h->incX[l], vin, h->incX[l + 1], h->incV[l + 1], l == 0, s, nullptr, 0,
                                   h->incR[l], true));
+            if (l + 1 == L) ADF_TRY(update_layer(h, l, N, h->incX[l + 1], h->incV[l + 1], s, true, &hm_all, &mags_ok));
+            else
             ADF_TRY(update_layer(h, l, N, h->incX[l + 1], h->incV[l + 1], s));
             if (l + 1 < L)
                 ADF_TRY(make_records(h, l + 1, N, h->incX[l + 1], h->incV[l + 1], false, h->incR[l + 1], nullptr, s));
@@ -806,6 +850,10 @@
         const int ncap = h->inc_sync ? n_seen : N;
         h->rows_dev = h->inc_cnt + l;
         int32_t st = message_layer(h, l, N, h->incX[l], vin, h->x, h->vecB, l == 0, s, list, ncap, h->incR[l], true);
+        if (st == ADF_OK && l + 1 == L) {
+            const head_mag_dst hm_list = {mags_before ? h->inc_magX : nullptr, h->inc_magV, list};
+            st = update_layer(h, l, ncap, h->x, h->vecB, s, true, &hm_list, &mags_ok);
+        } else
         if (st == ADF_OK) st = update_layer(h, l, ncap, h->x, h->vecB, s);
         if (st == ADF_OK) {
             adf_prof_begin(h, ADF_PROF_NODE, s);
@@ -817,10 +865,13 @@
         h->rows_dev = nullptr;
         ADF_TRY(st);
     }
+    h->inc_mag_valid = mags_ok;
     adf_prof_begin(h, ADF_PROF_HEADS, s);
     if (!out_idx) {
+        if (mags_ok) { h->hm_x = h->incX[L]; h->hm_vec = h->incV[L]; h->hm_n = N; h->hm_magx = h->inc_magX; h->hm_magv = h->inc_magV; }
         if (heads >= 1) ADF_TRY(adf_head_forward(h, 0, N, h->incX[L], h->incV[L], f1, s));
         if (heads == 2) ADF_TRY(adf_head_forward(h, 1, N, h->incX[L], h->incV[L], f2, s));
+        h->hm_x = h->hm_vec = nullptr;
         h->x_last = h->incX[L];
     } else {
         if (n_out > h->capS) {
@@ -856,6 +907,7 @@
     if (heads > h->hp.num_heads) { adf_set_error("the model has no force head"); return ADF_EINVAL; }
     if (!b->atomic_numbers || (heads >= 1 && !f1) || (heads == 2 && !f2)) { adf_set_error("null argument"); return ADF_EINVAL; }
     h->x_last = nullptr;
+    h->hm_x = h->hm_vec = nullptr;
     hipStream_t s = (hipStream_t)stream;
     const int N = b->num_atoms;
     ADF_TRY(ensure_capacity(h, N, b->num_systems));
@@ -892,12 +944,19 @@
             if (l == 0) ADF_TRY(message_layer(h, 0, N, h->x, vin, h->x, vout, true, s, nullptr, 0, rec0, rec0_ready));
             else
             ADF_TRY(message_layer(h, l, N, h->x, vin, h->x, vout, l == 0, s));
+            if (l + 1 == L) {
+                const head_mag_dst hm = {h->mag_xl, h->mag_v3, nullptr};
+                bool emitted = false;
+                ADF_TRY(update_layer(h, l, N, h->x, vout, s, true, &hm, &emitted));
+                if (emitted) { h->hm_x = h->x; h->hm_vec = vout; h->hm_n = N; h->hm_magx = h->mag_xl; h->hm_magv = h->mag_v3; h->mag_v3_valid = false; }
+            } else
             ADF_TRY(update_layer(h, l, N, h->x, vout, s));
             float* t = vin; vin = vout; vout = t;
         }
         adf_prof_begin(h, ADF_PROF_HEADS, s);
         if (heads >= 1) ADF_TRY(adf_head_forward(h, 0, N, h->x, vin, f1, s));
         if (heads == 2) ADF_TRY(adf_head_forward(h, 1, N, h->x, vin, f2, s));
+        h->hm_x = h->hm_vec = nullptr;
         adf_prof_end(h, s);
         h->x_last = h->x;
         return ADF_OK;
diff --git a/adsorbdiff_amd/csrc/common.h b/adsorbdiff_amd/csrc/common.h
--- a/adsorbdiff_amd/csrc/common.h
+++ b/adsorbdiff_amd/csrc/common.h
@@ -13,6 +13,7 @@
 #define ADF_MAX_K 128
 #define ADF_NFLAGS 8
 #define ADF_MAX_INDEG 1024
+#define ADF_MSG_VZ_WAVES_DEFAULT 8
 #define ADF_MAX_LAYERS 16
 
 void adf_set_error(const char* fmt, ...);
@@ -66,6 +67,8 @@
     long long rec_rows;
     float* catpart;
     long long part_stride;
+    float* hxpart;
+    float* hvpart;
 };
 struct adf_lift {
     float* buf;
@@ -104,6 +107,7 @@
     int fused_mlp;
     bool gemm_f32;
     bool msg_f32;
+    int msg_vz_waves;
     bool lift_on;
     adf_lift lift;
     float *mag_a, *mag_b;
@@ -120,6 +124,15 @@
     bool dbg_capture;
     float* dbg_mag;
     int dbg_comb_rows;
+    float* hmx_part;
+    float *hxpart, *hvpart, *npart0, *npart1, *x1mag;
+    float* mag_xl;
+    float *inc_magX, *inc_magV;
+    bool inc_mag_valid;
+    const float *hm_x, *hm_vec, *hm_magx, *hm_magv;
+    int hm_n;
+    int dbg_head_rows;
+    const float *dbg_hm_magx, *dbg_hm_magv;
 
     int64_t capN, capB, capE;
     int32_t* nbr_cnt;
@@ -209,11 +222,13 @@
 int32_t adf_launch_rowmag(const float* A, int lda, int K1, const float* A2, int K2, long long M, float* mag, hipStream_t s,
                           const int32_t* m_dev = nullptr, int m_mul = 1);
 int32_t adf_launch_rowmax_combine(const float* part, long long stride, int nparts, long long M, float* mag, hipStream_t s,
-                                  const int32_t* m_dev = nullptr, int m_mul = 1);
+                                  const int32_t* m_dev = nullptr, int m_mul = 1, const float* extra = nullptr,
+                                  const int32_t* list = nullptr);
 int32_t adf_split_weight(const float* w, long long n, adf_w16* out, unsigned int* scratch_bits, hipStream_t s,
                          int perm_H = 0, int K = 0, const float* bias = nullptr, int parts = 3);
 int32_t adf_launch_gemm16_vecnorm(const float* A, int lda, const adf_w16* W, float* nrm, int M, int N, int K,
-                                  hipStream_t s, const adf_lift* lf = nullptr, const float* premag = nullptr);
+                                  hipStream_t s, const adf_lift* lf = nullptr, const float* premag = nullptr,
+                                  float* normpart = nullptr, long long part_stride = 0);
 int32_t adf_launch_gemm16_fused(const float* A, int lda, const adf_w16* W, int M, int H, int K, int epi,
                                 const adf_epi* ep, hipStream_t s, const adf_lift* lf = nullptr);
 static inline int32_t adf_linear(const adf_painn* h, const float* A, int lda, const float* W, const adf_w16* W16,
diff --git a/adsorbdiff_amd/csrc/gemm16.hip b/adsorbdiff_amd/csrc/gemm16.hip
--- a/adsorbdiff_amd/csrc/gemm16.hip
+++ b/adsorbdiff_amd/csrc/gemm16.hip
@@ -37,7 +37,7 @@
     return s * 1.6666666666666667f;
 }
 
-template <int ACT, int MI, int NJ, int EPI, bool WR = false, int NWN = 2>
+template <int ACT, int MI, int NJ, int EPI, bool WR = false, int NWN = 2, bool EMX = false>
 __global__ __launch_bounds__(128 * NWN, (MI == 4 || NWN == 4 ? 1 : 2)) void adf_gemm_f16x3_kernel(
     const float* __restrict__ A, int lda, const _Float16* __restrict__ Whi, const _Float16* __restrict__ Wlo,
     const float* __restrict__ inv_scale, const float* __restrict__ bias, float* __restrict__ C, int ldc, int Mh, int N,
@@ -457,12 +457,21 @@
         }
         __builtin_amdgcn_fence(__ATOMIC_RELEASE, "wavefront");
         __builtin_amdgcn_wave_barrier();
+        float keep = 0.f;
 #pragma unroll
         for (int it = 0; it < 8; ++it) {
             const int lr = it * 4 + (lane >> 4), c4 = lane & 15;
             const int n = a0 + lr, c = cb + 4 * c4;
-            if (n < M && c < N)
-                *reinterpret_cast<float4*>(ep.cat + (size_t)n * N + c) = *reinterpret_cast<const float4*>(T + lr * TLD2 + 4 * c4);
+            const float4 nv_ = *reinterpret_cast<const float4*>(T + lr * TLD2 + 4 * c4);
+            if (n < M && c < N) *reinterpret_cast<float4*>(ep.cat + (size_t)n * N + c) = nv_;
+            if (ep.catpart) {
+                const float mg = adf_row16_max(c < N ? fmaxf(fmaxf(fmaxf(0.f, fabsf(nv_.x)), fabsf(nv_.y)), fmaxf(fabsf(nv_.z), fabsf(nv_.w))) : 0.f);
+                if (c4 == it) keep = mg;
+            }
+        }
+        if (ep.catpart) {
+            const int c4 = lane & 15, n = a0 + c4 * 4 + (lane >> 4);
+            if (c4 < 8 && n < M && cb < N) ep.catpart[(size_t)(cb / 64) * ep.part_stride + n] = keep;
         }
     } else {
         static_assert(EPI >= 3 || (NJ == 3 && MI == 2), "fused epilogues are written for the 64 x 96 wave tile");
@@ -532,6 +541,7 @@
                 }
             } else {
                 float4 d[4], xv[4], w1[4][3], tv[4][3];
+                float hkx = 0.f, hk0 = 0.f, hk1 = 0.f, hk2 = 0.f;
 #pragma unroll
                 for (int it = 0; it < 4; ++it) {
                     const int n = min(m0 + wm + 32 * i + it * 8 + (lane >> 3), M - 1);
@@ -576,6 +586,26 @@
 #else
 #define EPI2_ST(r_, p_, base_, v_) (*reinterpret_cast<float4*>(p_) = (v_))
 #endif
+                    if constexpr (EMX) {
+                        float4 tq[3];
+#pragma unroll
+                        for (int ax = 0; ax < 3; ++ax) {
+                            float4 t = tv[it][ax];
+                            const float4 v1 = w1[it][ax];
+                            t.x += p2.x * v1.x; t.y += p2.y * v1.y; t.z += p2.z * v1.z; t.w += p2.w * v1.w;
+                            tq[ax] = t;
+                        }
+                        if (n < M) {
+                            EPI2_ST(rx, ep.x + (size_t)n * H + c, ep.x, xo4);
+                            float* vr = ep.vec + (size_t)n * 3 * H + c;
+#pragma unroll
+                            for (int ax = 0; ax < 3; ++ax) EPI2_ST(rv, vr + ax * H, ep.vec, tq[ax]);
+                        }
+                        auto amax4 = [](const float4& v) { return fmaxf(fmaxf(fmaxf(0.f, fabsf(v.x)), fabsf(v.y)), fmaxf(fabsf(v.z), fabsf(v.w))); };
+                        const float mxx = adf_lane8_max(amax4(xo4));
+                        const float mv0 = adf_lane8_max(amax4(tq[0])), mv1 = adf_lane8_max(amax4(tq[1])), mv2 = adf_lane8_max(amax4(tq[2]));
+                        if (c4 == it) { hkx = mxx; hk0 = mv0; hk1 = mv1; hk2 = mv2; }
+                    } else
                     if (n < M) {
                         EPI2_ST(rx, ep.x + (size_t)n * H + c, ep.x, xo4);
                         float* vr = ep.vec + (size_t)n * 3 * H + c;
@@ -588,6 +618,14 @@
                         }
                     }
 #undef EPI2_ST
+                }
+                if constexpr (EMX) {
+                    const int n = m0 + wm + 32 * i + c4 * 8 + (lane >> 3);
+                    if (c4 < 4 && n < M) {
+                        ep.hxpart[(size_t)g * ep.part_stride + n] = hkx;
+                        float* vs = ep.hvpart + (size_t)g * 3 * ep.part_stride + 3 * (size_t)n;
+                        vs[0] = hk0; vs[1] = hk1; vs[2] = hk2;
+                    }
                 }
             }
             __builtin_amdgcn_wave_barrier();
@@ -622,19 +660,21 @@
 
 __global__ __launch_bounds__(256) void adf_rowmax_combine_kernel(const float* __restrict__ part, long long stride, int nparts,
                                                                  long long M, float* __restrict__ mag,
-                                                                 const int32_t* __restrict__ m_dev, int m_mul) {
+                                                                 const int32_t* __restrict__ m_dev, int m_mul,
+                                                                 const float* __restrict__ extra,
+                                                                 const int32_t* __restrict__ list) {
     const long long r = (long long)blockIdx.x * 256 + threadIdx.x;
     if (r >= M || (m_dev && r >= (long long)*m_dev * m_mul)) return;
-    float mx = 0.f;
+    float mx = extra ? fmaxf(0.f, extra[r]) : 0.f;
     for (int p = 0; p < nparts; ++p) mx = fmaxf(mx, part[(size_t)p * stride + r]);
-    mag[r] = mx;
+    mag[list ? (long long)list[r / m_mul] * m_mul + r % m_mul : r] = mx;
 }
 
 int32_t adf_launch_rowmax_combine(const float* part, long long stride, int nparts, long long M, float* mag, hipStream_t s,
-                                  const int32_t* m_dev, int m_mul) {
+                                  const int32_t* m_dev, int m_mul, const float* extra, const int32_t* list) {
     if (M <= 0) return ADF_OK;
     hipLaunchKernelGGL(adf_rowmax_combine_kernel, dim3((unsigned)((M + 255) / 256)), dim3(256), 0, s, part, stride, nparts, M,
-                       mag, m_dev, m_mul);
+                       mag, m_dev, m_mul, extra, list);
     ADF_HIP_CHECK(hipGetLastError());
     return ADF_OK;
 }
@@ -768,12 +808,13 @@
 }
 
 int32_t adf_launch_gemm16_vecnorm(const float* A, int lda, const adf_w16* W, float* nrm, int M, int N, int K,
-                                  hipStream_t s, const adf_lift* lf, const float* premag) {
+                                  hipStream_t s, const adf_lift* lf, const float* premag, float* normpart, long long part_stride) {
     if (M <= 0) return ADF_OK;
     if (K % HK != 0 || (lda & 3) || (N & 3)) { adf_set_error("gemm16_vecnorm: bad shape"); return ADF_EINVAL; }
     ADF_TRY(check_a_span(3ll * M, lda));
     adf_epi ep = {};
     ep.cat = nrm;
+    ep.catpart = normpart; ep.part_stride = part_stride;
     ADF_TRY(lift_mags(A, lda, K, nullptr, 0, 3ll * M, lf, premag, &ep.rmag, s));
     const int tn = (N + 127) / 128, tm8 = ((M + 63) / 64 + 7) / 8 * 8;
     static int w8 = -1;
@@ -835,14 +876,23 @@
         hipLaunchKernelGGL((adf_gemm_f16x3_kernel<0, 2, 3, EPI_, true, NWN_>), gw, dim3(128 * NWN_), 0, s, A, lda,            \
                            (const _Float16*)W->frag, (const _Float16*)nullptr, W->inv_scale, W->bias_perm, (float*)nullptr, 0, \
                            M, N, K, tnw, *ep)
+#define LAUNCHWFX(NWN_)                                                                                                       \
+        hipLaunchKernelGGL((adf_gemm_f16x3_kernel<0, 2, 3, 2, true, NWN_, true>), gw, dim3(128 * NWN_), 0, s, A, lda,         \
+                           (const _Float16*)W->frag, (const _Float16*)nullptr, W->inv_scale, W->bias_perm, (float*)nullptr, 0, \
+                           M, N, K, tnw, *ep)
         if (epi == 1) { if (wf == 4) LAUNCHWF(1, 4); else LAUNCHWF(1, 2); }
+        else if (ep->hxpart) { if (wf == 4) LAUNCHWFX(4); else LAUNCHWFX(2); }
         else { if (wf == 4) LAUNCHWF(2, 4); else LAUNCHWF(2, 2); }
 #undef LAUNCHWF
+#undef LAUNCHWFX
         ADF_HIP_CHECK(hipGetLastError());
         return ADF_OK;
     }
     if (epi == 1)
         hipLaunchKernelGGL((adf_gemm_f16x3_kernel<0, 2, 3, 1>), grid, dim3(256), 0, s, A, lda, (const _Float16*)W->hi,
+                           (const _Float16*)W->lo, W->inv_scale, W->bias_perm, (float*)nullptr, 0, M, N, K, tiles_n, *ep);
+    else if (ep->hxpart)
+        hipLaunchKernelGGL((adf_gemm_f16x3_kernel<0, 2, 3, 2, false, 2, true>), grid, dim3(256), 0, s, A, lda, (const _Float16*)W->hi,
                            (const _Float16*)W->lo, W->inv_scale, W->bias_perm, (float*)nullptr, 0, M, N, K, tiles_n, *ep);
     else
         hipLaunchKernelGGL((adf_gemm_f16x3_kernel<0, 2, 3, 2>), grid, dim3(256), 0, s, A, lda, (const _Float16*)W->hi,
diff --git a/adsorbdiff_amd/csrc/message.hip b/adsorbdiff_amd/csrc/message.hip
--- a/adsorbdiff_amd/csrc/message.hip
+++ b/adsorbdiff_amd/csrc/message.hip
@@ -31,9 +31,8 @@
 #define FWD_AHEAD 4
 #endif
 #define FWD_THREADS (64 * FWD_WAVES)
-#define MSG_WAVES_PER_SIMD (FWD_WAVES / 4)
-template <bool F16, bool VZ, bool UNI>
-__global__ __launch_bounds__(FWD_THREADS, MSG_WAVES_PER_SIMD) void adf_message_kernel(MsgParams p) {
+template <bool F16, bool VZ, bool UNI, int NW = FWD_WAVES>
+__global__ __launch_bounds__(64 * NW, NW / 4) void adf_message_kernel(MsgParams p) {
     extern __shared__ __attribute__((aligned(16))) float lds[];
     const int wfloats = F16 ? (2 * MSG_COLS * MSG_LDK) / 2 : p.R * MSG_COLS;
     float* Wl = lds;
@@ -42,7 +41,7 @@
     float* Bl = lds + wfloats;
     float* Mu = Bl + MSG_COLS;
     float* Meta = Mu + 144;
-    int* Ctr = reinterpret_cast<int*>(Meta + FWD_WAVES * 32 * 8);
+    int* Ctr = reinterpret_cast<int*>(Meta + NW * 32 * 8);
 
     const int tid = threadIdx.x;
     const int lane = tid & 63;
@@ -64,7 +63,7 @@
             const half8* src = reinterpret_cast<const half8*>(p.wpack16 + (size_t)slice * 2 * MSG_COLS * p.R);
             const half8 zero8 = {0, 0, 0, 0, 0, 0, 0, 0};
             const _Float16* b16 = reinterpret_cast<const _Float16*>(p.bpack) + (size_t)slice * MSG_COLS * 2;
-            for (int i = tid; i < 2 * MSG_COLS * 17; i += FWD_THREADS) {
+            for (int i = tid; i < 2 * MSG_COLS * 17; i += 64 * NW) {
                 const int row = i / 17, piece = i - row * 17;
                 half8 v = piece < R8 ? src[row * R8 + piece] : zero8;
                 if (piece == 16 && row < MSG_COLS) { v[0] = b16[2 * row]; v[1] = b16[2 * row + 1]; }
@@ -74,7 +73,7 @@
             const float4* src = reinterpret_cast<const float4*>(p.wpack + (size_t)slice * p.R * MSG_COLS);
             float4* dst = reinterpret_cast<float4*>(Wl);
             const int n4 = p.R * MSG_COLS / 4;
-            for (int i = tid; i < n4; i += FWD_THREADS) dst[i] = src[i];
+            for (int i = tid; i < n4; i += 64 * NW) dst[i] = src[i];
         }
         if (!F16 && tid < MSG_COLS) Bl[tid] = p.bpack[slice * MSG_COLS + tid];
         if (tid < 144) Mu[tid] = (tid < p.R ? p.mu[tid] : 2.0f) * (F16 ? p.sarg : 1.0f);
@@ -502,9 +501,9 @@
     return ADF_OK;
 }
 
-static size_t msg_lds_bytes(int R, bool f16) {
+static size_t msg_lds_bytes(int R, bool f16, int waves = FWD_WAVES) {
     const size_t w = f16 ? (size_t)2 * MSG_COLS * MSG_LDK * 2 : sizeof(float) * (size_t)R * MSG_COLS;
-    return w + sizeof(float) * (MSG_COLS + 144 + FWD_WAVES * 32 * 8) + 16;
+    return w + sizeof(float) * (MSG_COLS + 144 + waves * 32 * 8) + 16;
 }
 
 int32_t adf_pack_rbf_layer(adf_painn* h, int l, hipStream_t s) {
@@ -545,6 +544,11 @@
         SET_LDS(false, false, false); SET_LDS(false, true, false); SET_LDS(true, false, false); SET_LDS(true, true, false);
         SET_LDS(true, false, true); SET_LDS(true, true, true);
 #undef SET_LDS
+#define SET_LDS12(UNI_)                                                                                       \
+    ADF_HIP_CHECK(hipFuncSetAttribute(reinterpret_cast<const void*>(adf_message_kernel<true, true, UNI_, 12>), \
+                                      hipFuncAttributeMaxDynamicSharedMemorySize, (int)msg_lds_bytes(128, true, 12)))
+        SET_LDS12(false); SET_LDS12(true);
+#undef SET_LDS12
     }
     return ADF_OK;
 }
@@ -593,10 +597,14 @@
         const double d = sqrt(0.5 / (step * step) * 1.4426950408889634) * step;
         p.dmu2 = (float)(2.0 * d); p.dmusq = (float)(d * d); p.cstep = (float)exp2(-2.0 * d * d);
     }
-    if (f16 && h->rbf_uniform) { if (vec_is_zero) LAUNCH_MSG(true, true, true); else LAUNCH_MSG(true, false, true); }
+#define LAUNCH_MSG12(UNI_)                                                                                  \
+    hipLaunchKernelGGL((adf_message_kernel<true, true, UNI_, 12>), grid, dim3(64 * 12), msg_lds_bytes(R, true, 12), s, p)
+    if (f16 && vec_is_zero && h->msg_vz_waves == 12) { if (h->rbf_uniform) LAUNCH_MSG12(true); else LAUNCH_MSG12(false); }
+    else if (f16 && h->rbf_uniform) { if (vec_is_zero) LAUNCH_MSG(true, true, true); else LAUNCH_MSG(true, false, true); }
     else if (f16) { if (vec_is_zero) LAUNCH_MSG(true, true, false); else LAUNCH_MSG(true, false, false); }
     else { if (vec_is_zero) LAUNCH_MSG(false, true, false); else LAUNCH_MSG(false, false, false); }
 #undef LAUNCH_MSG
+#undef LAUNCH_MSG12
     ADF_HIP_CHECK(hipGetLastError());
     return ADF_OK;
 }
diff --git a/adsorbdiff_amd/csrc/nodewise.hip b/adsorbdiff_amd/csrc/nodewise.hip
--- a/adsorbdiff_amd/csrc/nodewise.hip
+++ b/adsorbdiff_amd/csrc/nodewise.hip
@@ -174,6 +174,23 @@
         reinterpret_cast<float4*>(xout + (size_t)n * Cout)[c] =
             make_float4(ssilu_d(xs.x), ssilu_d(xs.y), ssilu_d(xs.z), ssilu_d(xs.w));
     }
+}
+
+__global__ __launch_bounds__(256) void adf_head_xact_mag_kernel(const float* __restrict__ o, float* __restrict__ xout,
+                                                                 float* __restrict__ mag, int N, int Cout) {
+    const int lane = threadIdx.x & 63;
+    const int n = blockIdx.x * 4 + (threadIdx.x >> 6);
+    if (n >= N) return;
+    float mg = 0.f;
+    for (int c = lane; c < Cout / 4; c += 64) {
+        const float4 xs = reinterpret_cast<const float4*>(o + (size_t)n * 2 * Cout)[c];
+        const float4 v = make_float4(ssilu_d(xs.x), ssilu_d(xs.y), ssilu_d(xs.z), ssilu_d(xs.w));
+        reinterpret_cast<float4*>(xout + (size_t)n * Cout)[c] = v;
+        mg = fmaxf(fmaxf(fmaxf(mg, fabsf(v.x)), fabsf(v.y)), fmaxf(fabsf(v.z), fabsf(v.w)));
+    }
+#pragma unroll
+    for (int of = 32; of > 0; of >>= 1) mg = fmaxf(mg, __shfl_xor(mg, of));
+    if (lane == 0) mag[n] = mg;
 }
 
 __global__ __launch_bounds__(256) void adf_head_final_kernel(const float* __restrict__ u, const float* __restrict__ v,
@@ -255,29 +272,39 @@
     float* cat1 = h->dot;
     const bool lift = h->lift_on && !h->gemm_f32;
     const adf_lift* lf = lift ? &h->lift : nullptr;
+    static int fuse_gate = -1;
+    if (fuse_gate < 0) { const char* e = getenv("ADF_HEAD_GATE_FUSED"); fuse_gate = (e && atoi(e) == 0) ? 0 : 1; }
+    const bool fg = fuse_gate && !h->gemm_f32 && (H2 & 3) == 0;
+    const bool have = lift && fg && h->rmx && h->npart0 && x == h->hm_x && vec == h->hm_vec && N == h->hm_n && N <= h->part_stride;
+    const long long ps = h->part_stride;
     const float* vmag = nullptr;
-    if (lift) {
+    if (have) {
+        vmag = h->hm_magv;
+        h->mag_v3_valid = false;
+        h->dbg_head_rows = N; h->dbg_hm_magx = h->hm_magx; h->dbg_hm_magv = h->hm_magv;
+    } else if (lift) {
         if (head == 0 || !h->mag_v3_valid) ADF_TRY(adf_launch_rowmag(vec, H, H, nullptr, 0, 3ll * N, h->mag_v3, s));
         h->mag_v3_valid = head == 0;
         vmag = h->mag_v3;
+        h->dbg_head_rows = 0;
     }
     if (h->gemm_f32) {
         ADF_TRY(adf_linear(h, vec, H, b0.vec1_w, &b0.vec1_16, nullptr, t1, H, 3 * N, H, H, 0, s));
         hipLaunchKernelGGL(adf_head_norm_cat_kernel, dim3(ew_grid((long long)N * H / 4)), dim3(256), 0, s, x, t1, h->cat, N, H);
     } else {
-        ADF_TRY(adf_launch_gemm16_vecnorm(vec, H, &b0.vec1_16, h->cat, N, H, H, s, lf, vmag));
-    }
-    static int fuse_gate = -1;
-    if (fuse_gate < 0) { const char* e = getenv("ADF_HEAD_GATE_FUSED"); fuse_gate = (e && atoi(e) == 0) ? 0 : 1; }
-    const bool fg = fuse_gate && !h->gemm_f32 && (H2 & 3) == 0;
+        ADF_TRY(adf_launch_gemm16_vecnorm(vec, H, &b0.vec1_16, h->cat, N, H, H, s, lf, vmag, have ? h->npart0 : nullptr, ps));
+        if (have) ADF_TRY(adf_launch_rowmax_combine(h->npart0, ps, (H + 63) / 64, N, h->lift.buf, s, nullptr, 1, h->hm_magx));
+    }
     if (!fg) ADF_TRY(adf_linear(h, vec, H, b0.vec2_w, &b0.vec2_16, nullptr, t2, H2, 3 * N, H2, H, 0, s, vmag));
     if (h->gemm_f32) ADF_TRY(adf_linear(h, h->cat, 2 * H, b0.un0_w, &b0.un0_16, b0.un0_b, h->y, H, N, H, 2 * H, 1, s));
     else ADF_TRY(adf_launch_gemm16(x, H, &b0.un0_16, b0.un0_b, h->y, H, N, H, 2 * H, 1, s, h->cat, H,
-                                   h->lift_on ? &h->lift : nullptr, nullptr, h->lift_on ? h->mag_b : nullptr));
+                                   h->lift_on ? &h->lift : nullptr, have ? h->lift.buf : nullptr, h->lift_on ? h->mag_b : nullptr));
     ADF_TRY(adf_linear(h, h->y, H, b0.un2_w, &b0.un2_16, b0.un2_b, o, H, N, H, H, 0, s, (h->lift_on && !h->gemm_f32) ? h->mag_b : nullptr));
     if (fg) {
         ADF_TRY(adf_launch_gemm16(vec, H, &b0.vec2_16, nullptr, v1, H2, 3 * N, H2, H, 0, s, nullptr, 0, lf, vmag,
                                   lift ? h->lift.buf : nullptr, nullptr, 0, o + H2, H));
+        if (have) hipLaunchKernelGGL(adf_head_xact_mag_kernel, dim3((N + 3) / 4), dim3(256), 0, s, o, x1, h->x1mag, N, H2);
+        else
         hipLaunchKernelGGL(adf_head_xact_kernel, dim3(ew_grid((long long)N * H2 / 4)), dim3(256), 0, s, o, x1, N, H2);
     } else
     hipLaunchKernelGGL(adf_head_gate_kernel, dim3(ew_grid((long long)N * H2 / 4)), dim3(256), 0, s, o, t2, x1, v1, N, H2);
@@ -287,8 +314,10 @@
         ADF_TRY(adf_linear(h, cat1, H, b1.un0_w, &b1.un0_16, b1.un0_b, h->y, H2, N, H2, H, 1, s));
     } else {
         ADF_TRY(adf_launch_gemm16_vecnorm(v1, H2, &b1.vec1_16, cat1, N, H2, H2, s, h->lift_on ? &h->lift : nullptr,
-                                          (fg && lift) ? h->lift.buf : nullptr));
-        ADF_TRY(adf_launch_gemm16(x1, H2, &b1.un0_16, b1.un0_b, h->y, H2, N, H2, H, 1, s, cat1, H2, h->lift_on ? &h->lift : nullptr));
+                                          (fg && lift) ? h->lift.buf : nullptr, have ? h->npart1 : nullptr, ps));
+        if (have) ADF_TRY(adf_launch_rowmax_combine(h->npart1, ps, (H2 + 63) / 64, N, h->lift.buf, s, nullptr, 1, h->x1mag));
+        ADF_TRY(adf_launch_gemm16(x1, H2, &b1.un0_16, b1.un0_b, h->y, H2, N, H2, H, 1, s, cat1, H2, h->lift_on ? &h->lift : nullptr,
+                                  have ? h->lift.buf : nullptr));
     }
     hipLaunchKernelGGL(adf_head_final_kernel, dim3((N + 3) / 4), dim3(256), 0, s, h->y, v1, b1.vec2_w, b1.un2_w,
                        b1.un2_b, out, N, H2, h->flags);
```
